# ufal/neuralmonkey

Hardware: AMD Instinct MI355X
Metric: target tokens/sec/node (train), 512-hid GRU+attn (higher is better)
Workload: dtype f32; 1 GPU; translation.ini-shape: biGRU-512 enc + Bahdanau attn + GRU-512 dec, B=128/GPU, src_len=tgt_len=50, V=32000, weights N(0,0.05)/orthogonal (BASELINE.md 3), CrossEntropyTrainer(l2=1e-8, clip_norm=1.0) + Adam(1e-4), one optimizer step per step, 8 distinct HBM-resident batches in rotation; global_batch=128, seq_len=50, parallelism=dp1

## Files before the change

neuralmonkey_amd/_lib.py:

```python
import ctypes
import os
from ctypes import c_char_p, c_float, c_int, c_int64, c_void_p

import torch

_HERE = os.path.dirname(os.path.abspath(__file__))
LIB_PATH = os.path.join(_HERE, "libnmhip.so")

_lib = None

P = c_void_p
I = c_int
L = c_int64
F = c_float

SIGNATURES = {
    "nm_last_error": (c_char_p, []),
    "nm_version": (I, []),
    "nm_crc32c": (ctypes.c_uint32, [ctypes.c_uint32, P, L]),
    "nm_gemm_f32": (I, [P, I, I, L, L, L, P, L, P, L, P, L, P, I, I, L, L, L, L, I, P, L]),
    "nm_gemm_f32_group": (I, [P, I, I, L, L, L, P, L, L, L, I, L]),
    "nm_gemm_f32_chain": (I, [P, L, L, L, L, P, L, L, P, L, I, P, L]),
    "nm_colsum_chain": (I, [P, P, ctypes.c_int32, ctypes.c_int32, L, L, L, L, P, I, P, L]),
    "nm_outer_chain": (I, [P, P, L, L, L, L, L, L, P, I]),
    "nm_embedding_gather": (I, [P, P, L, L, P, L, P, L, I, F]),
    "nm_gru_gates_fwd": (I, [P, P, L, L, L, P, P, P, P, P, I, I, I, L, L]),
    "nm_gru_blend_fwd": (I, [P, P, L, L, L, P, P, P, P, P, P, L, L, L, P, I, I, I, L, L]),
    "nm_layer_norm_fwd": (I, [P, P, L, P, P, P, L, P, P, L, L, F]),
    "nm_add_layer_norm_fwd": (I, [P, P, L, P, L, P, P, P, L, P, L, L, L, F]),
    "nm_add_layer_norm_stats_fwd": (I, [P, P, P, P, P, P, P, P, P, L, L, F]),
    "nm_copy_cols": (I, [P, P, L, P, L, L, L]),
    "nm_reduce_sum": (I, [P, P, L, P]),
    "nm_log_softmax": (I, [P, P, L, P, P, P, L, L, L]),
    "nm_attn_workspace_bytes": (L, [L, L, L]),
    "nm_attn_fwd": (I, [P, P, P, P, P, P, P, L, L, L, L, L, P, L, P, P, L, P]),
    "nm_attn_fwd_multi": (I, [P, P, P, P, P, P, P, L, L, L, L, L, L, L, P, L, P, P, L, P]),
    "nm_gru_rh_seq": (I, [P, P, P, P, P, I, L, L, I, L]),
    "nm_gru_gemm": (I, [P, P, I, L, P, L, L, P, L, L]),
    "nm_gru_seq_fwd": (I, [P, P, ctypes.c_int32, L, L, L, L, P, L, L, P, L, L, P, L, P]),
    "nm_gru_seq_bwd": (I, [P, P, ctypes.c_int32, L, L, P, L, L, P, L, L, P, L, P]),
    "nm_lstm_seq_workspace_bytes": (L, [L, L, ctypes.c_int32]),
    "nm_lstm_seq_fwd": (I, [P, P, ctypes.c_int32, L, L, L, P, L, L, F, P, L, P]),
    "nm_lstm_seq_bwd": (I, [P, P, ctypes.c_int32, L, L, P, L, L, P, L, P]),
    "nm_nematus_seq_workspace_bytes": (L, [L, L, ctypes.c_int32]),
    "nm_nematus_seq_fwd": (I, [P, P, ctypes.c_int32, L, L, L, L, P, L, L, P, L, L, P, P, P, L, P]),
    "nm_nematus_seq_bwd": (I, [P, P, ctypes.c_int32, L, L, L, P, L, L, P, L, L, P, L, P]),
    "nm_proj_split_bytes": (L, [L, L]),
    "nm_proj_split_prepare": (I, [P, P, L, I, L, L, P, L]),
    "nm_proj_split_forget": (I, [P]),
    "nm_gru_seq_supported": (I, [L, L, ctypes.c_int32]),
    "nm_gru_seq_workspace_bytes": (L, [L, L, ctypes.c_int32]),
    "nm_gru_seq_failed": (I, [P]),
    "nm_gru_seq_force_give_up": (I, [ctypes.c_int32]),
    "nm_gru_seq_test_hog": (I, [P, ctypes.c_int32, L, L]),
    "nm_test_xcc_ids": (I, [P, P, ctypes.c_int32, ctypes.c_int32]),
    "nm_create": (I, [I, P]),
    "nm_destroy": (I, [P]),
    "nm_ctx_bind": (I, [P]),
    "nm_ctx_current": (P, []),
    "nm_ctx_device": (I, [P]),
    "nm_ctx_switch": (I, [P, c_char_p, P]),
    "nm_ctx_set_background": (I, [P, I]),
    "nm_allreduce_unique_id": (I, [P, L]),
    "nm_allreduce_init": (I, [I, I, P, P]),
    "nm_allreduce_bucket": (I, [P, P, P, L]),
    "nm_allreduce_wait": (I, [P, P]),
    "nm_allreduce_destroy": (I, [P]),
    "nm_prof_enable": (I, [P, I]),
    "nm_prof_attn_step": (I, [P, P, P]),
    "nm_row_stats": (I, [P, P, L, L, L, P, P, P]),
    "nm_gumbel_argmax": (I, [P, P, L, L, L, ctypes.c_uint32, P]),
    "nm_greedy_update": (I, [P, P, P, P, P, L, I, P]),
    "nm_xent": (I, [P, P, L, L, L, P, P, P, P, I, F]),
    "nm_xent_colsum": (I, [P, P, L, L, L, P, P, P, P, F, P, L]),
    "nm_beam_workspace_bytes": (L, [L, L, L]),
    "nm_beam_topk_step": (I, [P, P, L, L, L, L, P, P, P, P, P, P, I, P, P, P, P, P, P, P, P, L, P]),
    "nm_beam_topk_step_fused": (I, [P, P, L, L, L, L, P, P, P, P, I, P, P, P, P, P, P, P, P, L, P, P, P]),
    "nm_tanh_bwd": (I, [P, P, P, L]),
    "nm_colsum_workspace_bytes": (L, [L]),
    "nm_colsum": (I, [P, P, L, L, L, P, I, P, L]),
    "nm_colsum_algo": (I, [P, P, L, L, L, P, I, P, L, I]),
    "nm_embedding_scatter_add": (I, [P, P, L, L, P, L, P, L, I]),
    "nm_layer_norm_bwd": (I, [P, P, P, P, P, P, P, P, L, L]),
    "nm_layer_norm_bwd_params_workspace_bytes": (L, [L]),
    "nm_layer_norm_bwd_params": (I, [P, P, P, P, P, P, P, L, L, P, P, I, P, L]),
    "nm_gru_step_bwd": (I, [P, I, P, P, L, L, L, P, P, P, P, L, L, L, P, L, L, L, P, P, P, P, I, I, I, L, L]),
    "nm_gru_seq_shift": (I, [P, P, P, P, I, L, L, I, L]),
    "nm_attn_softmax_bwd": (I, [P, P, P, P, P, L, L, L]),
    "nm_attn_energy_bwd": (I, [P, P, P, P, P, P, P, P, L, L, L, L, I]),
    "nm_attn_step_bwd": (I, [P, P, L, P, P, P, P, P, L, P, P, P, L, L, L, L, L]),
    "nm_attn_softmax_fwd": (I, [P, P, P, P, L, L, L, L]),
    "nm_ew": (I, [P, I, P, L, P, L, P, L, L, L, F, I]),
    "nm_blend_fwd": (I, [P, P, L, P, L, P, L, P, L, L, L]),
    "nm_blend_bwd": (I, [P, P, L, P, L, P, L, P, L, P, L, P, L, P, L, L, L]),
    "nm_gemm_bf16x3_nt": (I, [P, L, L, L, P, L, P, L, P, L, I, I]),
    "nm_lstm_cell_fwd": (I, [P, P, L, P, L, P, L, P, L, P, L, L, L, F]),
    "nm_lstm_cell_bwd": (I, [P, P, L, P, L, P, L, P, L, P, L, P, L, P, L, L, L, I, I]),
    "nm_nematus_cell_fwd": (I, [P, P, L, P, L, P, L, P, L, P, L, P, P, P, L, L, L]),
    "nm_nematus_state_step": (I, [P, P, L, P, L, P, P, L, P, L, P, P, P, L, L, L]),
    "nm_nematus_full_step": (I, [P, P, L, P, L, P, P, L, P, L, P, P, L, P, P, P, L, L, L, L]),
    "nm_nematus_cell_bwd": (I, [P, P, L, P, P, P, L, P, L, P, L, P, L, P, L, P, L, P, L, L, L, I, I, I, I]),
    "nm_dropout": (I, [P, P, L, P, L, L, L, F, ctypes.c_uint32, P, I]),
    "nm_rnn_select_fwd": (I, [P, P, L, P, L, P, I, P, L, P, L, L, L]),
    "nm_rnn_select_bwd": (I, [P, P, L, P, L, P, I, P, L, P, L, L, L]),
    "nm_reverse_sequence": (I, [P, P, P, P, L, L, L, I]),
    "nm_maxout_fwd": (I, [P, P, L, P, L, P, L, L, L]),
    "nm_maxout_bwd": (I, [P, P, L, P, P, L, L, L, L]),
    "nm_sdp_attn_fwd": (I, [P, P, L, P, L, P, L, P, L, L, L, L, L, L, L, I, F, ctypes.c_uint32, P, P, L, P]),
    "nm_sdp_attn_step": (I, [P, P, L, P, L, P, L, P, L, L, L, L, L, P, L, P, L, P]),
    "nm_sdp_attn_bwd": (I, [P, P, L, P, L, P, L, P, L, P, P, L, L, L, L, L, L, I, F, ctypes.c_uint32, P,
                            P, L, P, L, P, L, P, I]),
    "nm_add_position": (I, [P, P, P, P, L, L, L, L]),
    "nm_unfinished_mask": (I, [P, P, P, L, L]),
    "nm_time_sum": (I, [P, P, P, L, L, L]),
    "nm_time_bcast_add": (I, [P, P, P, L, L, L]),
    "nm_optim_workspace_bytes": (L, [L, L]),
    "nm_optim_regularize_norms": (I, [P, P, P, P, P, P, P, P, P, L, L, F, F, P, P, L]),
    "nm_optim_clip_adam": (I, [P, P, P, P, P, P, P, P, P, P, P, L, L, F, F, F, F, F, P, L]),
    "nm_optim_clip_adadelta": (I, [P, P, P, P, P, P, P, P, P, P, P, L, L, F, F, F, F, P, L]),
    "nm_optim_partials": (I, [P, P, P, P, P, P, P, P, P, L, L, F, F, L, L, P, L]),
    "nm_optim_partials_list": (I, [P, P, P, P, P, P, P, P, P, L, L, F, F, P, L, P, L]),
    "nm_optim_apply_list": (I, [P, I, P, P, P, P, P, P, P, P, P, P, L, L, F, F, F, F, F, P, L, P, P, L]),
    "nm_optim_segments": (I, [P, P, P, P, P, P, P, L, L, P, P, L]),
    "nm_optim_apply": (I, [P, I, P, P, P, P, P, P, P, P, P, P, L, L, F, F, F, F, F, L, L, P, P, L]),
    "nm_zero_if": (I, [P, P, P, L]),
    "nm_fill_u32": (I, [P, P, L, ctypes.c_uint32]),
    "nm_copy_d2d": (I, [P, P, P, L]),
    "nm_gather_rows_f32": (I, [P, P, L, P, P, L, L, L]),
    "nm_beam_reorder_tokens": (I, [P, P, P, P, P, L, L]),
    "nm_beam_backtrace": (I, [P, P, P, P, P, L, L]),
    "nm_logits_stats_tile": (L, [L]),
    "nm_logits_stats_bytes": (L, [L, L]),
    "nm_logits_stats_gemm": (I, [P, I, L, L, L, P, L, P, L, P, P, L, P, L]),
    "nm_greedy_finish": (I, [P, P, L, L, P, P, P, I, P, P, L, L, P, L, P, P, P]),
    "nm_attn_partials_layout": (I, [L, L, L, L, P, P, P]),
    "nm_attn_fwd_partials": (I, [P, P, P, P, P, P, P, L, L, L, L, L, P, L]),
    "nm_step_group": (I, [P, L, P, ctypes.c_int32]),
    "nm_decoder_step_fused": (I, [P, P]),
    "nm_dec_step_cluster_supported": (I, [L, L, L, L]),
    "nm_dec_step_cluster_workspace_bytes": (L, [L, L]),
    "nm_prof_stream_read": (I, [P, P, L, P]),
    "nm_beam_topk_step_tiles": (I, [P, P, L, P, L, L, L, L, P, P, P, P, I, P, P, P, P, P, P, P, P, L, P, P, P]),
    "nm_conv1d_pool_fwd": (I, [P, P, L, I, I, I, I, I, P, P, P, P, P, P, L, P, P, P, P, I]),
    "nm_conv1d_wgrad_workspace_bytes": (L, [I, I, I, I, P, P]),
    "nm_conv1d_pool_bwd": (I, [P, P, L, I, I, I, I, I, P, P, P, P, P, P, L, P, P, I, P, P, I, P, L, I]),
    "nm_highway_fwd": (I, [P, P, P, L, P, L, P, P, P, P, P, L, L]),
    "nm_highway_bwd": (I, [P, P, P, L, P, P, P, P, L, P, L, L, I]),
}

CTC_SIGNATURES = {
    "nm_ctc_workspace_bytes": (L, [L, L, L]),
    "nm_ctc_mask_lengths": (I, [P, P, L, L, L, P]),
    "nm_ctc_loss_fwd": (I, [P, P, L, L, L, L, L, P, L, P, P, I, P, P, P, L]),
    "nm_ctc_loss_bwd": (I, [P, P, L, L, L, L, L, P, L, P, P, P, P, L, L, P, L]),
    "nm_ctc_greedy": (I, [P, P, L, L, L, L, L, P, I, ctypes.c_int32, P, P, P, L]),
}

LABEL_SIGNATURES = {
    "nm_label_rows_max_classes": (L, []),
    "nm_label_rows": (I, [P, P, L, L, L, P, ctypes.c_int32, P, I, P, P, L, P, P, ctypes.c_int32, P]),
    "nm_label_rows_from_stats": (I, [P, P, L, L, L, P, ctypes.c_int32, P, P, P, P, P, P, ctypes.c_int32, P]),
}

POOL_SIGNATURES = {
    "nm_pool_fwd": (I, [P, I, P, L, P, L, L, L, P, L, P]),
    "nm_pool_bwd": (I, [P, I, P, L, P, P, L, P, P, L, L, L, L, P, L, I]),
    "nm_time_softmax_fwd": (I, [P, P, L, P, L, L, L, P, L, P, L, P]),
    "nm_time_softmax_bwd": (I, [P, P, L, P, L, P, P, L, L, L, P, L, I]),
    "nm_sqerr_rows": (I, [P, P, L, L, L, P, P, I, P]),
}

CONVS2S_SIGNATURES = {
    "nm_conv1d_glu_fwd": (I, [P, P, L, L, L, L, L, P, P, P, L, P, P, I]),
    "nm_conv1d_glu_workspace_bytes": (L, [L, L, L, L]),
    "nm_conv1d_glu_bwd": (I, [P, P, L, L, L, L, L, P, P, P, P, L, P, P, L, I, P, P, I, P, L, I]),
}



class NMHipError(RuntimeError):
    pass


class GruEpilogue(ctypes.Structure):
    _fields_ = [("mode", ctypes.c_int32), ("t", ctypes.c_int32), ("rev_mask", ctypes.c_int32),
                ("ndir", ctypes.c_int32), ("R", L), ("H", L), ("lengths", P),
                ("xp", P), ("x_dir", L), ("x_row", L), ("x_time", L),
                ("h_in", P), ("h_out", P), ("ru", P), ("rh", P), ("c_save", P),
                ("out", P), ("o_dir", L), ("o_row", L), ("o_time", L),
                ("dh", P), ("dout", P), ("do_dir", L), ("do_row", L), ("do_time", L),
                ("c", P), ("h0", P), ("hseq", P), ("hs_dir", L), ("hs_row", L), ("hs_time", L),
                ("dxp", P), ("dx_dir", L), ("dx_row", L), ("dx_time", L),
                ("dgpre", P), ("dcpre", P)]


class StepProblem(ctypes.Structure):
    _fields_ = [("A", P), ("lda", L), ("Bt", P), ("ldb", L), ("N", L), ("K", L),
                ("a_kind", ctypes.c_int32), ("epilogue", ctypes.c_int32), ("act", ctypes.c_int32),
                ("nchunk", ctypes.c_int32),
                ("bias", P), ("add", P), ("ldadd", L), ("C", P), ("ldc", L),
                ("pctx", P), ("pstat", P), ("energies", P), ("mask", P), ("weights", P),
                ("S", L), ("mask_div", L), ("mask_mod", L),
                ("h", P), ("ldh", L), ("ru", P), ("rh", P), ("xc", P), ("ldxc", L),
                ("h_out", P), ("ldho", L), ("h_out2", P), ("ldho2", L), ("add_ids", P), ("xc_ids", P)]


class DecoderStep(ctypes.Structure):
    _fields_ = ([(n, L) for n in ("rows", "emb", "rnn", "attn_state", "ctx_width", "out", "vocab", "src_len",
                                  "rows_per_key")] +
                [("cat", P), ("h_copy", P), ("ld_h_copy", L), ("out_state", P), ("ld_out_state", L),
                 ("attn_weights", P), ("logits", P), ("ld_logits", L), ("stats", P), ("stats_bytes", L)] +
                [(n, P) for n in ("ru", "rh", "xc", "y", "pre_e", "pre", "ctx")] +
                [("attn_workspace", P), ("attn_workspace_bytes", L)] +
                [(n, P) for n in ("wg_t", "bg", "wcx_t", "wch_t", "bc", "wq_t", "bq", "keys", "values", "mask", "v",
                                  "attn_bias", "wo_h_t", "wo_e_t", "wo_c_t", "bo", "w_vocab")] +
                [("ld_w_vocab", L), ("b_vocab", P), ("out_act", ctypes.c_int32), ("vocab_trans_b", ctypes.c_int32)] +
                [(n, L) for n in ("ld_cat", "ld_ctx", "ld_wg", "ld_wcx", "ld_wch", "ld_wq", "ld_wo_h", "ld_wo_e",
                                  "ld_wo_c")] +
                [("in_table", P), ("ld_table", L), ("in_ids", P)] +
                [("cluster_ws", P), ("cluster_ws_bytes", L), ("sticky_error", P)])


def load():
    global _lib
    if _lib is not None:
        return _lib
    if not os.path.exists(LIB_PATH):
        raise NMHipError(
            f"{LIB_PATH} is missing: build it with `python -m neuralmonkey_amd.build` "
            "(hipcc --offload-arch=gfx950). There is no CPU fallback.")
    lib = ctypes.CDLL(LIB_PATH)
    for name, (res, args) in (list(SIGNATURES.items()) + list(CTC_SIGNATURES.items())
                              + list(LABEL_SIGNATURES.items()) + list(POOL_SIGNATURES.items())
                              + list(CONVS2S_SIGNATURES.items())):
        fn = getattr(lib, name)
        fn.restype = res
        fn.argtypes = args
    _lib = lib
    return lib


def check(code, what):
    if code != 0:
        msg = load().nm_last_error()
        raise NMHipError(f"{what} failed ({code}): {msg.decode() if msg else '?'}")
```

neuralmonkey_amd/csrc/nm_gemm.hip:

```cpp
#include <atomic>

#include "nm_common.h"

#include <stdlib.h>

typedef float f32x16 __attribute__((ext_vector_type(16)));

bool nm_medium_gemm(hipStream_t st, int transB, long M, long N, long K, const float* A, long lda, const float* B,
                    long ldb, float* C, long ldc, const float* bias, int act, int accumulate);

struct GemmArgs {
    const float* A;
    const float* B;
    float* C;
    const float* bias;
    int M, N, K;
    long lda, ldb, ldc;
    long sA, sB, sC;
    int act;
    int accumulate;
    float* ws;
    int splitk;
    int swizzle;
    float* stats;
    int store_c;
    int prio;
    const float* const* ptrs;
    int chain_k;
};

__device__ __forceinline__ float apply_act(float x, int act) {
    if (act == 1) return nm_tanh(x);
    if (act == 2) return fmaxf(x, 0.0f);
    return x;
}

__device__ __forceinline__ void store_tile32(const GemmArgs& g, float* __restrict__ C,
                                             const f32x16& acc, int m0, int n0, int lane) {
    const int col = n0 + (lane & 31);
    if (col >= g.N) return;
    const float bv = g.bias ? g.bias[col] : 0.0f;
#pragma unroll
    for (int r = 0; r < 16; ++r) {
        const int row = m0 + (r & 3) + 8 * (r >> 2) + 4 * (lane >> 5);
        if (row < g.M) {
            float* p = C + (long)row * g.ldc + col;
            float v = acc[r] + bv;
            if (g.accumulate) v += *p;
            *p = apply_act(v, g.act);
        }
    }
}

template <int WM, int WN, int TM, int TN, bool TA, bool TB, bool VEC, int BK, bool STATS = false, int PF = 1,
          int NCH = 1, bool CHAIN = false>
__global__ __launch_bounds__(WM * WN * 64) void gemm_tiled(GemmArgs g, int tiles_m) {
    static_assert(!CHAIN || (TA && !TB && VEC && !STATS), "chained K: the weight-gradient form only");
    constexpr int NT = WM * WN * 64;
    constexpr int BM = WM * 32 * TM, BN = WN * 32 * TN;
    constexpr int LA = BM * BK / 4 / NT, LB = BN * BK / 4 / NT, KQ = BK / 4;
    static_assert(LA >= 1 && LB >= 1 && LA * NT * 4 == BM * BK && LB * NT * 4 == BN * BK, "tile / thread mismatch");
    constexpr int LDAS = BM + 4, LDBS = BN + 4;
    constexpr int A_FLOATS = 2 * BK * LDAS, B_FLOATS = 2 * BK * LDBS;
    constexpr int ST_ROWS = BM > 256 ? 128 : BM / 2;
    constexpr int ST_FLOATS = STATS ? ST_ROWS * (BN + 1) + 3 * NT : 0;
    constexpr int SM_FLOATS = A_FLOATS + B_FLOATS > ST_FLOATS ? A_FLOATS + B_FLOATS : ST_FLOATS;
    static_assert((A_FLOATS * 4) % 16 == 0, "B tile must stay 16-byte aligned");
    __shared__ __attribute__((aligned(16))) float smem[SM_FLOATS];
    float (*As)[BK][LDAS] = reinterpret_cast<float (*)[BK][LDAS]>(smem);
    float (*Bs)[BK][LDBS] = reinterpret_cast<float (*)[BK][LDBS]>(smem + A_FLOATS);

    const int tid = threadIdx.x, lane = tid & 63, wave = tid >> 6;
    int bm, bn;
    {
        const int npid = (int)gridDim.x;
        int pid = (int)blockIdx.x;
        if (g.swizzle) {
            const int per = npid / 8, rem = npid % 8, x = pid % 8, i = pid / 8;
            pid = x * per + (x < rem ? x : rem) + i;
            constexpr int GROUP_M = 8;
            const int tiles_n = npid / tiles_m;
            const int width = GROUP_M * tiles_n;
            const int group = pid / width, first = group * GROUP_M;
            const int gsz = (tiles_m - first) < GROUP_M ? (tiles_m - first) : GROUP_M;
            bm = first + (pid % width) % gsz;
            bn = (pid % width) / gsz;
        } else {
            bm = pid % tiles_m;
            bn = pid / tiles_m;
        }
    }
    const int m0 = bm * BM, n0 = bn * BN;
    const float* __restrict__ A = (g.ptrs && !CHAIN) ? g.ptrs[3 * blockIdx.z] : g.A + (long)blockIdx.z * g.sA;
    const float* __restrict__ B = (g.ptrs && !CHAIN) ? g.ptrs[3 * blockIdx.z + 1] : g.B + (long)blockIdx.z * g.sB;
    float* __restrict__ C = (g.ptrs && !CHAIN) ? const_cast<float*>(g.ptrs[3 * blockIdx.z + 2]) : g.C + (long)blockIdx.z * g.sC;

    float4 ra0[LA], rb0[LB], ra1[PF == 2 ? LA : 1], rb1[PF == 2 ? LB : 1];

    auto load_a = [&](int k0, float4* ra) {
#pragma unroll
        for (int it = 0; it < LA; ++it) {
            const int idx = tid + it * NT;
            int m, k;
            if (TA) { k = idx / (BM / 4); m = (idx % (BM / 4)) * 4; }
            else    { m = idx / KQ;       k = (idx % KQ) * 4; }
            const int gm = m0 + m, gk = k0 + k;
            float4 v = make_float4(0.f, 0.f, 0.f, 0.f);
            if (TA) {
                const float* p = A + (long)gk * g.lda + gm;
                if constexpr (CHAIN) {
                    const int mem = k0 / g.chain_k;
                    p = g.ptrs[3 * mem] + (long)(gk - mem * g.chain_k) * g.lda + gm;
                }
                if (gk < g.K) {
                    if (VEC) { if (gm < g.M) v = *reinterpret_cast<const float4*>(p); }
                    else {
                        if (gm + 0 < g.M) v.x = p[0];
                        if (gm + 1 < g.M) v.y = p[1];
                        if (gm + 2 < g.M) v.z = p[2];
                        if (gm + 3 < g.M) v.w = p[3];
                    }
                }
            } else {
                const float* p = A + (long)gm * g.lda + gk;
                if (gm < g.M) {
                    if (VEC) { if (gk < g.K) v = *reinterpret_cast<const float4*>(p); }
                    else {
                        if (gk + 0 < g.K) v.x = p[0];
                        if (gk + 1 < g.K) v.y = p[1];
                        if (gk + 2 < g.K) v.z = p[2];
                        if (gk + 3 < g.K) v.w = p[3];
                    }
                }
            }
            ra[it] = v;
        }
    };
    auto load_b = [&](int k0, float4* rb) {
#pragma unroll
        for (int it = 0; it < LB; ++it) {
            const int idx = tid + it * NT;
            int n, k;
            if (!TB) { k = idx / (BN / 4); n = (idx % (BN / 4)) * 4; }
            else     { n = idx / KQ;       k = (idx % KQ) * 4; }
            const int gn = n0 + n, gk = k0 + k;
            float4 v = make_float4(0.f, 0.f, 0.f, 0.f);
            if (!TB) {
                const float* p = B + (long)gk * g.ldb + gn;
                if constexpr (CHAIN) {
                    const int mem = k0 / g.chain_k;
                    p = g.ptrs[3 * mem + 1] + (long)(gk - mem * g.chain_k) * g.ldb + gn;
                }
                if (gk < g.K) {
                    if (VEC) { if (gn < g.N) v = *reinterpret_cast<const float4*>(p); }
                    else {
                        if (gn + 0 < g.N) v.x = p[0];
                        if (gn + 1 < g.N) v.y = p[1];
                        if (gn + 2 < g.N) v.z = p[2];
                        if (gn + 3 < g.N) v.w = p[3];
                    }
                }
            } else {
                const float* p = B + (long)gn * g.ldb + gk;
                if (gn < g.N) {
                    if (VEC) { if (gk < g.K) v = *reinterpret_cast<const float4*>(p); }
                    else {
                        if (gk + 0 < g.K) v.x = p[0];
                        if (gk + 1 < g.K) v.y = p[1];
                        if (gk + 2 < g.K) v.z = p[2];
                        if (gk + 3 < g.K) v.w = p[3];
                    }
                }
            }
            rb[it] = v;
        }
    };
    auto store_lds = [&](int buf, const float4* ra, const float4* rb) {
#pragma unroll
        for (int it = 0; it < LA; ++it) {
            const int idx = tid + it * NT;
            if (TA) {
                const int k = idx / (BM / 4), m = (idx % (BM / 4)) * 4;
                *reinterpret_cast<float4*>(&As[buf][k][m]) = ra[it];
            } else {
                const int m = idx / KQ, k = (idx % KQ) * 4;
                As[buf][k + 0][m] = ra[it].x;
                As[buf][k + 1][m] = ra[it].y;
                As[buf][k + 2][m] = ra[it].z;
                As[buf][k + 3][m] = ra[it].w;
            }
        }
#pragma unroll
        for (int it = 0; it < LB; ++it) {
            const int idx = tid + it * NT;
            if (!TB) {
                const int k = idx / (BN / 4), n = (idx % (BN / 4)) * 4;
                *reinterpret_cast<float4*>(&Bs[buf][k][n]) = rb[it];
            } else {
                const int n = idx / KQ, k = (idx % KQ) * 4;
                Bs[buf][k + 0][n] = rb[it].x;
                Bs[buf][k + 1][n] = rb[it].y;
                Bs[buf][k + 2][n] = rb[it].z;
                Bs[buf][k + 3][n] = rb[it].w;
            }
        }
    };

    static_assert(NCH == 1 || NCH == 2 || NCH == 4, "accumulation chains: 1, 2 or 4");
    static_assert(NCH == 1 || PF == 1, "chains are implemented for the one-tile-ahead loop");
    f32x16 accs[NCH][TM][TN];
#pragma unroll
    for (int c = 0; c < NCH; ++c)
#pragma unroll
        for (int i = 0; i < TM; ++i)
#pragma unroll
            for (int j = 0; j < TN; ++j)
#pragma unroll
                for (int r = 0; r < 16; ++r) accs[c][i][j][r] = 0.0f;
    f32x16 (&acc)[TM][TN] = accs[0];

    const int wm = (wave / WN) * 32 * TM, wn = (wave % WN) * 32 * TN;
    const int nkt_all = (g.K + BK - 1) / BK;
    const int per_slice = (nkt_all + g.splitk - 1) / g.splitk;
    const int kt0 = blockIdx.y * per_slice;
    const int nkt = min(nkt_all, kt0 + per_slice);

    auto mma_tile = [&](int cur, f32x16 (&acc)[TM][TN]) {
        float a[2][TM], b[2][TN];
#pragma unroll
        for (int i = 0; i < TM; ++i) a[0][i] = As[cur][lane >> 5][wm + i * 32 + (lane & 31)];
#pragma unroll
        for (int j = 0; j < TN; ++j) b[0][j] = Bs[cur][lane >> 5][wn + j * 32 + (lane & 31)];
#pragma unroll
        for (int kk = 0; kk < BK; kk += 2) {
            const int p = (kk >> 1) & 1;
            if (kk + 2 < BK) {
                const int kr = kk + 2 + (lane >> 5);
#pragma unroll
                for (int i = 0; i < TM; ++i) a[p ^ 1][i] = As[cur][kr][wm + i * 32 + (lane & 31)];
#pragma unroll
                for (int j = 0; j < TN; ++j) b[p ^ 1][j] = Bs[cur][kr][wn + j * 32 + (lane & 31)];
            }
#pragma unroll
            for (int i = 0; i < TM; ++i)
#pragma unroll
                for (int j = 0; j < TN; ++j)
                    acc[i][j] = __builtin_amdgcn_mfma_f32_32x32x2f32(a[p][i], b[p][j], acc[i][j], 0, 0, 0);
            __builtin_amdgcn_sched_group_barrier(0x100, TM + TN, 0);
            __builtin_amdgcn_sched_group_barrier(0x008, TM * TN, 0);
        }
    };

    load_a(kt0 * BK, ra0);
    load_b(kt0 * BK, rb0);
    store_lds(0, ra0, rb0);
    __syncthreads();
    if constexpr (PF == 2) {
        if (kt0 + 1 < nkt) { load_a((kt0 + 1) * BK, ra1); load_b((kt0 + 1) * BK, rb1); }
        int kt = kt0;
        while (kt < nkt) {
            if (kt + 2 < nkt) { load_a((kt + 2) * BK, ra0); load_b((kt + 2) * BK, rb0); }
            mma_tile(0, accs[0]);
            if (kt + 1 < nkt) store_lds(1, ra1, rb1);
            __syncthreads();
            if (++kt >= nkt) break;
            if (kt + 2 < nkt) { load_a((kt + 2) * BK, ra1); load_b((kt + 2) * BK, rb1); }
            mma_tile(1, accs[0]);
            if (kt + 1 < nkt) store_lds(0, ra0, rb0);
            __syncthreads();
            ++kt;
        }
    } else if constexpr (NCH == 1) {
        int cur = 0;
        for (int kt = kt0; kt < nkt; ++kt) {
            if (kt + 1 < nkt) { load_a((kt + 1) * BK, ra0); load_b((kt + 1) * BK, rb0); }
            mma_tile(cur, accs[0]);
            if (kt + 1 < nkt) store_lds(cur ^ 1, ra0, rb0);
            __syncthreads();
            cur ^= 1;
        }
    } else {
        int kt = kt0;
        while (kt < nkt) {
#pragma unroll
            for (int c = 0; c < NCH; ++c) {
                if (kt + 1 < nkt) { load_a((kt + 1) * BK, ra0); load_b((kt + 1) * BK, rb0); }
                mma_tile(c & 1, accs[c]);
                if (kt + 1 < nkt) store_lds((c & 1) ^ 1, ra0, rb0);
                __syncthreads();
                if (++kt >= nkt) break;
            }
        }
#pragma unroll
        for (int i = 0; i < TM; ++i)
#pragma unroll
            for (int j = 0; j < TN; ++j) {
                if constexpr (NCH == 4) {
#pragma unroll
                    for (int r = 0; r < 16; ++r)
                        accs[0][i][j][r] = (accs[0][i][j][r] + accs[1][i][j][r]) + (accs[2][i][j][r] + accs[3][i][j][r]);
                } else {
#pragma unroll
                    for (int r = 0; r < 16; ++r) accs[0][i][j][r] += accs[1][i][j][r];
                }
            }
    }

    if (g.splitk > 1) {
        GemmArgs gs = g;
        gs.ldc = g.N; gs.bias = nullptr; gs.act = 0; gs.accumulate = 0;
        float* slab = g.ws + (long)blockIdx.y * g.M * g.N;
#pragma unroll
        for (int i = 0; i < TM; ++i)
#pragma unroll
            for (int j = 0; j < TN; ++j)
                store_tile32(gs, slab, acc[i][j], m0 + wm + i * 32, n0 + wn + j * 32, lane);
        return;
    }
    if constexpr (STATS) {
        if (g.act == 9) return;
        constexpr int HR = ST_ROWS, TS = BN + 1;
        constexpr int NP = BM / HR;
        static_assert(NP * HR == BM, "statistics epilogue: whole passes");
        constexpr int TPR = NT / HR, CW = BN / TPR;
        static_assert(NT % HR == 0 && BN % TPR == 0 && TPR <= 16, "statistics epilogue thread layout");
        float* T = smem;
        float* pmax = smem + HR * TS;
        int* parg = reinterpret_cast<int*>(pmax + NT);
        float* psum = pmax + 2 * NT;
        bool okj[TN];
#pragma unroll
        for (int j = 0; j < TN; ++j) {
            const int col = n0 + wn + j * 32 + (lane & 31);
            okj[j] = col < g.N;
            const float bv = (okj[j] && g.bias) ? g.bias[col] : 0.0f;
#pragma unroll
            for (int i = 0; i < TM; ++i)
#pragma unroll
                for (int r = 0; r < 16; ++r) acc[i][j][r] += bv;
        }
        const int tiles_n = (int)gridDim.x / tiles_m;
        const int rr = tid % HR, q = tid / HR;
        for (int h = 0; h < NP; ++h) {
            __syncthreads();
#pragma unroll
            for (int i = 0; i < TM; ++i) {
                const int rbase = wm + i * 32 - h * HR;
                if (rbase >= 0 && rbase < HR) {
#pragma unroll
                    for (int j = 0; j < TN; ++j)
#pragma unroll
                        for (int r = 0; r < 16; ++r)
                            T[(rbase + (r & 3) + 8 * (r >> 2) + 4 * (lane >> 5)) * TS + wn + j * 32 + (lane & 31)] =
                                okj[j] ? acc[i][j][r] : -INFINITY;
                }
            }
            __syncthreads();
            const float* trow = T + rr * TS + q * CW;
            float best = -INFINITY;
            int bi = 0x7fffffff;
#pragma unroll
            for (int c = 0; c < CW; ++c) {
                const float v = trow[c];
                if (v > best) { best = v; bi = n0 + q * CW + c; }
            }
            pmax[q * HR + rr] = best;
            parg[q * HR + rr] = bi;
            __syncthreads();
            float m = pmax[rr];
#pragma unroll
            for (int w = 1; w < TPR; ++w) m = fmaxf(m, pmax[w * HR + rr]);
            float sum = 0.0f;
#pragma unroll
            for (int c = 0; c < CW; ++c) sum += expf(trow[c] - m);
            psum[q * HR + rr] = sum;
            __syncthreads();
            const int row = m0 + h * HR + tid;
            if (tid < HR && row < g.M) {
                float tot = psum[tid];
                int a = parg[tid];
#pragma unroll
                for (int w = 1; w < TPR; ++w) {
                    tot += psum[w * HR + tid];
                }
                float bm = pmax[tid];
#pragma unroll
                for (int w = 1; w < TPR; ++w)
                    if (pmax[w * HR + tid] > bm) { bm = pmax[w * HR + tid]; a = parg[w * HR + tid]; }
                float4 rec;
                rec.x = bm; rec.y = tot; rec.z = __int_as_float(a); rec.w = 0.0f;
                *reinterpret_cast<float4*>(g.stats + ((long)row * tiles_n + bn) * 4) = rec;
            }
        }
        if (!g.store_c) return;
        GemmArgs gs = g;
        gs.bias = nullptr;
#pragma unroll
        for (int i = 0; i < TM; ++i)
#pragma unroll
            for (int j = 0; j < TN; ++j)
                store_tile32(gs, C, acc[i][j], m0 + wm + i * 32, n0 + wn + j * 32, lane);
        return;
    }
    if (!g.store_c) return;
#pragma unroll
    for (int i = 0; i < TM; ++i)
#pragma unroll
        for (int j = 0; j < TN; ++j)
            store_tile32(g, C, acc[i][j], m0 + wm + i * 32, n0 + wn + j * 32, lane);
}

__global__ void splitk_reduce(GemmArgs g) {
    const long idx = (long)blockIdx.x * blockDim.x + threadIdx.x;
    const long total = (long)g.M * g.N;
    if (idx >= total) return;
    const int row = (int)(idx / g.N), col = (int)(idx - (long)row * g.N);
    float s = 0.0f;
    for (int k = 0; k < g.splitk; ++k) s += g.ws[(long)k * total + idx];
    float* p = g.C + (long)row * g.ldc + col;
    float v = s + (g.bias ? g.bias[col] : 0.0f);
    if (g.accumulate) v += *p;
    *p = apply_act(v, g.act);
}

#include "nm_gru.h"

__device__ __forceinline__ void gru_epilogue(const GruEpi& e, int d, int row, int col, float s) {
    const int H = e.H;
    const long ro = (long)d * e.R + row;
    int pos, ppos;
    const bool live = gru_epi_pos(e, row, d, e.t, pos, ppos);
    if (e.mode == 1) {
        float gate = 0.0f;
        if (live) gate = nm_sigmoid(e.xp[d * e.x_dir + (long)row * e.x_row + (long)pos * e.x_time + col] + s);
        e.ru[ro * 2 * H + col] = gate;
        if (col < H) e.rh[ro * H + col] = live ? gate * e.h_in[ro * H + col] : 0.0f;
    } else if (e.mode == 2) {
        const float hp = e.h_in[ro * H + col];
        if (!live) {
            if (e.h_out != e.h_in) e.h_out[ro * H + col] = hp;
            if (e.c_save) e.c_save[ro * H + col] = 0.0f;
            return;
        }
        const float c = nm_tanh(e.xp[d * e.x_dir + (long)row * e.x_row + (long)pos * e.x_time + 2 * H + col] + s);
        const float u = e.ru[ro * 2 * H + H + col];
        const float hn = u * hp + (1.0f - u) * c;
        e.h_out[ro * H + col] = hn;
        if (e.c_save) e.c_save[ro * H + col] = c;
        if (e.out) e.out[d * e.o_dir + (long)row * e.o_row + (long)pos * e.o_time + col] = hn;
    } else if (e.mode == 3) {
        if (!live) { e.dgpre[ro * 2 * H + col] = 0.0f; return; }
        const float rr = e.ru[ro * 2 * H + col];
        const float hp = gru_epi_hprev(e, ro, d, row, e.t, ppos, col);
        const float drp = s * hp * rr * (1.0f - rr);
        e.dh[ro * H + col] += s * rr;
        e.dgpre[ro * 2 * H + col] = drp;
        e.dxp[d * e.dx_dir + (long)row * e.dx_row + (long)pos * e.dx_time + col] = drp;
    } else {
        if (!live) {
            e.dh[ro * H + col] = s;
            e.dcpre[ro * H + col] = 0.0f;
            e.dgpre[ro * 2 * H + H + col] = 0.0f;
            return;
        }
        float dhv = s;
        if (e.dout) dhv += e.dout[d * e.do_dir + (long)row * e.do_row + (long)pos * e.do_time + col];
        const float u = e.ru[ro * 2 * H + H + col];
        const float c = e.c[ro * H + col];
        const float hp = gru_epi_hprev(e, ro, d, row, e.t, ppos, col);
        const float dcp = dhv * (1.0f - u) * (1.0f - c * c);
        const float dup = dhv * (hp - c) * u * (1.0f - u);
        e.dh[ro * H + col] = dhv * u;
        e.dcpre[ro * H + col] = dcp;
        e.dgpre[ro * 2 * H + H + col] = dup;
        float* dx = e.dxp + d * e.dx_dir + (long)row * e.dx_row + (long)pos * e.dx_time;
        dx[H + col] = dup;
        dx[2 * H + col] = dcp;
    }
}

struct GruPre {
    float a, b, c, d;
    int pos, ppos;
    bool live;
};

__device__ __forceinline__ GruPre gru_epi_load(const GruEpi& e, int d, int row, int col, const float* __restrict__ C,
                                               long ldc, bool accumulate) {
    GruPre q;
    q.a = q.b = q.c = q.d = 0.0f;
    const int H = e.H;
    const long ro = (long)d * e.R + row;
    q.live = gru_epi_pos(e, row, d, e.t, q.pos, q.ppos);
    if (e.mode == 1) {
        if (q.live) q.a = e.xp[d * e.x_dir + (long)row * e.x_row + (long)q.pos * e.x_time + col];
        if (col < H && q.live) q.b = e.h_in[ro * H + col];
    } else if (e.mode == 2) {
        q.b = e.h_in[ro * H + col];
        if (q.live) {
            q.a = e.xp[d * e.x_dir + (long)row * e.x_row + (long)q.pos * e.x_time + 2 * H + col];
            q.c = e.ru[ro * 2 * H + H + col];
        }
    } else if (e.mode == 3) {
        if (q.live) {
            q.a = e.ru[ro * 2 * H + col];
            q.b = gru_epi_hprev(e, ro, d, row, e.t, q.ppos, col);
            q.c = e.dh[ro * H + col];
        }
    } else {
        if (accumulate) q.d = C[(long)row * ldc + col];
        if (q.live) {
            if (e.dout) q.a = e.dout[d * e.do_dir + (long)row * e.do_row + (long)q.pos * e.do_time + col];
            q.b = e.ru[ro * 2 * H + H + col];
            q.c = e.c[ro * H + col];
        }
    }
    return q;
}

__device__ __forceinline__ void gru_epi_apply(const GruEpi& e, const GruPre& q, int d, int row, int col, float s) {
    const int H = e.H;
    const long ro = (long)d * e.R + row;
    if (e.mode == 1) {
        const float gate = q.live ? nm_sigmoid(q.a + s) : 0.0f;
        e.ru[ro * 2 * H + col] = gate;
        if (col < H) e.rh[ro * H + col] = q.live ? gate * q.b : 0.0f;
    } else if (e.mode == 2) {
        const float hp = q.b;
        if (!q.live) {
            if (e.h_out != e.h_in) e.h_out[ro * H + col] = hp;
            if (e.c_save) e.c_save[ro * H + col] = 0.0f;
            return;
        }
        const float c = nm_tanh(q.a + s);
        const float u = q.c;
        const float hn = u * hp + (1.0f - u) * c;
        e.h_out[ro * H + col] = hn;
        if (e.c_save) e.c_save[ro * H + col] = c;
        if (e.out) e.out[d * e.o_dir + (long)row * e.o_row + (long)q.pos * e.o_time + col] = hn;
    } else if (e.mode == 3) {
        if (!q.live) { e.dgpre[ro * 2 * H + col] = 0.0f; return; }
        const float rr = q.a, hp = q.b;
        const float drp = s * hp * rr * (1.0f - rr);
        e.dh[ro * H + col] = q.c + s * rr;
        e.dgpre[ro * 2 * H + col] = drp;
        e.dxp[d * e.dx_dir + (long)row * e.dx_row + (long)q.pos * e.dx_time + col] = drp;
    } else {
        s += q.d;
        if (!q.live) {
            e.dh[ro * H + col] = s;
            e.dcpre[ro * H + col] = 0.0f;
            e.dgpre[ro * 2 * H + H + col] = 0.0f;
            return;
        }
        const float dhv = s + q.a;
        const float u = q.b, c = q.c;
        const float hp = gru_epi_hprev(e, ro, d, row, e.t, q.ppos, col);
        const float dcp = dhv * (1.0f - u) * (1.0f - c * c);
        const float dup = dhv * (hp - c) * u * (1.0f - u);
        e.dh[ro * H + col] = dhv * u;
        e.dcpre[ro * H + col] = dcp;
        e.dgpre[ro * 2 * H + H + col] = dup;
        float* dx = e.dxp + d * e.dx_dir + (long)row * e.dx_row + (long)q.pos * e.dx_time;
        dx[H + col] = dup;
        dx[2 * H + col] = dcp;
    }
}

template <int KS, bool TB>
__global__ __launch_bounds__(KS * 64) void gemm_skinny(GemmArgs g, int tiles_m, GruEpi epi) {
    if (g.prio) __builtin_amdgcn_s_setprio(3);
    __shared__ float red[KS][16][64];
    const int tid = threadIdx.x, lane = tid & 63, wave = tid >> 6;
    const int bm = blockIdx.x % tiles_m, bn = blockIdx.x / tiles_m;
    const int m0 = bm * 32, n0 = bn * 32;
    const float* __restrict__ A = g.A + (long)blockIdx.z * g.sA;
    const float* __restrict__ B = g.B + (long)blockIdx.z * g.sB;
    float* __restrict__ C = g.C + (long)blockIdx.z * g.sC;

    const int r = lane & 31, half = lane >> 5;
    const int mm = min(m0 + r, g.M - 1), nn = min(n0 + r, g.N - 1);
    const int kper = ((g.K / 8 + KS - 1) / KS) * 8;
    const int kbeg = wave * kper, kend = min(g.K, kbeg + kper);

    f32x16 acc;
#pragma unroll
    for (int i = 0; i < 16; ++i) acc[i] = 0.0f;

    const float* ap = A + (long)mm * g.lda + 4 * half;
    const float* bp = TB ? (B + (long)nn * g.ldb + 4 * half) : (B + (long)(4 * half) * g.ldb + nn);
    for (int k0 = kbeg; k0 < kend; k0 += 64) {
        float4 av[8], bv[8];
#pragma unroll
        for (int c = 0; c < 8; ++c) {
            const int k = k0 + 8 * c;
            av[c] = make_float4(0.f, 0.f, 0.f, 0.f);
            bv[c] = av[c];
            if (k < kend) {
                av[c] = *reinterpret_cast<const float4*>(ap + k);
                if (TB) {
                    bv[c] = *reinterpret_cast<const float4*>(bp + k);
                } else {
                    const float* q = bp + (long)k * g.ldb;
                    bv[c].x = q[0];
                    bv[c].y = q[g.ldb];
                    bv[c].z = q[2 * g.ldb];
                    bv[c].w = q[3 * g.ldb];
                }
            }
        }
#pragma unroll
        for (int c = 0; c < 8; ++c) {
            if (k0 + 8 * c >= kend) break;
            acc = __builtin_amdgcn_mfma_f32_32x32x2f32(av[c].x, bv[c].x, acc, 0, 0, 0);
            acc = __builtin_amdgcn_mfma_f32_32x32x2f32(av[c].y, bv[c].y, acc, 0, 0, 0);
            acc = __builtin_amdgcn_mfma_f32_32x32x2f32(av[c].z, bv[c].z, acc, 0, 0, 0);
            acc = __builtin_amdgcn_mfma_f32_32x32x2f32(av[c].w, bv[c].w, acc, 0, 0, 0);
        }
    }
#pragma unroll
    for (int i = 0; i < 16; ++i) red[wave][i][lane] = acc[i];
    __syncthreads();
    for (int o = tid; o < 16 * 64; o += KS * 64) {
        const int reg = o >> 6, ln = o & 63;
        float s = 0.0f;
#pragma unroll
        for (int w = 0; w < KS; ++w) s += red[w][reg][ln];
        const int col = n0 + (ln & 31);
        const int row = m0 + (reg & 3) + 8 * (reg >> 2) + 4 * (ln >> 5);
        if (row < g.M && col < g.N) {
            if (epi.mode) {
                if (g.accumulate) s += C[(long)row * g.ldc + col];
                gru_epilogue(epi, blockIdx.z, row, col, s);
                continue;
            }
            float* p = C + (long)row * g.ldc + col;
            float v = s + (g.bias ? g.bias[col] : 0.0f);
            if (g.accumulate) v += *p;
            *p = apply_act(v, g.act);
        }
    }
}

typedef float f32x4 __attribute__((ext_vector_type(4)));

template <int KS, bool TB>
__device__ __forceinline__ void skinny16_tile(const GemmArgs& g, int tiles_m, const GruEpi& epi, int tile, int z,
                                              float (*red)[4][64]) {
    const int tid = threadIdx.x, lane = tid & 63, wave = tid >> 6;
    const int bm = tile % tiles_m, bn = tile / tiles_m;
    const int m0 = bm * 16, n0 = bn * 16;
    const float* __restrict__ A = g.A + (long)z * g.sA;
    const float* __restrict__ B = g.B + (long)z * g.sB;
    float* __restrict__ C = g.C + (long)z * g.sC;

    const int i16 = lane & 15, kq = lane >> 4;
    const int mm = min(m0 + i16, g.M - 1), nn = min(n0 + i16, g.N - 1);
    const int kper = (((g.K + 15) / 16 + KS - 1) / KS) * 16;
    const int kbeg = wave * kper, kend = min(g.K, kbeg + kper);

    f32x4 acc;
#pragma unroll
    for (int i = 0; i < 4; ++i) acc[i] = 0.0f;

    const int e_col = n0 + (tid & 15), e_row = m0 + 4 * ((tid & 63) >> 4) + (tid >> 6);
    const bool e_ok = tid < 256 && e_row < g.M && e_col < g.N;
    GruPre pre;
    float e_bias = 0.0f, e_old = 0.0f;
    if (e_ok) {
        if (epi.mode) pre = gru_epi_load(epi, z, e_row, e_col, C, g.ldc, g.accumulate != 0);
        else {
            if (g.bias) e_bias = g.bias[e_col];
            if (g.accumulate) e_old = C[(long)e_row * g.ldc + e_col];
        }
    }

    const float* ap = A + (long)mm * g.lda + 4 * kq;
    const float* bp = TB ? (B + (long)nn * g.ldb + 4 * kq) : (B + (long)(4 * kq) * g.ldb + nn);
    for (int k0 = kbeg; k0 < kend; k0 += 64) {
        float4 av[4], bv[4];
#pragma unroll
        for (int c = 0; c < 4; ++c) {
            const int k = k0 + 16 * c;
            av[c] = make_float4(0.f, 0.f, 0.f, 0.f);
            bv[c] = av[c];
            if (k + 4 * kq < kend) {
                av[c] = *reinterpret_cast<const float4*>(ap + k);
                if (TB) {
                    bv[c] = *reinterpret_cast<const float4*>(bp + k);
                } else {
                    const float* q = bp + (long)k * g.ldb;
                    bv[c].x = q[0];
                    bv[c].y = q[g.ldb];
                    bv[c].z = q[2 * g.ldb];
                    bv[c].w = q[3 * g.ldb];
                }
            }
        }
#pragma unroll
        for (int c = 0; c < 4; ++c) {
            if (k0 + 16 * c >= kend) break;
            acc = __builtin_amdgcn_mfma_f32_16x16x4f32(av[c].x, bv[c].x, acc, 0, 0, 0);
            acc = __builtin_amdgcn_mfma_f32_16x16x4f32(av[c].y, bv[c].y, acc, 0, 0, 0);
            acc = __builtin_amdgcn_mfma_f32_16x16x4f32(av[c].z, bv[c].z, acc, 0, 0, 0);
            acc = __builtin_amdgcn_mfma_f32_16x16x4f32(av[c].w, bv[c].w, acc, 0, 0, 0);
        }
    }
#pragma unroll
    for (int i = 0; i < 4; ++i) red[wave][i][lane] = acc[i];
    __syncthreads();
    static_assert(KS >= 4, "the epilogue maps one output element to each of the first 256 threads");
    if (e_ok) {
// ... 45 lines not shown
        for (int i = 0; i < 4; ++i) acc[g][i] = 0.0f;
    const float* ap = p.h + (long)mm * p.ldh + 4 * kq;
    const float* bp = p.w + (long)(4 * kq) * p.ldw + un;
    for (int k0 = kbeg; k0 < kend; k0 += 64) {
        float4 av[4], bv[3][4];
#pragma unroll
        for (int c = 0; c < 4; ++c) {
            const int k = k0 + 16 * c;
            av[c] = make_float4(0.f, 0.f, 0.f, 0.f);
#pragma unroll
            for (int g = 0; g < 3; ++g) bv[g][c] = av[c];
            if (k + 4 * kq < kend) {
                av[c] = *reinterpret_cast<const float4*>(ap + k);
#pragma unroll
                for (int g = 0; g < 3; ++g) {
                    const float* q = bp + (long)k * p.ldw + (long)g * p.H;
                    bv[g][c].x = q[0];
                    bv[g][c].y = q[p.ldw];
                    bv[g][c].z = q[2 * p.ldw];
                    bv[g][c].w = q[3 * p.ldw];
                }
            }
        }
#pragma unroll
        for (int c = 0; c < 4; ++c) {
            if (k0 + 16 * c >= kend) break;
#pragma unroll
            for (int g = 0; g < 3; ++g) {
                acc[g] = __builtin_amdgcn_mfma_f32_16x16x4f32(av[c].x, bv[g][c].x, acc[g], 0, 0, 0);
                acc[g] = __builtin_amdgcn_mfma_f32_16x16x4f32(av[c].y, bv[g][c].y, acc[g], 0, 0, 0);
                acc[g] = __builtin_amdgcn_mfma_f32_16x16x4f32(av[c].z, bv[g][c].z, acc[g], 0, 0, 0);
                acc[g] = __builtin_amdgcn_mfma_f32_16x16x4f32(av[c].w, bv[g][c].w, acc[g], 0, 0, 0);
            }
        }
    }
#pragma unroll
    for (int g = 0; g < 3; ++g)
#pragma unroll
        for (int i = 0; i < 4; ++i) red[wave][g][i][lane] = acc[g][i];
    __syncthreads();
    static_assert(KS >= 4, "one output element per thread of the first four waves");
    const int e_col = u0 + (tid & 15), e_row = m0 + 4 * ((tid & 63) >> 4) + (tid >> 6);
    if (tid >= 256 || e_row >= p.M || e_col >= p.H) return;
    const int reg = tid >> 6, ln = tid & 63;
    float s[3];
#pragma unroll
    for (int g = 0; g < 3; ++g) {
        float t = 0.0f;
#pragma unroll
        for (int w = 0; w < KS; ++w) t += red[w][g][reg][ln];
        s[g] = t + (p.b ? p.b[g * p.H + e_col] : 0.0f);
    }
    const float* xr = p.x + (long)e_row * p.ldx + e_col;
    const float r = nm_sigmoid(s[0] + xr[0]);
    const float u = nm_sigmoid(s[1] + xr[p.H]);
    const float c = nm_tanh(s[2] * r + xr[2 * p.H]);
    p.hn[(long)e_row * p.ldhn + e_col] = u * p.h[(long)e_row * p.ldh + e_col] + (1.0f - u) * c;
    if (p.ru) {
        p.ru[(long)e_row * 2 * p.H + e_col] = r;
        p.ru[(long)e_row * 2 * p.H + p.H + e_col] = u;
    }
    if (p.c) p.c[(long)e_row * p.H + e_col] = c;
    if (p.sc) p.sc[(long)e_row * p.ldsc + e_col] = s[2];
}

struct NemFull {
    NemStep st;
    const float* xin; long ldxi;
    const float* wi; long ldwi;
    const float* bi;
    int D;
};

template <int KS>
__device__ __forceinline__ void nem_accumulate(const float* __restrict__ A, long lda, const float* __restrict__ W, long ldw,
                                               int H, int K, int mm, int un, int kq, int wave, f32x4& a0, f32x4& a1,
                                               f32x4& a2) {
    const int kper = (((K + 15) / 16 + KS - 1) / KS) * 16;
    const int kbeg = wave * kper, kend = min(K, kbeg + kper);
    const float* ap = A + (long)mm * lda + 4 * kq;
    const float* bp = W + (long)(4 * kq) * ldw + un;
    for (int k0 = kbeg; k0 < kend; k0 += 64) {
        float4 av[4], bv[3][4];
#pragma unroll
        for (int c = 0; c < 4; ++c) {
            const int k = k0 + 16 * c;
            av[c] = make_float4(0.f, 0.f, 0.f, 0.f);
#pragma unroll
            for (int g = 0; g < 3; ++g) bv[g][c] = av[c];
            if (k + 4 * kq < kend) {
                av[c] = *reinterpret_cast<const float4*>(ap + k);
#pragma unroll
                for (int g = 0; g < 3; ++g) {
                    const float* q = bp + (long)k * ldw + (long)g * H;
                    bv[g][c].x = q[0];
                    bv[g][c].y = q[ldw];
                    bv[g][c].z = q[2 * ldw];
                    bv[g][c].w = q[3 * ldw];
                }
            }
        }
#pragma unroll
        for (int c = 0; c < 4; ++c) {
            if (k0 + 16 * c >= kend) break;
            a0 = __builtin_amdgcn_mfma_f32_16x16x4f32(av[c].x, bv[0][c].x, a0, 0, 0, 0);
            a0 = __builtin_amdgcn_mfma_f32_16x16x4f32(av[c].y, bv[0][c].y, a0, 0, 0, 0);
            a0 = __builtin_amdgcn_mfma_f32_16x16x4f32(av[c].z, bv[0][c].z, a0, 0, 0, 0);
            a0 = __builtin_amdgcn_mfma_f32_16x16x4f32(av[c].w, bv[0][c].w, a0, 0, 0, 0);
            a1 = __builtin_amdgcn_mfma_f32_16x16x4f32(av[c].x, bv[1][c].x, a1, 0, 0, 0);
            a1 = __builtin_amdgcn_mfma_f32_16x16x4f32(av[c].y, bv[1][c].y, a1, 0, 0, 0);
            a1 = __builtin_amdgcn_mfma_f32_16x16x4f32(av[c].z, bv[1][c].z, a1, 0, 0, 0);
            a1 = __builtin_amdgcn_mfma_f32_16x16x4f32(av[c].w, bv[1][c].w, a1, 0, 0, 0);
            a2 = __builtin_amdgcn_mfma_f32_16x16x4f32(av[c].x, bv[2][c].x, a2, 0, 0, 0);
            a2 = __builtin_amdgcn_mfma_f32_16x16x4f32(av[c].y, bv[2][c].y, a2, 0, 0, 0);
            a2 = __builtin_amdgcn_mfma_f32_16x16x4f32(av[c].z, bv[2][c].z, a2, 0, 0, 0);
            a2 = __builtin_amdgcn_mfma_f32_16x16x4f32(av[c].w, bv[2][c].w, a2, 0, 0, 0);
        }
    }
}

template <int KS>
__global__ __launch_bounds__(KS * 64) void nematus_full_step_kernel(NemFull f) {
    const NemStep& p = f.st;
    if (p.prio) __builtin_amdgcn_s_setprio(3);
    __shared__ float red[KS][4][4][64];
    const int tid = threadIdx.x, lane = tid & 63, wave = tid >> 6;
    const int tiles_m = (p.M + 15) / 16;
    const int bm = blockIdx.x % tiles_m, bu = blockIdx.x / tiles_m;
    const int m0 = bm * 16, u0 = bu * 16;
    const int i16 = lane & 15, kq = lane >> 4;
    const int mm = min(m0 + i16, p.M - 1), un = min(u0 + i16, p.H - 1);
    f32x4 acc[4];
#pragma unroll
    for (int g = 0; g < 4; ++g)
#pragma unroll
        for (int i = 0; i < 4; ++i) acc[g][i] = 0.0f;
    nem_accumulate<KS>(p.h, p.ldh, p.w, p.ldw, p.H, p.H, mm, un, kq, wave, acc[0], acc[1], acc[2]);
    nem_accumulate<KS>(f.xin, f.ldxi, f.wi, f.ldwi, p.H, f.D, mm, un, kq, wave, acc[0], acc[1], acc[3]);
#pragma unroll
    for (int g = 0; g < 4; ++g)
#pragma unroll
        for (int i = 0; i < 4; ++i) red[wave][g][i][lane] = acc[g][i];
    __syncthreads();
    static_assert(KS >= 4, "one output element per thread of the first four waves");
    const int e_col = u0 + (tid & 15), e_row = m0 + 4 * ((tid & 63) >> 4) + (tid >> 6);
    if (tid >= 256 || e_row >= p.M || e_col >= p.H) return;
    const int reg = tid >> 6, ln = tid & 63;
    float s[4];
#pragma unroll
    for (int g = 0; g < 4; ++g) {
        float t = 0.0f;
#pragma unroll
        for (int w = 0; w < KS; ++w) t += red[w][g][reg][ln];
        s[g] = t;
    }
    const int H = p.H;
    if (p.b) { s[0] += p.b[e_col]; s[1] += p.b[H + e_col]; s[2] += p.b[2 * H + e_col]; }
    if (f.bi) { s[0] += f.bi[e_col]; s[1] += f.bi[H + e_col]; s[3] += f.bi[2 * H + e_col]; }
    const float r = nm_sigmoid(s[0]);
    const float u = nm_sigmoid(s[1]);
    const float c = nm_tanh(s[2] * r + s[3]);
    p.hn[(long)e_row * p.ldhn + e_col] = u * p.h[(long)e_row * p.ldh + e_col] + (1.0f - u) * c;
    if (p.ru) {
        p.ru[(long)e_row * 2 * H + e_col] = r;
        p.ru[(long)e_row * 2 * H + H + e_col] = u;
    }
    if (p.c) p.c[(long)e_row * H + e_col] = c;
    if (p.sc) p.sc[(long)e_row * p.ldsc + e_col] = s[2];
}

extern "C" int nm_nematus_full_step(void* stream, const float* h_prev, int64_t ldh, const float* w_st, int64_t ldw,
                                    const float* b_st, const float* x, int64_t ldx, const float* w_in, int64_t ldwi,
                                    const float* b_in, float* h_new, int64_t ldhn, float* ru, float* c_out, float* sc_out,
                                    int64_t ldsc, int64_t rows, int64_t H, int64_t D) {
    NM_REQUIRE(h_prev && w_st && x && w_in && h_new, "nm_nematus_full_step: null pointer");
    NM_REQUIRE(rows >= 0 && H > 0 && H % 8 == 0 && D > 0 && D % 8 == 0 && ldh >= H && ldh % 4 == 0 && ldx >= D &&
                   ldx % 4 == 0 && ldw >= 3 * H && ldwi >= 3 * H && ldhn >= H && (!sc_out || ldsc >= H) && rows < (1 << 24),
               "nm_nematus_full_step: bad shape rows=%ld H=%ld D=%ld (H, D in steps of 8, rows of h and x 16-byte aligned)",
               (long)rows, (long)H, (long)D);
    NM_REQUIRE(nm_aligned16(h_prev) && nm_aligned16(x), "nm_nematus_full_step: h_prev / x not 16-byte aligned");
    NM_REQUIRE(h_new != h_prev, "nm_nematus_full_step: the new state may not overwrite the old one (other tiles read it)");
    if (rows == 0) return NM_OK;
    NemFull f{{h_prev, (long)ldh, w_st, (long)ldw, b_st, nullptr, 0, h_new, (long)ldhn, ru, c_out, sc_out, (long)ldsc,
               (int)rows, (int)H, nm_cur()->sw.background ? 0 : nm_cur()->sw.step_prio},
              x, (long)ldx, w_in, (long)ldwi, b_in, (int)D};
    const dim3 grid((unsigned)(nm_cdiv(rows, 16) * nm_cdiv(H, 16)));
    hipLaunchKernelGGL(nematus_full_step_kernel<8>, grid, dim3(512), 0, nm_stream(stream), f);
    NM_LAUNCH_CHECK("nm_nematus_full_step");
}

extern "C" int nm_nematus_state_step(void* stream, const float* h_prev, int64_t ldh, const float* w_st, int64_t ldw,
                                     const float* b_st, const float* x_all, int64_t ldx, float* h_new, int64_t ldhn,
                                     float* ru, float* c_out, float* sc_out, int64_t ldsc, int64_t rows, int64_t H) {
    NM_REQUIRE(h_prev && w_st && x_all && h_new, "nm_nematus_state_step: null pointer");
    NM_REQUIRE(rows >= 0 && H > 0 && H % 8 == 0 && ldh >= H && ldh % 4 == 0 && ldw >= 3 * H && ldx >= 3 * H && ldhn >= H &&
                   (!sc_out || ldsc >= H) && rows < (1 << 24),
               "nm_nematus_state_step: bad shape rows=%ld H=%ld (H in steps of 8, rows of h 16-byte aligned)", (long)rows,
               (long)H);
    NM_REQUIRE(nm_aligned16(h_prev), "nm_nematus_state_step: h_prev not 16-byte aligned");
    NM_REQUIRE(h_new != h_prev, "nm_nematus_state_step: the new state may not overwrite the old one (other tiles read it)");
    if (rows == 0) return NM_OK;
    NemStep p{h_prev, (long)ldh, w_st, (long)ldw, b_st, x_all, (long)ldx, h_new, (long)ldhn, ru, c_out, sc_out, (long)ldsc,
              (int)rows, (int)H, nm_cur()->sw.background ? 0 : nm_cur()->sw.step_prio};
    const dim3 grid((unsigned)(nm_cdiv(rows, 16) * nm_cdiv(H, 16)));
    if (H >= 512) hipLaunchKernelGGL(nematus_state_step_kernel<16>, grid, dim3(1024), 0, nm_stream(stream), p);
    else hipLaunchKernelGGL(nematus_state_step_kernel<8>, grid, dim3(512), 0, nm_stream(stream), p);
    NM_LAUNCH_CHECK("nm_nematus_state_step");
}

static constexpr int NM_GEMM_BG_MAX_PAD = 96 * 1024;
static inline int bg_pad(int want_lds, int static_lds) {
    if (want_lds <= static_lds) return 0;
    const int pad = ((want_lds - static_lds + 255) / 256) * 256;
    return pad > NM_GEMM_BG_MAX_PAD ? NM_GEMM_BG_MAX_PAD : pad;
}

typedef std::atomic<unsigned> DevMask;

template <typename Kern, typename... Args>
static void launch_padded(Kern kern, DevMask& devs, int pad, dim3 grid, dim3 block, hipStream_t st, Args... args) {
    if (pad > 0) {
        const unsigned ok_bit = 1u << (nm_cur()->device & 15), bad_bit = ok_bit << 16;
        unsigned seen = devs.load(std::memory_order_relaxed);
        if (!(seen & (ok_bit | bad_bit))) {
            const bool ok = hipFuncSetAttribute((const void*)kern, hipFuncAttributeMaxDynamicSharedMemorySize,
                                                NM_GEMM_BG_MAX_PAD) == hipSuccess;
            if (!ok) (void)hipGetLastError();
            seen = devs.fetch_or(ok ? ok_bit : bad_bit, std::memory_order_relaxed) | (ok ? ok_bit : bad_bit);
        }
        if ((seen & bad_bit) && pad > 30 * 1024) pad = 30 * 1024;
    }
    hipLaunchKernelGGL(kern, grid, block, (size_t)pad, st, args...);
}

static inline int bg_lds_target() {
    const int cap = nm_cur()->sw.gemm_bg_wgs;
    return (cap >= 1 && cap <= 3) ? 160 * 1024 / (cap + 1) + 512 : 0;
}

static void launch_skinny(const GemmArgs& g_in, int batch, bool tb, const GruEpi& epi, hipStream_t st) {
    GemmArgs g = g_in;
    const bool background = nm_cur()->sw.background != 0;
    g.prio = background ? 0 : nm_cur()->sw.step_prio;
    const int want = background ? bg_lds_target() : 0;
    const int K = g.K;
    const bool no16 = nm_cur()->sw.gemm_no16;
    if (!no16 && K >= 256 && (long)nm_cdiv(g.M, 32) * nm_cdiv(g.N, 32) * batch < 256) {
        const int tiles_m = nm_cdiv(g.M, 16), tiles_n = nm_cdiv(g.N, 16);
        dim3 grid(tiles_m * tiles_n, 1, (unsigned)batch);
        static const bool wide = !(getenv("NM_SKINNY16_WIDE") && atoi(getenv("NM_SKINNY16_WIDE")) == 0);
        const long ntiles = (long)tiles_m * tiles_n * batch;
        const int ks = (K >= 512 && !(wide && ntiles > 512)) ? 16 : 8;
        static DevMask devs16[4];
#define NM_GS16(KS_, I_)                                                                                               \
    do {                                                                                                               \
        const int pad = bg_pad(want, KS_ * 1024);                                                                      \
        if (tb) launch_padded(gemm_skinny16<KS_, true>, devs16[I_], pad, grid, dim3(KS_ * 64), st, g, tiles_m, epi);   \
        else launch_padded(gemm_skinny16<KS_, false>, devs16[I_ + 1], pad, grid, dim3(KS_ * 64), st, g, tiles_m, epi); \
    } while (0)
        if (ks == 16) NM_GS16(16, 0);
        else NM_GS16(8, 2);
#undef NM_GS16
        return;
    }
    const int tiles_m = nm_cdiv(g.M, 32), tiles_n = nm_cdiv(g.N, 32);
    dim3 grid(tiles_m * tiles_n, 1, (unsigned)batch);
    const int ks = (K >= 512) ? 16 : (K >= 256 ? 8 : (K >= 128 ? 4 : 1));
    static DevMask devs32[8];
#define NM_GS(KS_, I_)                                                                                               \
    do {                                                                                                             \
        const int pad = bg_pad(want, KS_ * 4096);                                                                    \
        if (tb) launch_padded(gemm_skinny<KS_, true>, devs32[I_], pad, grid, dim3(KS_ * 64), st, g, tiles_m, epi);   \
        else launch_padded(gemm_skinny<KS_, false>, devs32[I_ + 1], pad, grid, dim3(KS_ * 64), st, g, tiles_m, epi); \
    } while (0)
    if (ks == 16) NM_GS(16, 0);
    else if (ks == 8) NM_GS(8, 2);
    else if (ks == 4) NM_GS(4, 4);
    else NM_GS(1, 6);
#undef NM_GS
}

template <int WM, int WN, int TM, int TN, int BK, int PF = 1, int NCH = 1>
static void launch_tiled(const GemmArgs& g, int batch, bool ta, bool tb, bool vec, hipStream_t st, int pad_lds = 0) {
    const int tiles_m = nm_cdiv(g.M, WM * 32 * TM), tiles_n = nm_cdiv(g.N, WN * 32 * TN);
    dim3 grid(tiles_m * tiles_n, g.splitk, batch), block(WM * WN * 64);
    static DevMask attr_devs[8];
#define NM_GT(TA_, TB_, V_)                                                                              \
    launch_padded(gemm_tiled<WM, WN, TM, TN, TA_, TB_, V_, BK, false, PF, NCH>,                         \
                  attr_devs[(TA_ ? 4 : 0) + (TB_ ? 2 : 0) + (V_ ? 1 : 0)], pad_lds, grid, block, st, g, tiles_m)
    if (vec) {
        if (!ta && !tb) NM_GT(false, false, true);
        else if (!ta && tb) NM_GT(false, true, true);
        else if (ta && !tb) NM_GT(true, false, true);
        else NM_GT(true, true, true);
    } else {
        if (!ta && !tb) NM_GT(false, false, false);
        else if (!ta && tb) NM_GT(false, true, false);
        else if (ta && !tb) NM_GT(true, false, false);
        else NM_GT(true, true, false);
    }
#undef NM_GT
}

extern "C" int nm_gemm_f32(void* stream, int transA, int transB, int64_t M, int64_t N, int64_t K,
                           const float* A, int64_t lda, const float* B, int64_t ldb, float* C,
                           int64_t ldc, const float* bias, int act, int accumulate, int64_t batch,
                           int64_t strideA, int64_t strideB, int64_t strideC, int algo,
                           void* workspace, int64_t workspace_bytes) {
    NM_REQUIRE(A && B && C, "nm_gemm_f32: null operand");
    NM_REQUIRE(M >= 0 && N >= 0 && K >= 0 && batch >= 1, "nm_gemm_f32: bad shape %ld %ld %ld x%ld",
               (long)M, (long)N, (long)K, (long)batch);
    NM_REQUIRE(act >= 0 && act <= 2, "nm_gemm_f32: bad act %d", act);
    NM_REQUIRE(M < (1 << 30) && N < (1 << 30) && K < (1 << 30), "nm_gemm_f32: dim too large");
    if (M == 0 || N == 0) return NM_OK;
    NM_REQUIRE(K > 0, "nm_gemm_f32: K == 0");
    GemmArgs g{A, B, C, bias, (int)M, (int)N, (int)K, (long)lda, (long)ldb, (long)ldc,
               (long)strideA, (long)strideB, (long)strideC, act, accumulate, nullptr, 1, 0, nullptr, 1};
    const NmSwitches& sw = nm_cur()->sw;
    const int swz_env = sw.gemm_swz;
    g.swizzle = swz_env;
    const bool nostore = sw.gemm_nostore;
    if (nostore) g.store_c = 0;
    hipStream_t st = nm_stream(stream);
    const bool ta = transA != 0, tb = transB != 0;
    if (algo == 0 && !sw.background && !ta && batch == 1 && !nostore &&
        nm_medium_gemm(st, transB, M, N, K, A, lda, B, ldb, C, ldc, bias, act, accumulate)) {
        NM_LAUNCH_CHECK("nm_gemm_f32 (medium)");
    }

    const bool a_vec = nm_aligned16(A) && lda % 4 == 0 && strideA % 4 == 0 && ((ta ? M : K) % 4 == 0);
    const bool b_vec = nm_aligned16(B) && ldb % 4 == 0 && strideB % 4 == 0 && ((tb ? K : N) % 4 == 0);
    const bool vec = a_vec && b_vec;

    int bg_lds = 0;
    if (algo == 4 || (algo == 0 && sw.background)) {
        algo = 0;
        bg_lds = bg_lds_target();
    }
    bool skinny_ok = !ta && a_vec && K % 8 == 0 && (!tb || b_vec);
    int pick = algo;
    if (pick == 0) {
        const long blocks128 = (long)nm_cdiv(M, 128) * nm_cdiv(N, 128) * batch;
        if (skinny_ok && M <= 256 && (long)N * K <= (4L << 20)) pick = 3;
        else if (blocks128 >= 512) pick = 1;
        else pick = 2;
    }
    if (pick == 3) {
        NM_REQUIRE(skinny_ok, "nm_gemm_f32: skinny path needs transA=0, aligned A, K%%8==0");
        launch_skinny(g, (int)batch, tb, GruEpi{}, st);
    } else {
        if (workspace && batch == 1 && K >= 1024) {
            const bool big = (algo == 1) || (algo == 0 && M >= 128 && N >= 128);
            const int tile = big ? 128 : 64;
            const long tiles = (long)nm_cdiv(M, tile) * nm_cdiv(N, tile);
            const int sk_env = sw.gemm_sk;
            const long nkt = (K + 15) / 16;
            const double kt_us = big ? 0.95 : 0.30;
            long best_sk = 1;
            double best = 1e30;
            for (long sk = 1; sk <= 16; ++sk) {
                if (sk > 1 && (K / sk < 128 || sk * M * N * (long)sizeof(float) > workspace_bytes)) break;
                const long blocks = tiles * sk;
                const long rounds = (blocks + 255) / 256;
                const double per_cu = (double)blocks / 256.0;
                const double thin = per_cu <= 1.0 ? 1.35 : (per_cu <= 2.0 ? 1.15 : 1.0);
                double cost = (double)rounds * (double)((nkt + sk - 1) / sk) * kt_us * thin;
                if (sk > 1) cost += (double)(sk + 1) * M * N * 4.0 / 3.0e6 + 3.0;
                if (cost < best) { best = cost; best_sk = sk; }
            }
            if (sk_env > 0 && sk_env <= 16 && K / sk_env >= 128 &&
                (long)sk_env * M * N * (long)sizeof(float) <= workspace_bytes) best_sk = sk_env;
            if (best_sk >= 2) {
                g.splitk = (int)best_sk;
                g.ws = reinterpret_cast<float*>(workspace);
                if (algo == 0) pick = big ? 1 : 2;
            }
        }
        const int cfg_env = sw.gemm_cfg;
        if (pick == 1) {
            if (bg_lds > 0 && sw.gemm_bg_cfg == 2) launch_tiled<4, 2, 2, 2, 16>(g, (int)batch, ta, tb, vec, st, bg_pad(bg_lds, 50176));
            else if (cfg_env == 1) launch_tiled<4, 2, 1, 2, 16>(g, (int)batch, ta, tb, vec, st, bg_pad(bg_lds, 33792));
            else if (cfg_env == 3) launch_tiled<4, 4, 1, 1, 32>(g, (int)batch, ta, tb, vec, st);
            else if (cfg_env == 4) launch_tiled<4, 2, 1, 2, 32>(g, (int)batch, ta, tb, vec, st);
            else if (cfg_env == 5) launch_tiled<2, 4, 2, 1, 16>(g, (int)batch, ta, tb, vec, st);
            else if (cfg_env == 2) launch_tiled<4, 2, 2, 2, 16>(g, (int)batch, ta, tb, vec, st);
            else if (cfg_env == 6) launch_tiled<4, 2, 1, 2, 16, 2>(g, (int)batch, ta, tb, vec, st);
            else if (cfg_env == 7) launch_tiled<4, 2, 2, 2, 16, 2>(g, (int)batch, ta, tb, vec, st);
            else if (cfg_env == 8) launch_tiled<2, 2, 2, 2, 16, 2>(g, (int)batch, ta, tb, vec, st);
            else if (cfg_env == 9) launch_tiled<4, 2, 1, 2, 32, 2>(g, (int)batch, ta, tb, vec, st);
            else launch_tiled<2, 2, 2, 2, 16>(g, (int)batch, ta, tb, vec, st);
        } else if (sw.gemm_cfg64 == 1 && bg_lds == 0 && g.splitk == 1) {
            launch_tiled<2, 1, 2, 2, 16>(g, (int)batch, ta, tb, vec, st);
        } else if (sw.gemm_cfg64 == 2 && bg_lds == 0 && g.splitk == 1) {
            launch_tiled<1, 2, 2, 2, 16>(g, (int)batch, ta, tb, vec, st);
        } else if (sw.gemm_cfg64 == 3 && bg_lds == 0 && g.splitk == 1) {
            launch_tiled<2, 2, 2, 2, 16>(g, (int)batch, ta, tb, vec, st);
        } else if (sw.gemm_chains == 4) {
            launch_tiled<2, 2, 1, 1, 16, 1, 4>(g, (int)batch, ta, tb, vec, st);
        } else if (sw.gemm_chains == 2) {
            launch_tiled<2, 2, 1, 1, 16, 1, 2>(g, (int)batch, ta, tb, vec, st);
        } else {
            launch_tiled<2, 2, 1, 1, 16>(g, (int)batch, ta, tb, vec, st, bg_pad(bg_lds, 17408));
        }
        if (g.splitk > 1) {
            const long total = (long)M * N;
            hipLaunchKernelGGL(splitk_reduce, dim3(nm_cdiv(total, 256)), dim3(256), 0, st, g);
        }
    }
    NM_LAUNCH_CHECK("nm_gemm_f32");
}

extern "C" int nm_gemm_f32_group(void* stream, int transA, int transB, int64_t M, int64_t N, int64_t K,
                                 const void* pointer_table, int64_t lda, int64_t ldb, int64_t ldc, int accumulate,
                                 int64_t count) {
    NM_REQUIRE(pointer_table && count >= 1 && count < 65536, "nm_gemm_f32_group: null table / bad count %ld", (long)count);
    NM_REQUIRE(M > 0 && N > 0 && K > 0 && M < (1 << 30) && N < (1 << 30) && K < (1 << 30),
               "nm_gemm_f32_group: bad shape %ld %ld %ld", (long)M, (long)N, (long)K);
    const bool ta = transA != 0, tb = transB != 0;
    NM_REQUIRE(lda % 4 == 0 && ldb % 4 == 0 && ldc % 4 == 0 && (ta ? M : K) % 4 == 0 && (tb ? K : N) % 4 == 0,
               "nm_gemm_f32_group: leading dimensions and contiguous extents must be multiples of 4 (the operands "
               "themselves 16-byte aligned)");
    GemmArgs g{nullptr, nullptr, nullptr, nullptr, (int)M, (int)N, (int)K, (long)lda, (long)ldb, (long)ldc,
               0, 0, 0, 0, accumulate, nullptr, 1, 0, nullptr, 1};
    g.swizzle = nm_cur()->sw.gemm_swz;
    g.ptrs = reinterpret_cast<const float* const*>(pointer_table);
    hipStream_t st = nm_stream(stream);
    const long blocks128 = (long)nm_cdiv(M, 128) * nm_cdiv(N, 128) * count;
    if (blocks128 >= 192) launch_tiled<4, 2, 1, 2, 16>(g, (int)count, ta, tb, true, st);
    else launch_tiled<2, 2, 1, 1, 16>(g, (int)count, ta, tb, true, st);
    NM_LAUNCH_CHECK("nm_gemm_f32_group");
}

extern "C" int nm_gemm_f32_chain(void* stream, int64_t M, int64_t N, int64_t rows, int64_t count,
                                 const void* pointer_table, int64_t lda, int64_t ldb, float* C, int64_t ldc,
                                 int accumulate, void* workspace, int64_t workspace_bytes) {
    NM_REQUIRE(pointer_table && C && count >= 1 && count < 65536, "nm_gemm_f32_chain: null pointer / bad count %ld", (long)count);
    NM_REQUIRE(M > 0 && N > 0 && rows > 0 && rows % 16 == 0 && rows * count < (1 << 30) && M < (1 << 30) && N < (1 << 30),
               "nm_gemm_f32_chain: bad shape M=%ld N=%ld rows=%ld (a multiple of 16) x %ld", (long)M, (long)N, (long)rows,
               (long)count);
    NM_REQUIRE(lda % 4 == 0 && ldb % 4 == 0 && M % 4 == 0 && N % 4 == 0,
               "nm_gemm_f32_chain: leading dimensions and M, N must be multiples of 4 (the operands 16-byte aligned)");
    const long K = rows * count;
    GemmArgs g{nullptr, nullptr, C, nullptr, (int)M, (int)N, (int)K, (long)lda, (long)ldb, (long)ldc,
               0, 0, 0, 0, accumulate, nullptr, 1, 0, nullptr, 1};
    g.swizzle = nm_cur()->sw.gemm_swz;
    g.ptrs = reinterpret_cast<const float* const*>(pointer_table);
    g.chain_k = (int)rows;
    const bool big = M >= 128 && N >= 128;
    const int tile = big ? 128 : 64;
    const long tiles = (long)nm_cdiv(M, tile) * nm_cdiv(N, tile);
    if (workspace && K >= 1024) {
        const long nkt = (K + 15) / 16;
        const double kt_us = big ? 0.95 : 0.30;
        long best_sk = 1;
        double best = 1e30;
        for (long sk = 1; sk <= 16; ++sk) {
            if (sk > 1 && (K / sk < 128 || sk * M * N * (long)sizeof(float) > workspace_bytes)) break;
            const long blocks = tiles * sk;
            const long rounds = (blocks + 255) / 256;
            const double per_cu = (double)blocks / 256.0;
            const double thin = per_cu <= 1.0 ? 1.35 : (per_cu <= 2.0 ? 1.15 : 1.0);
            double cost = (double)rounds * (double)((nkt + sk - 1) / sk) * kt_us * thin;
            if (sk > 1) cost += (double)(sk + 1) * M * N * 4.0 / 3.0e6 + 3.0;
            if (cost < best) { best = cost; best_sk = sk; }
        }
        if (best_sk >= 2) { g.splitk = (int)best_sk; g.ws = reinterpret_cast<float*>(workspace); }
    }
    hipStream_t st = nm_stream(stream);
    static DevMask devs[2];
    if (big) {
        const int tiles_m = nm_cdiv(g.M, 128), tiles_n = nm_cdiv(g.N, 128);
        launch_padded(gemm_tiled<4, 2, 1, 2, true, false, true, 16, false, 1, 1, true>, devs[0], 0,
                      dim3(tiles_m * tiles_n, g.splitk, 1), dim3(512), st, g, tiles_m);
    } else {
        const int tiles_m = nm_cdiv(g.M, 64), tiles_n = nm_cdiv(g.N, 64);
        launch_padded(gemm_tiled<2, 2, 1, 1, true, false, true, 16, false, 1, 1, true>, devs[1], 0,
                      dim3(tiles_m * tiles_n, g.splitk, 1), dim3(256), st, g, tiles_m);
    }
    if (g.splitk > 1)
        hipLaunchKernelGGL(splitk_reduce, dim3(nm_cdiv((long)M * N, 256)), dim3(256), 0, st, g);
    NM_LAUNCH_CHECK("nm_gemm_f32_chain");
}


extern "C" int nm_gru_gemm(void* stream, const nm_gru_epilogue* e, int transB, int64_t K, const float* A,
                           int64_t lda, int64_t strideA, const float* B, int64_t ldb, int64_t strideB) {
    NM_REQUIRE(e && A && B, "nm_gru_gemm: null pointer");
    NM_REQUIRE(e->mode >= 1 && e->mode <= 4, "nm_gru_gemm: mode must be 1..4");
    NM_REQUIRE(e->R > 0 && e->H > 0 && e->H % 4 == 0 && e->ndir >= 1 && e->ndir <= 2 && K > 0 && K % 8 == 0,
               "nm_gru_gemm: bad shape R=%ld H=%ld K=%ld", (long)e->R, (long)e->H, (long)K);
    NM_REQUIRE(nm_aligned16(A) && lda % 4 == 0 && strideA % 4 == 0 &&
                   (!transB || (nm_aligned16(B) && ldb % 4 == 0 && strideB % 4 == 0)),
               "nm_gru_gemm: operands must be 16-byte aligned with strides %% 4 == 0");
    const bool fwd = e->mode <= 2;
    if (fwd) NM_REQUIRE(e->xp && e->h_in && e->ru && (e->mode == 1 ? (e->rh != nullptr) : (e->h_out != nullptr)),
                        "nm_gru_gemm: missing forward operand");
    else NM_REQUIRE(e->dh && e->ru && e->hseq && e->dxp && e->dgpre && (e->mode == 3 || (e->c && e->dcpre)),
                    "nm_gru_gemm: missing backward operand");
    const int64_t N = (e->mode == 1) ? 2 * e->H : e->H;
    GemmArgs g{A, B, e->dh, nullptr, (int)e->R, (int)N, (int)K, (long)lda, (long)ldb, (long)e->H,
               (long)strideA, (long)strideB, (long)(e->R * e->H), 0, e->mode == 4 ? 1 : 0, nullptr, 1, 0, nullptr, 1};
    GruEpi d;
    d.mode = e->mode; d.lengths = e->lengths; d.t = e->t; d.rev_mask = e->rev_mask; d.H = (int)e->H; d.R = e->R;
    d.xp = e->xp; d.x_dir = e->x_dir; d.x_row = e->x_row; d.x_time = e->x_time;
    d.h_in = e->h_in; d.h_out = e->h_out; d.ru = e->ru; d.rh = e->rh; d.c_save = e->c_save;
    d.out = e->out; d.o_dir = e->o_dir; d.o_row = e->o_row; d.o_time = e->o_time;
    d.dh = e->dh; d.dout = e->dout; d.do_dir = e->do_dir; d.do_row = e->do_row; d.do_time = e->do_time;
    d.c = e->c; d.h0 = e->h0; d.hseq = e->hseq; d.hs_dir = e->hs_dir; d.hs_row = e->hs_row; d.hs_time = e->hs_time;
    d.dxp = e->dxp; d.dx_dir = e->dx_dir; d.dx_row = e->dx_row; d.dx_time = e->dx_time;
    d.dgpre = e->dgpre; d.dcpre = e->dcpre;
    launch_skinny(g, e->ndir, transB != 0, d, nm_stream(stream));
    NM_LAUNCH_CHECK("nm_gru_gemm");
}

static int stats_cfg() {
    return nm_cur()->sw.stats_cfg;
}
extern "C" int64_t nm_logits_stats_tile(int64_t M) { return (M <= 256 && !(stats_cfg() & 1)) ? 64 : 128; }

extern "C" int64_t nm_logits_stats_bytes(int64_t M, int64_t N) {
    if (M <= 0 || N <= 0) return 0;
    const int64_t tile = nm_logits_stats_tile(M);
    return M * ((N + tile - 1) / tile) * 4 * (int64_t)sizeof(float);
}

extern "C" int nm_logits_stats_gemm(void* stream, int transB, int64_t M, int64_t N, int64_t K, const float* A,
                                    int64_t lda, const float* B, int64_t ldb, const float* bias, float* C,
                                    int64_t ldc, float* stats, int64_t stats_bytes) {
    NM_REQUIRE(A && B && stats, "nm_logits_stats_gemm: null operand");
    NM_REQUIRE(M > 0 && N > 0 && K > 0 && M < (1 << 30) && N < (1 << 30) && K < (1 << 30),
               "nm_logits_stats_gemm: bad shape %ld %ld %ld", (long)M, (long)N, (long)K);
    NM_REQUIRE(stats_bytes >= nm_logits_stats_bytes(M, N) && nm_aligned16(stats),
               "nm_logits_stats_gemm: statistics buffer too small / unaligned");
    NM_REQUIRE(!C || ldc >= N, "nm_logits_stats_gemm: ldc < N");
    const bool tb = transB != 0;
    const bool vec = nm_aligned16(A) && lda % 4 == 0 && K % 4 == 0 && nm_aligned16(B) && ldb % 4 == 0 &&
                     ((tb ? K : N) % 4 == 0);
    NM_REQUIRE(vec, "nm_logits_stats_gemm: operands must be 16-byte aligned with K, N and the leading dimensions "
                    "multiples of 4");
    GemmArgs g{A, B, C, bias, (int)M, (int)N, (int)K, (long)lda, (long)ldb, (long)(C ? ldc : 0), 0, 0, 0, 0, 0,
               nullptr, 1, 1, stats, C ? 1 : 0};
    const bool ablate = nm_cur()->sw.stats_ablate;
    if (ablate) g.act = 9;
    const int tile = (int)nm_logits_stats_tile(M);
    hipStream_t st = nm_stream(stream);
    if (!ablate && nm_proj_split_try(st, transB, M, N, K, A, lda, B, bias, C, C ? ldc : 0, stats, tile)) {
        NM_LAUNCH_CHECK("nm_logits_stats_gemm (split)");
    }
    if (!ablate && nm_proj_astat_try(st, transB, M, N, K, A, lda, B, ldb, bias, C, C ? ldc : 0, stats, tile)) {
        NM_LAUNCH_CHECK("nm_logits_stats_gemm (activation-stationary)");
    }
    const bool pf2 = (stats_cfg() & 2) != 0;
    const int tiles_m = nm_cdiv(M, 128), tiles_n = nm_cdiv(N, tile);
    dim3 grid(tiles_m * tiles_n, 1, 1), block(512);
#define NM_ST(TN_, BK_, TB_, PF_) \
    hipLaunchKernelGGL((gemm_tiled<4, 2, 1, TN_, false, TB_, true, BK_, true, PF_>), grid, block, 0, st, g, tiles_m)
    if (tile == 64) {
        if (tb) { if (pf2) NM_ST(1, 32, true, 2); else NM_ST(1, 32, true, 1); }
        else { if (pf2) NM_ST(1, 32, false, 2); else NM_ST(1, 32, false, 1); }
    } else {
        if (tb) { if (pf2) NM_ST(2, 16, true, 2); else NM_ST(2, 16, true, 1); }
        else { if (pf2) NM_ST(2, 16, false, 2); else NM_ST(2, 16, false, 1); }
    }
#undef NM_ST
    NM_LAUNCH_CHECK("nm_logits_stats_gemm");
}
```

neuralmonkey_amd/csrc/nm_logits.hip:

```cpp
#include "nm_common.h"
#include <stdlib.h>

#define NM_NEG_INF_F (-1e9f)

template <int NT>
__device__ __forceinline__ void block_argmax(float& v, int& i, float* shv, int* shi) {
#pragma unroll
    for (int off = 32; off > 0; off >>= 1) {
        const float ov = __shfl_xor(v, off, 64);
        const int oi = __shfl_xor(i, off, 64);
        if (ov > v || (ov == v && oi < i)) { v = ov; i = oi; }
    }
    const int w = threadIdx.x >> 6;
    if ((threadIdx.x & 63) == 0) { shv[w] = v; shi[w] = i; }
    __syncthreads();
    if (threadIdx.x == 0) {
        float bv = shv[0];
        int bi = shi[0];
        for (int k = 1; k < NT / 64; ++k)
            if (shv[k] > bv || (shv[k] == bv && shi[k] < bi)) { bv = shv[k]; bi = shi[k]; }
        shv[0] = bv;
        shi[0] = bi;
    }
    __syncthreads();
// ... 888 lines not shown

template <int NT>
__device__ __forceinline__ void merge_row_tiles(const float4* __restrict__ st, int ntiles, float& M, int& A, float& lse,
                                                float* shf, int* shi) {
    float bv = -INFINITY;
    int bi = 0x7fffffff;
    for (int t = threadIdx.x; t < ntiles; t += NT) {
        const float4 r = st[t];
        const int a = __float_as_int(r.z);
        if (r.x > bv || (r.x == bv && a < bi)) { bv = r.x; bi = a; }
    }
    block_argmax<NT>(bv, bi, shf, shi);
    float s = 0.0f;
    for (int t = threadIdx.x; t < ntiles; t += NT) {
        const float4 r = st[t];
        s += r.y * expf(r.x - bv);
    }
    s = block_sum<NT>(s, shf);
    M = bv; A = bi; lse = logf(s);
}

__global__ __launch_bounds__(256) void greedy_finish_kernel(const float4* __restrict__ stats, int ntiles,
                                                            int* __restrict__ finished, int* __restrict__ sym_out,
                                                            int* __restrict__ mask_out, int end_id,
                                                            int* __restrict__ all_finished,
                                                            const float* __restrict__ table, int V, int E,
                                                            float* __restrict__ emb_out, long ld_emb,
                                                            int* __restrict__ argmax_out, float* __restrict__ max_out,
                                                            float* __restrict__ lse_out) {
    __shared__ float shf[4];
    __shared__ int shi[4];
    __shared__ int sym_s;
    const int r = blockIdx.x;
    float M, lse;
    int A;
    merge_row_tiles<256>(stats + (long)r * ntiles, ntiles, M, A, lse, shf, shi);
    if (threadIdx.x == 0) {
        int f = finished[r];
        const int s = f ? 0 : A;
        f = f | (s == end_id);
        finished[r] = f;
        sym_out[r] = s;
        if (mask_out) mask_out[r] = !f;
        if (all_finished && !f) *all_finished = 0;
        if (argmax_out) argmax_out[r] = A;
        if (max_out) max_out[r] = M;
        if (lse_out) lse_out[r] = lse;
        sym_s = s;
    }
    __syncthreads();
    if (!emb_out) return;
    int s = sym_s;
    s = s < 0 ? 0 : (s >= V ? V - 1 : s);
    const float* src = table + (long)s * E;
    float* dst = emb_out + (long)r * ld_emb;
    if ((E & 3) == 0 && (ld_emb & 3) == 0 && nm_aligned16_dev(src) && nm_aligned16_dev(dst)) {
        for (int c = threadIdx.x * 4; c < E; c += 1024)
            *reinterpret_cast<float4*>(dst + c) = *reinterpret_cast<const float4*>(src + c);
    } else {
        for (int c = threadIdx.x; c < E; c += 256) dst[c] = src[c];
    }
}

extern "C" int nm_greedy_finish(void* stream, const float* stats, int64_t ntiles, int64_t R, int32_t* finished,
                                int32_t* sym_out, int32_t* mask_out, int end_id, int32_t* all_finished,
                                const float* table, int64_t V, int64_t E, float* emb_out, int64_t ld_emb,
                                int32_t* argmax_out, float* max_out, float* lse_out) {
    NM_REQUIRE(stats && finished && sym_out && R >= 0 && ntiles > 0, "nm_greedy_finish: bad args");
    NM_REQUIRE(nm_aligned16(stats), "nm_greedy_finish: statistics must be 16-byte aligned");
    NM_REQUIRE(!emb_out || (table && V > 0 && E > 0 && ld_emb >= E), "nm_greedy_finish: bad embedding arguments");
    if (R == 0) return NM_OK;
    hipLaunchKernelGGL(greedy_finish_kernel, dim3((unsigned)R), dim3(256), 0, nm_stream(stream),
                       reinterpret_cast<const float4*>(stats), (int)ntiles, finished, sym_out, mask_out, end_id,
                       all_finished, table, (int)V, (int)E, emb_out, (long)ld_emb, argmax_out, max_out, lse_out);
    NM_LAUNCH_CHECK("nm_greedy_finish");
}

#define TILE_SCAN_TILES 64
template <int K>
__global__ __launch_bounds__(256) void beam_tile_scan_kernel(const float* __restrict__ x, long ldx, int V,
                                                             const float4* __restrict__ stats, int ntiles, int tile_w,
                                                             float* __restrict__ max_out, float* __restrict__ lse_out,
                                                             int k, const float* __restrict__ logprob_sum,
                                                             const int* __restrict__ lengths,
                                                             const int* __restrict__ finished,
                                                             const float* __restrict__ penalty,
                                                             float* __restrict__ part_score, int* __restrict__ part_idx) {
    __shared__ float shf[4];
    __shared__ int shi[4];
    __shared__ float shs[4 * K];
    __shared__ int shx[4 * K];
    __shared__ float cand_s[ROW_SCAN_CAND];
    __shared__ int cand_i[ROW_SCAN_CAND];
    __shared__ int cand_n, tile_n;
    __shared__ int tile_list[TILE_SCAN_TILES];
    const int r = blockIdx.x, tid = threadIdx.x, lane = tid & 63, wave = tid >> 6;
    const int base = (r % k) * V;
    if (finished[r]) {
        if (tid < K) {
            const float pen = penalty[lengths[r]];
            const float lp = (tid == 0) ? 0.0f : NM_NEG_INF_F;
            part_score[(long)r * K + tid] = tid < V ? (logprob_sum[r] + lp) / pen : -INFINITY;
            part_idx[(long)r * K + tid] = tid < V ? base + tid : 0x7fffffff;
        }
        return;
    }
    const float4* st = stats + (long)r * ntiles;
    float bv, lse;
    int bi;
    merge_row_tiles<256>(st, ntiles, bv, bi, lse, shf, shi);
    if (tid == 0) {
        if (max_out) max_out[r] = bv;
        if (lse_out) lse_out[r] = lse;
        cand_n = 0;
        tile_n = 0;
    }
    const float lps = logprob_sum[r];
    const float pen = penalty[lengths[r] + 1];
    float tau = -INFINITY;
    {
        float mine[4];
#pragma unroll
        for (int q = 0; q < 4; ++q) mine[q] = (tid + q * 256 < ntiles) ? st[tid + q * 256].x : -INFINITY;
        for (int p = 0; p < K; ++p) {
            float v = fmaxf(fmaxf(mine[0], mine[1]), fmaxf(mine[2], mine[3]));
            int who = tid;
            block_argmax<256>(v, who, shf, shi);
            tau = v;
            if (who == tid) {
                bool done = false;
#pragma unroll
                for (int q = 0; q < 4; ++q)
                    if (!done && mine[q] == v) { mine[q] = -INFINITY; done = true; }
            }
        }
    }
    const float margin = (fabsf(lse) + fabsf(lps) + (bv - tau) + 1.0f) * (1.0f / 262144.0f);
    const float cut = tau - margin;
    __syncthreads();
    bool overflow = !(cut > -INFINITY) || ntiles > 1024;
    if (!overflow) {
        for (int t = tid; t < ntiles; t += 256) {
            if (st[t].x >= cut) {
                const int slot = atomicAdd(&tile_n, 1);
                if (slot < TILE_SCAN_TILES) tile_list[slot] = t;
            }
        }
        __syncthreads();
        const int nt = tile_n;
        if (nt > TILE_SCAN_TILES) overflow = true;
        else {
            const float* row = x + (long)r * ldx;
            for (int i = tid; i < nt * tile_w; i += 256) {
                const int col = tile_list[i / tile_w] * tile_w + (i % tile_w);
                if (col < V) {
                    const float xe = row[col];
                    if (xe >= cut) {
                        const int slot = atomicAdd(&cand_n, 1);
                        if (slot < ROW_SCAN_CAND) {
                            cand_s[slot] = (lps + ((xe - bv) - lse)) / pen;
                            cand_i[slot] = base + col;
                        }
                    }
                }
            }
            __syncthreads();
            if (cand_n > ROW_SCAN_CAND) overflow = true;
        }
    }
    float s[K];
    int ix[K];
#pragma unroll
    for (int p = 0; p < K; ++p) { s[p] = -INFINITY; ix[p] = 0x7fffffff; }
    if (!overflow) {
        const int ncand = cand_n;
        if (tid < ncand) {
            const float sc = cand_s[tid];
            const int ic = cand_i[tid];
            int rank = 0;
            for (int j = 0; j < ncand; ++j) rank += cand_better(cand_s[j], cand_i[j], sc, ic) ? 1 : 0;
            if (rank < K) { part_score[(long)r * K + rank] = sc; part_idx[(long)r * K + rank] = ic; }
        } else if (tid < K) {
            part_score[(long)r * K + tid] = -INFINITY;
            part_idx[(long)r * K + tid] = 0x7fffffff;
        }
        return;
    }
    {
        const float* row = x + (long)r * ldx;
        for (int v = tid; v < V; v += 256) topk_insert<K>(s, ix, (lps + ((row[v] - bv) - lse)) / pen, base + v);
    }
    topk_wave_merge<K>(s, ix);
    if (lane == 0) {
#pragma unroll
        for (int p = 0; p < K; ++p) { shs[wave * K + p] = s[p]; shx[wave * K + p] = ix[p]; }
    }
    __syncthreads();
    if (wave == 0) {
#pragma unroll
        for (int p = 0; p < K; ++p) {
            s[p] = lane < 4 ? shs[lane * K + p] : -INFINITY;
            ix[p] = lane < 4 ? shx[lane * K + p] : 0x7fffffff;
        }
        topk_wave_merge<K>(s, ix);
        if (lane == 0) {
#pragma unroll
            for (int p = 0; p < K; ++p) { part_score[(long)r * K + p] = s[p]; part_idx[(long)r * K + p] = ix[p]; }
        }
    }
}

extern "C" int nm_beam_topk_step_tiles(void* stream, const float* logits, int64_t ldx, const float* stats,
                                       int64_t tile_w, int64_t B, int64_t k, int64_t V, const float* logprob_sum,
                                       const int32_t* lengths, const int32_t* finished, const float* penalty,
                                       int end_id, float* out_score, int32_t* out_word, int32_t* out_beam,
                                       float* out_logprob_sum, int32_t* out_lengths, int32_t* out_finished,
                                       int32_t* out_src_row, void* workspace, int64_t workspace_bytes,
                                       int32_t* all_finished, float* rmax_out, float* rlse_out) {
    NM_REQUIRE(logits && stats && logprob_sum && lengths && finished && penalty && out_score && out_word && out_beam &&
                   out_logprob_sum && out_lengths && out_finished && out_src_row && workspace && rmax_out && rlse_out,
               "nm_beam_topk_step_tiles: null pointer");
    NM_REQUIRE(B > 0 && k >= 1 && k <= BEAM_MAX_K && V > 0 && k * V < (1L << 31) && ldx >= V,
               "nm_beam_topk_step_tiles: bad shape B=%ld k=%ld V=%ld", (long)B, (long)k, (long)V);
    NM_REQUIRE((tile_w == 64 || tile_w == 128) && nm_aligned16(stats),
               "nm_beam_topk_step_tiles: tile width %ld (nm_logits_stats_tile gives 64 or 128)", (long)tile_w);
    const int64_t ntiles = (V + tile_w - 1) / tile_w;
    NM_REQUIRE(workspace_bytes >= nm_beam_workspace_bytes(B, k, V), "nm_beam_topk_step_tiles: workspace too small");
    float* ps = reinterpret_cast<float*>(workspace);
    int* pi = reinterpret_cast<int*>(ps + B * 64 * BEAM_MAX_K);
    const unsigned rows = (unsigned)(B * k);
    hipStream_t st = nm_stream(stream);
    const float4* st4 = reinterpret_cast<const float4*>(stats);
#define NM_TILES(K_)                                                                                              \
    do {                                                                                                          \
        hipLaunchKernelGGL((beam_tile_scan_kernel<K_>), dim3(rows), dim3(256), 0, st, logits, (long)ldx, (int)V, st4, \
                           (int)ntiles, (int)tile_w, rmax_out, rlse_out, (int)k, logprob_sum, lengths, finished, penalty, \
                           ps, pi);                                                                               \
        hipLaunchKernelGGL((beam_topk_final<K_>), dim3((unsigned)B), dim3(64), 0, st, logits, (long)ldx, (int)V,   \
                           (int)k, rmax_out, rlse_out, logprob_sum, lengths, finished, penalty, ps, pi, (int)k,    \
                           (int)B, end_id, out_score, out_word, out_beam, out_logprob_sum, out_lengths,           \
                           out_finished, out_src_row, all_finished);                                             \
    } while (0)
    if (k <= 4) NM_TILES(4);
    else if (k <= 8) NM_TILES(8);
    else NM_TILES(16);
#undef NM_TILES
    NM_LAUNCH_CHECK("nm_beam_topk_step_tiles");
}

__global__ void gather_rows_f32_kernel(const float* __restrict__ src, long lds_, const int* __restrict__ idx,
                                       float* __restrict__ dst, long ldd, long rows, int w) {
    const long r = blockIdx.y;
    const int c = blockIdx.x * blockDim.x + threadIdx.x;
    if (c < w) dst[r * ldd + c] = src[(long)idx[r] * lds_ + c];
}

extern "C" int nm_gather_rows_f32(void* stream, const float* src, int64_t ld_src, const int32_t* idx,
                                  float* dst, int64_t ld_dst, int64_t rows, int64_t width) {
    NM_REQUIRE(src && idx && dst && rows >= 0 && width >= 0 && src != dst, "nm_gather_rows_f32: bad args");
    if (rows == 0 || width == 0) return NM_OK;
    hipLaunchKernelGGL(gather_rows_f32_kernel, dim3(nm_cdiv(width, 256), (unsigned)rows), dim3(256), 0,
                       nm_stream(stream), src, (long)ld_src, idx, dst, (long)ld_dst, (long)rows, (int)width);
    NM_LAUNCH_CHECK("nm_gather_rows_f32");
}

__global__ void beam_tokens_kernel(const int* __restrict__ src, const int* __restrict__ idx,
                                   const int* __restrict__ word, int* __restrict__ dst, int steps, int R) {
    const int r = blockIdx.x * blockDim.x + threadIdx.x;
    if (r >= R) return;
    const int sr = idx[r];
    for (int t = 0; t < steps; ++t) dst[(long)t * R + r] = src[(long)t * R + sr];
    dst[(long)steps * R + r] = word[r];
}

extern "C" int nm_beam_reorder_tokens(void* stream, const int32_t* src, const int32_t* src_row,
                                      const int32_t* word, int32_t* dst, int64_t steps, int64_t R) {
    NM_REQUIRE(src && src_row && word && dst && steps >= 0 && R > 0 && src != dst,
               "nm_beam_reorder_tokens: bad args");
    hipLaunchKernelGGL(beam_tokens_kernel, dim3(nm_cdiv(R, 256)), dim3(256), 0, nm_stream(stream), src,
                       src_row, word, dst, (int)steps, (int)R);
    NM_LAUNCH_CHECK("nm_beam_reorder_tokens");
}


__global__ void beam_backtrace_kernel(const int* __restrict__ parent, const int* __restrict__ word,
                                      const int* __restrict__ first, int* __restrict__ out, int steps, int R) {
    const int r = blockIdx.x * blockDim.x + threadIdx.x;
    if (r >= R) return;
    int cur = r;
    for (int t = steps - 1; t >= 0; --t) {
        out[(long)(t + 1) * R + r] = word[(long)t * R + cur];
        cur = parent[(long)t * R + cur];
    }
    out[r] = first[cur];
}

extern "C" int nm_beam_backtrace(void* stream, const int32_t* src_row, const int32_t* word, const int32_t* first,
                                 int32_t* out, int64_t steps, int64_t R) {
    NM_REQUIRE(src_row && word && first && out && steps >= 0 && R > 0 && R < (1LL << 31), "nm_beam_backtrace: bad args");
    hipLaunchKernelGGL(beam_backtrace_kernel, dim3(nm_cdiv(R, 64)), dim3(64), 0, nm_stream(stream), src_row, word,
                       first, out, (int)steps, (int)R);
    NM_LAUNCH_CHECK("nm_beam_backtrace");
}
```

neuralmonkey_amd/decoders/decoder.py:

```python
from typing import Any, List, NamedTuple, Optional, Tuple

import contextlib
import os

import numpy as np
import torch

from .. import ops
from ..attention.base_attention import AttentionLoopState, BaseAttention
from ..model.model_part import InitializerSpecs, ModelPart
from ..model.sequence import EmbeddedSequence
from ..model.stateful import Stateful
from ..nn import gru
from ..nn.dropout import dropout
from ..runtime import tensor
from ..vocabulary import END_TOKEN_INDEX, START_TOKEN_INDEX, Vocabulary, sentence_mask
from .autoregressive import (AutoregressiveDecoder, DecoderConstants, DecoderFeedables,
                             DecoderHistories, LoopState)
from .decoder_general import GeneralDecoderMixin, make_stepper
from .encoder_projection import (EncoderProjection, concat_encoder_projection, empty_initial_state,
                                 linear_encoder_projection)
from .output_projection import OutputProjection, OutputProjectionSpec, nonlinear_output

RNN_CELL_TYPES = ("NematusGRU", "GRU", "LSTM")
FORWARD_OVERLAP = int(os.environ.get("NM_FWD_OVERLAP", "1"))
DW_EARLY = os.environ.get("NM_DW_EARLY", "0") != "0"
CHECK_EVERY = int(os.environ.get("NM_CHECK_EVERY", "8"))
CHECK_EVERY_BEAM = int(os.environ.get("NM_CHECK_EVERY_BEAM", "4"))
CHECK_EVERY_TRANSFORMER = int(os.environ.get("NM_CHECK_EVERY_TRANSFORMER", "4"))


class RNNFeedables(NamedTuple):
    prev_rnn_state: torch.Tensor
    prev_rnn_output: torch.Tensor
    prev_contexts: List[torch.Tensor]


class RNNHistories(NamedTuple):
    rnn_outputs: torch.Tensor
    attention_histories: List[Any]


class TrainResult(NamedTuple):
    loss_sum: torch.Tensor
    token_count: float
    steps: int
    saved: dict


class RuntimeResult(NamedTuple):
    symbols: torch.Tensor
    mask: torch.Tensor
    steps: int
    xent_sum: Optional[torch.Tensor]
    logits: Optional[torch.Tensor]
    output_states: torch.Tensor
    rnn_outputs: torch.Tensor
    attention_weights: List[torch.Tensor]


class Decoder(GeneralDecoderMixin, AutoregressiveDecoder):
    def __init__(self, encoders: List[Stateful], vocabulary: Vocabulary, data_id: str, name: str,
                 max_output_len: int, dropout_keep_prob: float = 1.0, embedding_size: int = None,
                 embeddings_source: EmbeddedSequence = None, tie_embeddings: bool = False,
                 label_smoothing: float = None, rnn_size: int = None,
                 output_projection: OutputProjectionSpec = None,
                 encoder_projection: EncoderProjection = None,
                 attentions: List[BaseAttention] = None, attention_on_input: bool = False,
                 rnn_cell: str = "GRU", conditional_gru: bool = False, supress_unk: bool = False,
                 reuse: ModelPart = None, save_checkpoint: str = None, load_checkpoint: str = None,
                 initializers: InitializerSpecs = None) -> None:
        AutoregressiveDecoder.__init__(
            self, name=name, vocabulary=vocabulary, data_id=data_id, max_output_len=max_output_len,
            dropout_keep_prob=dropout_keep_prob, embedding_size=embedding_size,
            embeddings_source=embeddings_source, tie_embeddings=tie_embeddings,
            label_smoothing=label_smoothing, supress_unk=supress_unk, reuse=reuse,
            save_checkpoint=save_checkpoint, load_checkpoint=load_checkpoint, initializers=initializers)
        self.encoders = encoders
        self._output_projection_spec = output_projection
        self._conditional_gru = conditional_gru
        self._attention_on_input = attention_on_input
        self._rnn_cell_str = rnn_cell
        self._rnn_size = rnn_size
        self._encoder_projection = encoder_projection
        self.attentions: List[BaseAttention] = attentions if attentions is not None else []
        if not rnn_size and not encoder_projection and not encoders:
            raise ValueError("No RNN size, no encoders and no encoder_projection specified")
        if self._rnn_cell_str not in RNN_CELL_TYPES:
            raise ValueError("RNN cell must be a either 'GRU', 'LSTM', or 'NematusGRU'. Not {}"
                             .format(self._rnn_cell_str))
        for att in self.attentions:
            att.bind_query_size(self.rnn_size)
            if hasattr(att, "bind_decoder"):
                att.bind_decoder(self)
        self._build_cells()
        if self.embedding_size != self.output_dimension:
            raise ValueError("The dimension ({}) of the output projection must be same as the "
                             "dimension of the input embedding ({})"
                             .format(self.output_dimension, self.embedding_size))

    @property
    def encoder_projection(self) -> EncoderProjection:
        if not hasattr(self, "_enc_proj_cached"):
            if self._encoder_projection is not None:
                proj = self._encoder_projection
            elif not self.encoders:
                proj = empty_initial_state
            elif self._rnn_size is None:
                proj = concat_encoder_projection
            else:
                proj = linear_encoder_projection(self.dropout_keep_prob)
            self._enc_proj_cached = proj
        return self._enc_proj_cached

    @property
    def rnn_size(self) -> int:
        if self._rnn_size is not None:
            return self._rnn_size
        if self._encoder_projection is None:
            assert self.encoders
            return sum(e.output_size for e in self.encoders)
        raise ValueError("Cannot infer RNN size.")

    @property
    def output_projection_spec(self) -> Tuple[OutputProjection, int]:
        if not hasattr(self, "_out_proj_cached"):
            spec = self._output_projection_spec
            if spec is None:
                spec = (nonlinear_output(self.rnn_size)[0], self.rnn_size)
            elif not isinstance(spec, tuple):
                spec = (spec, self.rnn_size)
            self._out_proj_cached = spec
        return self._out_proj_cached

    @property
    def output_projection(self) -> OutputProjection:
        return self.output_projection_spec[0]

    @property
    def output_dimension(self) -> int:
        return self.output_projection_spec[1]

    def declare_variables(self, store) -> None:
        AutoregressiveDecoder.declare_variables(self, store)
        e, h = self.embedding_size, self.rnn_size
        self.encoder_projection.declare_variables(self, store, self.rnn_size, self.encoders)
        self._declare_general_variables(store)
        self.output_projection.declare_variables(
            self, store, h, e, [a.context_vector_size for a in self.attentions])

    def _cell(self, ctx):
        pre = "attention_decoder/OrthoGRUCell"
        e = self.embedding_size
        wg, wc = self.var(ctx, pre + "/gates/kernel"), self.var(ctx, pre + "/candidate/kernel")
        return {"wg_x": wg[:e], "wg_h": wg[e:], "bg": self.var(ctx, pre + "/gates/bias"),
                "wc_x": wc[:e], "wc_h": wc[e:], "bc": self.var(ctx, pre + "/candidate/bias")}

    @tensor
    def initial_state(self, ctx) -> torch.Tensor:
        bsz = int(ctx.fed(self.batch_size))
        out = ctx.buffer((id(self), "s0"), (bsz, self.rnn_size))
        train = bool(ctx.fed(self.train_mode))
        state = self.encoder_projection.apply(ctx, self, self.rnn_size, self.encoders, out, train)
        return dropout(ctx, state, self.dropout_keep_prob, train)

    def _time_loops_beside(self) -> bool:
        encs = list(self.encoders) + [att.encoder for att in self.attentions]
        return any(getattr(enc, "has_time_loop", False) for enc in encs)

    def _input_projection(self, ctx, cell, emb, xp, algo=0):
        h = self.rnn_size
        ops.gemm(emb, cell["wg_x"], out=xp[:, :2 * h], bias=cell["bg"], algo=algo)
        ops.gemm(emb, cell["wc_x"], out=xp[:, 2 * h:], bias=cell["bc"], algo=algo)

    def _recurrent(self, ctx, cell, xp, t_index, x_time_stride, h_prev, h_out, ru, c_save, bufs, rh=None, wt=None):
        h = self.rnn_size
        rows = h_prev.shape[0]
        rh = bufs["rh"] if rh is None else rh
        wg, wc = wt if wt is not None else (cell["wg_h"], cell["wc_h"])
        gru.step_fwd(xp, (0, 3 * h, x_time_stride), h_prev, h_out, wg, wc, ru, rh, c_save,
                     None, (0, 0, 0), None, t_index, 1, rows, h, False, bufs["hg"], bufs["hc"],
                     transposed=wt is not None)

    def _step_bufs(self, ctx, rows):
        h = self.rnn_size
        key = (id(self), "step", rows)
        return {"hg": ctx.buffer(key + ("hg",), (rows, 2 * h)), "hc": ctx.buffer(key + ("hc",), (rows, h)),
                "rh": ctx.buffer(key + ("rh",), (rows, h)), "ru": ctx.buffer(key + ("ru",), (rows, 2 * h)),
                "xp": ctx.buffer(key + ("xp",), (rows, 3 * h))}

    def full_step(self, ctx, cell, emb_in, h_prev, h_out, att_states, out_state, logits, bufs):
        self._input_projection(ctx, cell, emb_in, bufs["xp"])
        self._recurrent(ctx, cell, bufs["xp"], 0, 0, h_prev, h_out, bufs["ru"], None, bufs)
        contexts, new_states = [], []
        for att, st in zip(self.attentions, att_states):
            c, ns = att.attention(ctx, h_out, h_prev, emb_in, st)
            contexts.append(c)
            new_states.append(ns)
        self.output_projection.apply(ctx, self, h_out, emb_in, contexts, out_state)
        self.state_to_logits(ctx, out_state, logits)
        return new_states

    def _dec_input_ids(self, ctx) -> torch.Tensor:
        def shift(ids):
            tb = np.ascontiguousarray(ids.T)
            out = np.empty_like(tb)
            out[0] = START_TOKEN_INDEX
            out[1:] = tb[:-1]
            return out
        key = (id(self), "dec_in_tb")
        if key not in ctx.memo:
            ctx.memo[key] = ctx.session.staged(key, ctx.session.to_device(ctx.fed(self.train_tokens), torch.int32,
                                                                         "dec_in_tb", shift))
        return ctx.memo[key]

    def stage_inputs(self, ctx) -> None:
        AutoregressiveDecoder.stage_inputs(self, ctx)
        if self.has_targets(ctx):
            self._dec_input_ids(ctx)

    def decoding_loop(self, ctx, train_mode: bool, sample: bool = False, temperature: float = 1.0):
        self.check_sampling_args(train_mode, sample, temperature)
        if train_mode:
            return self._train_loop(ctx)
        if sample or temperature != 1.0:
            return self._runtime_loop(ctx, keep_logits=True, sample=sample, temperature=float(temperature))
        return self._runtime_loop(ctx, keep_logits=False)

    def _train_loop(self, ctx, want_grad: bool = False, grad_scale: Optional[torch.Tensor] = None) -> TrainResult:
        if self.uses_general_path(bool(ctx.fed(self.train_mode))):
            return self._general_train_loop(ctx, want_grad, grad_scale)
        key = (id(self), "train")
        tgt = self.train_inputs(ctx)
        tmask = self.train_mask(ctx)
        steps, bsz = tgt.shape
        e, h, v = self.embedding_size, self.rnn_size, len(self.vocabulary)
        cell = self._cell(ctx)
        rows = steps * bsz

        overlap = FORWARD_OVERLAP and ctx.session.side_active() and self._time_loops_beside()
        emb_all = ctx.buffer(key + ("emb",), (steps, bsz, e))
        xp = ctx.buffer(key + ("xp",), (rows, 3 * h))
        dec_ids = self._dec_input_ids(ctx)
        def input_half():
            self.embed_input_symbols(ctx, dec_ids.reshape(-1), out=emb_all.view(rows, e))
            self._input_projection(ctx, cell, emb_all.view(rows, e), xp,
                                   algo=ops.GEMM_BACKGROUND if overlap and FORWARD_OVERLAP == 2 else 0)
        if overlap:
            ctx.session.defer_side(input_half)
        else:
            input_half()

        s0 = self.initial_state(ctx)
        if overlap:
            ctx.session.start_deferred_side()
            ctx.session.join_side(0)
            for att in self.attentions:
                att.attention_states(ctx)
                att.attention_mask(ctx)
            with ctx.session.side(0):
                for att in self.attentions:
                    att.hidden_features(ctx)
        s_ext = ctx.buffer(key + ("s_ext",), (steps + 1, bsz, h))
        ops.copy(s_ext[0], s0)
        s_all = s_ext[1:]
        ru_all = ctx.buffer(key + ("ru_all",), (steps, bsz, 2 * h))
        c_all = ctx.buffer(key + ("c_all",), (steps, bsz, h))
        rh_all = ctx.buffer(key + ("rh_all",), (steps, bsz, h))
        bufs = self._step_bufs(ctx, bsz)
        att_states = [a.initial_loop_state(ctx, bsz, steps) for a in self.attentions]
        y_all = [ctx.buffer(key + ("y", i), (steps, bsz, a.state_size)) for i, a in enumerate(self.attentions)]
        e_all = [ctx.buffer(key + ("e", i), (steps, bsz, st.weights.shape[2])) for i, st in enumerate(att_states)]
        for att in self.attentions:
            att.hidden_features(ctx)
            att.attention_mask(ctx)

        wt = None

        def time_loop():
            for t in range(steps):
                self._recurrent(ctx, cell, xp, t, bsz * 3 * h, s_ext[t], s_all[t], ru_all[t], c_all[t], bufs,
                                rh=rh_all[t], wt=wt)
        loop_h = gru.seq_mode(ctx.session, bsz, h, 1, cell["wg_h"], cell["wc_h"])
        if loop_h:
            gru.seq_fwd(ctx, id(self), loop_h, steps, 1, bsz, h, xp, (0, 3 * h, bsz * 3 * h), s_ext[0], s_ext[1], bsz * h,
                        ru_all[0], bsz * 2 * h, rh_all[0], bsz * h, c_all[0], bsz * h, cell["wg_h"], cell["wc_h"])
        else:
            ctx.session.graphed((id(self), "train_loop", bsz, steps), time_loop)
        if overlap:
            ctx.session.join_side(0)
        for i, att in enumerate(self.attentions):
            att.attention_all_steps(ctx, s_all, y_all[i], att_states[i].contexts, att_states[i].weights, e_all[i])
        att_states = [AttentionLoopState(st.contexts, st.weights, steps) for st in att_states]

        out_all = ctx.buffer(key + ("out",), (rows, self.output_dimension))
        self.output_projection.apply(ctx, self, s_all.view(rows, h), emb_all.view(rows, e),
                                     [st.contexts.view(rows, -1) for st in att_states], out_all)
        logits = ctx.buffer(key + ("logits",), (rows, v))
        self.state_to_logits(ctx, out_all, logits)
        loss_rows = ctx.buffer(key + ("loss_rows",), (rows,))
        db_partial = None
        if want_grad and not self.tie_embeddings and ops.xent_colsum_ok(logits):
            db_partial = ctx.buffer(key + ("db_partial",), (min(rows, ops.XENT_COLSUM_ROWS), v))
            ops.xent_colsum(logits, tgt.reshape(-1), self.xent_weights(tmask.reshape(-1)), loss_rows, grad_scale,
                            self.label_smoothing or 0.0, db_partial)
        else:
            ops.xent(logits, tgt.reshape(-1), self.xent_weights(tmask.reshape(-1)), loss_rows, grad_scale, want_grad,
                     self.label_smoothing or 0.0)
        loss_sum = ctx.buffer(key + ("loss_sum",), (1,))
        ops.reduce_sum(loss_rows, loss_sum)
        for att, st in zip(self.attentions, att_states):
            att.finalize_loop("{}_train".format(self.name), st)
        saved = {"emb_all": emb_all, "xp": xp, "s0": s0, "s_all": s_all, "s_ext": s_ext, "ru_all": ru_all,
                 "c_all": c_all, "rh_all": rh_all, "y_all": y_all, "e_all": e_all,
                 "att_states": att_states, "out_all": out_all,
                 "dlogits": logits if want_grad else None, "db_partial": db_partial, "cell": cell, "steps": steps,
                 "bsz": bsz,
                 "loss_rows": loss_rows, "loss_layout": "tb"}
        return TrainResult(loss_sum, self.train_token_count(ctx), steps, saved)

    def backward(self, ctx, res: TrainResult) -> None:
        store = ctx.store
        sv = res.saved
        if "tape" in sv:
            return self._general_backward(ctx, res)
        steps, bsz = sv["steps"], sv["bsz"]
        rows = steps * bsz
        e, h, v = self.embedding_size, self.rnn_size, len(self.vocabulary)
        key = (id(self), "bwd")
        cell = sv["cell"]
        dlogits, out_all = sv["dlogits"], sv["out_all"]
        emb2 = sv["emb_all"].view(rows, e)
        s2 = sv["s_all"].reshape(rows, h)
        odim = self.output_dimension

        loops = self._time_loops_beside()
        side = ctx.session.side if loops else (lambda lane=0: contextlib.nullcontext())
        bg = ctx.session.leaf_algo() if loops else 0
        acc = self.shares_variables
        from .. import distributed
        dp = distributed.current()
        dp_overlap = dp is not None and bool(ctx.memo.get("dp_overlap", False))

        d_out = ctx.buffer(key + ("d_out",), (rows, odim))
        if self.tie_embeddings:
            emat = self.embedding_matrix(ctx)
            ops.gemm(dlogits, emat, out=d_out)
        else:
            ops.gemm(dlogits, self.var(ctx, "state_to_word_W"), out=d_out, trans_b=True)

        proj = self.output_projection
        if proj.activation == "tanh":
            ops.tanh_bwd(d_out, out_all)
        elif proj.activation != "identity":
            raise NotImplementedError("backward of activation {}".format(proj.activation))
        wo = proj.kernel(ctx, self)
        g_wo = store.g(self.var_name("attention_decoder/{}/kernel".format(proj.scope)))
        ctx_all = [st.contexts.view(rows, -1) for st in sv["att_states"]]
        d_s = ctx.buffer(key + ("d_s",), (rows, h))
        d_emb = ctx.buffer(key + ("d_emb",), (rows, e))
        d_ctx = [ctx.buffer(key + ("d_ctx", i), (rows, c.shape[1])) for i, c in enumerate(ctx_all)]
        row = 0
        for x, dx, sz in zip([s2, emb2] + ctx_all, [d_s, d_emb] + d_ctx, proj.sizes):
            ops.gemm(d_out, wo[row:row + sz], out=dx, trans_b=True)
            row += sz
        with side():
            row = 0
            for x, sz in zip([s2, emb2] + ctx_all, proj.sizes):
                ops.gemm(x, d_out, out=g_wo[row:row + sz], trans_a=True, accumulate=acc, algo=bg)
                row += sz
            ops.colsum(d_out, store.g(self.var_name("attention_decoder/{}/bias".format(proj.scope))), accumulate=acc)

        def vocabulary_projection_gradient():
            if self.tie_embeddings:
                ops.gemm(dlogits, out_all, out=store.g(self.embedding_matrix_name), trans_a=True,
                         accumulate=True, algo=bg)
            else:
                ops.gemm(out_all, dlogits, out=store.g(self.var_name("state_to_word_W")), trans_a=True, accumulate=acc,
                         algo=bg)
                ops.colsum(sv["db_partial"] if sv.get("db_partial") is not None else dlogits,
                           store.g(self.var_name("state_to_word_b")), accumulate=acc)
                if dp_overlap:
                    dp.all_reduce_early(store, [self.var_name("state_to_word_W"), self.var_name("state_to_word_b")])
        early_dw = DW_EARLY
        if early_dw:
            with side(1):
                vocabulary_projection_gradient()

        d_att_states = []
        for i, att in enumerate(self.attentions):
            st = sv["att_states"][i]
            d_att_states.append(att.backward(ctx, d_ctx[i].view(steps, bsz, -1), sv["s_all"], sv["y_all"][i],
                                             st.weights, sv["e_all"][i], d_s))
        if not early_dw:
            with side(1):
                vocabulary_projection_gradient()

        dh = ctx.buffer(key + ("dh",), (1, bsz, h), zero=True)
        dxp = ctx.buffer(key + ("dxp",), (rows, 3 * h))
        dgpre = ctx.buffer(key + ("dgpre",), (2, 1, bsz, 2 * h))
        dcpre = ctx.buffer(key + ("dcpre",), (1, bsz, h))
        drh = ctx.buffer(key + ("drh",), (1, bsz, h))
        s_all = sv["s_all"]
        seq_strides = (0, h, bsz * h)
        dxp_strides = (0, 3 * h, bsz * 3 * h)
        def bptt_loop():
            ops.zero(dh)
            gru.bptt(steps, dh, d_s, seq_strides, sv["ru_all"], sv["c_all"], sv["s0"], s_all, seq_strides, dxp,
                     dxp_strides, cell["wg_h"].unsqueeze(0), cell["wc_h"].unsqueeze(0), None, 1, bsz, h, False,
                     dgpre, dcpre, drh)
        loop_h = gru.seq_mode(ctx.session, bsz, h, 1, cell["wg_h"], cell["wc_h"])
        if loop_h:
            ops.zero(dh)
            gru.seq_bwd(ctx, id(self), loop_h, steps, 1, bsz, h, dh, d_s, seq_strides, sv["ru_all"][0], bsz * 2 * h,
                        sv["c_all"][0], bsz * h, sv["s0"], s_all, seq_strides, dxp, dxp_strides, cell["wg_h"],
                        cell["wc_h"])
            if dp is not None:
                dp.after_time_loops()
        else:
            ctx.session.graphed((id(self), "bptt_loop", bsz, steps), bptt_loop)
        ds0 = dh[0]

        pre = "attention_decoder/OrthoGRUCell"
        g_wg, g_wc = store.g(self.var_name(pre + "/gates/kernel")), store.g(self.var_name(pre + "/candidate/kernel"))
        dg_all, dc_all = dxp[:, :2 * h], dxp[:, 2 * h:]
        s_prev = sv["s_ext"][:steps].reshape(rows, h)
        with side():
            ops.gemm(emb2, dg_all, out=g_wg[:e], trans_a=True, accumulate=acc, algo=bg)
            ops.gemm(s_prev, dg_all, out=g_wg[e:], trans_a=True, accumulate=acc, algo=bg)
            ops.gemm(emb2, dc_all, out=g_wc[:e], trans_a=True, accumulate=acc, algo=bg)
            ops.gemm(sv["rh_all"].view(rows, h), dc_all, out=g_wc[e:], trans_a=True, accumulate=acc, algo=bg)
            ops.colsum(dg_all, store.g(self.var_name(pre + "/gates/bias")), accumulate=acc)
            ops.colsum(dc_all, store.g(self.var_name(pre + "/candidate/bias")), accumulate=acc)
            ops.gemm(dg_all, cell["wg_x"], out=d_emb, trans_b=True, accumulate=True, algo=bg)
            ops.gemm(dc_all, cell["wc_x"], out=d_emb, trans_b=True, accumulate=True, algo=bg)
            ops.embedding_scatter_add(store.g(self.embedding_matrix_name), self._dec_input_ids(ctx).reshape(-1),
                                      d_emb)
            if dp_overlap and not self.tie_embeddings and self.embeddings_source is None:
                sparse = False
                if dp.sparse_embeddings:
                    ids_host = np.concatenate([np.asarray(ctx.fed(self.train_tokens)).reshape(-1),
                                               np.asarray([START_TOKEN_INDEX])])
                    negate = lambda src, dst: ops.ew("scale", src, None, dst, alpha=-1.0)
                    scatter = lambda table, ids, rows: ops.embedding_scatter_add(table, ids, rows)
                    sparse = dp.exchange_sparse_rows(store, self.embedding_matrix_name, ids_host, ops.gather_rows,
                                                     scatter, negate, skip_pad=False)
                if not sparse:
                    dp.all_reduce_early(store, [self.embedding_matrix_name])

        d_enc_out = self.encoder_projection.backward(ctx, self, self.rnn_size, self.encoders, ds0)
        enc_grads = {}
        for att, dst in zip(self.attentions, d_att_states):
            enc_grads.setdefault(att.encoder, [None, None])[0] = dst
        for enc, dfin in zip(self.encoders, d_enc_out):
            enc_grads.setdefault(enc, [None, None])[1] = dfin
        for enc, (dst, dfin) in enc_grads.items():
            ctx.defer_backward(enc, dst, dfin)

    @tensor
    def train_loss(self, ctx) -> torch.Tensor:
        res = self.train_loop_result(ctx)
        out = ctx.buffer((id(self), "train_loss"), (1,))
        alpha = 1.0 / res.token_count if res.token_count else float("nan")
        return ops.ew("scale", res.loss_sum[0:1], None, out, alpha=alpha)[0]

    def _runtime_loop(self, ctx, keep_logits: bool, sample: bool = False, temperature: float = 1.0) -> RuntimeResult:
        key = (id(self), "run", keep_logits)
        plain = not sample and temperature == 1.0
        if not plain:
            key = key + ("sample" if sample else "argmax", temperature)
        bsz = int(ctx.fed(self.batch_size))
        e, h, v = self.embedding_size, self.rnn_size, len(self.vocabulary)
        tmax = self.max_output_len
        has_tgt = self.has_targets(ctx)
        if has_tgt:
            tgt, tmask = self.train_inputs(ctx), self.train_mask(ctx)
            t_target = tgt.shape[0]

        s0 = self.initial_state(ctx)
        s_all = ctx.buffer(key + ("s_all",), (tmax, bsz, h))
        out_all = ctx.buffer(key + ("out_all",), (tmax, bsz, self.output_dimension))
        symbols = ctx.buffer(key + ("sym",), (tmax, bsz), torch.int32, zero=True)
        omask = ctx.buffer(key + ("mask",), (tmax, bsz), torch.int32, zero=True)
        finished = ctx.buffer(key + ("fin",), (bsz,), torch.int32, zero=True)
        allfin = ctx.buffer(key + ("allfin",), (tmax,), torch.int32)
        ops.fill(allfin, 1)
        argmax = ctx.buffer(key + ("argmax",), (bsz,), torch.int32)
        logits_all = ctx.buffer(key + ("logits_all",), (tmax, bsz, v)) if keep_logits else None
        logits_one = ctx.buffer(key + ("logits",), (bsz, v))
        xent_rows = ctx.buffer(key + ("xent_rows",), (tmax, bsz), zero=True) if has_tgt else None
        stepper = make_stepper(self, ctx, bsz, "greedy")
        stepper.start(s0)
        emb = stepper.emb_view
        att_states = [a.initial_loop_state(ctx, bsz, tmax) for a in self.attentions]

        go = ctx.buffer(key + ("go",), (bsz,), torch.int32)
        ops.fill(go, START_TOKEN_INDEX)
        self.embed_input_symbols(ctx, go, out=emb)
        att0 = att_states
        graph_ok = getattr(stepper, "graph_safe", False)
        indexed = getattr(stepper, "indexed", False)
        for att in self.attentions if graph_ok else []:
            att.hidden_features(ctx)
            att.attention_mask(ctx)
        self.decoding_bias(ctx)
        t_xent = min(t_target, tmax) if has_tgt else 0

        drops = bool(ctx.fed(self.train_mode)) and self.dropout_keep_prob < 1.0
        use_stats = plain and graph_ok and not drops and self.logits_stats_ok(ctx, out_all[0])
        salts = self.sampling_salts(ctx, tmax) if sample else None
        stats = ctx.buffer(key + ("stats",), (ops.logits_stats_numel(bsz, v),)) if use_stats else None
        table = self.embedding_matrix(ctx)

        resident = getattr(stepper, "state_resident", False)
        h_prev_of = lambda t: s0 if t == 0 else (stepper.sel if resident else s_all[t - 1])

        tabled = getattr(stepper, "table", None) is not None
        ids_kw = (lambda t: {"ids": go if t == 0 else symbols[t - 1]}) if tabled else (lambda t: {})

        def body(t):
            logits = logits_all[t] if keep_logits else logits_one
            st_t = [AttentionLoopState(st.contexts, st.weights, t) for st in att0]
            if use_stats:
                want_logits = keep_logits or t < t_xent
                stepper.step(emb, st_t, out_all[t], logits if want_logits else None, h_out=s_all[t],
                             h_prev=h_prev_of(t), stats=stats, **ids_kw(t))
                if t < t_xent:
                    ops.xent(logits, tgt[t], tmask[t], xent_rows[t])
                ops.greedy_finish(stats, v, finished, symbols[t], omask[t], END_TOKEN_INDEX, allfin[t:t + 1],
                                  table=None if tabled else table, emb_out=None if tabled else emb)
                return
            if graph_ok:
                stepper.step(emb, st_t, out_all[t], logits, h_out=s_all[t], h_prev=h_prev_of(t), **ids_kw(t))
            else:
                if indexed:
                    stepper.set_position(t, 0)
                stepper.step(emb, st_t, out_all[t], logits, h_out=s_all[t])
            if temperature != 1.0:
                ops.ew("scale", logits, None, logits, alpha=1.0 / temperature)
            if sample:
                ops.gumbel_argmax(logits, salts[t], argmax)
            else:
                ops.row_stats(logits, None, None, argmax)
            if t < t_xent:
                ops.xent(logits, tgt[t], tmask[t], xent_rows[t])
            ops.greedy_update(argmax, finished, symbols[t], omask[t], END_TOKEN_INDEX, allfin[t:t + 1])
            if not (tabled and graph_ok):
                self.embed_input_symbols(ctx, symbols[t], out=emb)

        shape_key = tuple(tuple(st.weights.shape) for st in att0)
        graphed = (graph_ok or indexed) and not sample
        chunk_key = key + ("chunk", bsz, t_xent, shape_key, getattr(stepper, "shape_key", ()))

        def launch(t0, n):
            def chunk():
                for t in range(t0, t0 + n):
                    body(t)
            if graphed:
                ctx.session.graphed(chunk_key + (t0, n), chunk)
            else:
                chunk()
        steps, _ = ctx.session.decode_chunks(tmax, CHECK_EVERY, launch, allfin, run_ahead=graphed)
        xent_sum = None
        if has_tgt:
            xent_sum = ctx.buffer(key + ("xent_sum",), (1,))
            ops.reduce_sum(xent_rows[:min(steps, t_target)].reshape(-1), xent_sum)
        att_states = [AttentionLoopState(st.contexts, st.weights, steps) for st in att_states]
        for att, st in zip(self.attentions, att_states):
            att.finalize_loop("{}_run".format(self.name), st)
        return RuntimeResult(symbols[:steps], omask[:steps], steps, xent_sum,
                             logits_all[:steps] if keep_logits else None, out_all[:steps], s_all[:steps],
                             [st.weights[:steps] for st in att_states])

    @tensor
    def runtime_loss(self, ctx):
        res = self.runtime_loop_result(ctx)
        if res.xent_sum is None:
            return 0.0
        return res.xent_sum[0] / res.mask.sum().to(torch.float32)

    @tensor
    def decoded_symbols(self, ctx) -> torch.Tensor:
        return self.runtime_loop_result(ctx).symbols

    @tensor
    def runtime_mask(self, ctx) -> torch.Tensor:
        return self.runtime_loop_result(ctx).mask

    @tensor
    def runtime_logits(self, ctx) -> torch.Tensor:
        key = (id(self), "runtime_full")
        if key not in ctx.memo:
            ctx.memo[key] = self._runtime_loop(ctx, keep_logits=True)
        return ctx.memo[key].logits

    @tensor
    def runtime_logprobs(self, ctx) -> torch.Tensor:
        logits = self.runtime_logits(ctx)
        t, b, v = logits.shape
        mx = ctx.buffer((id(self), "lp_max"), (t * b,))
        lse = ctx.buffer((id(self), "lp_lse"), (t * b,))
        ops.row_stats(logits.view(t * b, v), mx, lse, None)
        out = ctx.buffer((id(self), "logprobs"), (t, b, v))
        ops.log_softmax_from_stats(logits.view(t * b, v), mx, lse, out.view(t * b, v))
        return out

    @tensor
    def train_logprobs(self, ctx) -> torch.Tensor:
        logits = self.train_logits(ctx)
        t, b, v = logits.shape
        logits = logits.contiguous()
        mx = ctx.buffer((id(self), "train_lp_max"), (t * b,))
        lse = ctx.buffer((id(self), "train_lp_lse"), (t * b,))
        ops.row_stats(logits.view(t * b, v), mx, lse, None)
        out = ctx.buffer((id(self), "train_logprobs"), (t, b, v))
        ops.log_softmax_from_stats(logits.view(t * b, v), mx, lse, out.view(t * b, v))
        return out

    @tensor
    def runtime_output_states(self, ctx) -> torch.Tensor:
        return self.runtime_loop_result(ctx).output_states

    @tensor
    def train_logits(self, ctx) -> torch.Tensor:
        res = self.train_loop_result(ctx)
        if res.saved["dlogits"] is not None:
            raise RuntimeError("train_logits were overwritten by their gradient in this run")
        steps, bsz = res.saved["steps"], res.saved["bsz"]
        if "tape" in res.saved:
            return res.saved["logits"].view(steps, bsz, -1)
        return ctx.buffer((id(self), "train", "logits"), (steps * bsz, len(self.vocabulary))) \
            .view(steps, bsz, -1)
```

neuralmonkey_amd/ops.py:

```python
import ctypes
import struct
import os
import threading
from typing import Optional

import numpy as np
import torch

from . import _lib

ACT = {None: 0, "none": 0, "tanh": 1, "relu": 2}


def _stream():
    return torch.cuda.current_stream().cuda_stream


def _p(t: Optional[torch.Tensor]):
    return None if t is None else t.data_ptr()


def _f32(t):
    assert t.dtype == torch.float32 and t.is_cuda, (t.dtype, t.device)
    return t
# ... 26 lines not shown
    d = x.shape[-1]
    rows = x.numel() // d
    assert sum_out.is_contiguous() and out.is_contiguous()
    _lib.check(_lib.load().nm_add_layer_norm_stats_fwd(_stream(), a.data_ptr(), x.data_ptr(), gamma.data_ptr(),
                                                       beta.data_ptr(), sum_out.data_ptr(), out.data_ptr(),
                                                       mean.data_ptr(), rstd.data_ptr(), rows, d, float(eps)),
               "nm_add_layer_norm_stats_fwd")
    return sum_out, out


GEMM_BACKGROUND = 4


def gemm(a: torch.Tensor, b: torch.Tensor, out: Optional[torch.Tensor] = None, bias=None, act=None,
         trans_a=False, trans_b=False, accumulate=False, algo=0):
    lib = _lib.load()
    _f32(a), _f32(b)
    batched = a.dim() == 3
    if batched:
        assert b.dim() == 3 and a.shape[0] == b.shape[0]
        nb = a.shape[0]
        a2, b2 = a[0], b[0]
        s_a, s_b = a.stride(0), b.stride(0)
    else:
        nb, a2, b2, s_a, s_b = 1, a, b, 0, 0
    assert a2.stride(1) == 1 and b2.stride(1) == 1, "inner stride must be 1"
    m, k = (a2.shape[1], a2.shape[0]) if trans_a else (a2.shape[0], a2.shape[1])
    kb, n = (b2.shape[1], b2.shape[0]) if trans_b else (b2.shape[0], b2.shape[1])
    assert k == kb, f"inner dims differ: {k} vs {kb}"
    if out is None:
        assert not accumulate
        out = torch.empty((nb, m, n) if batched else (m, n), dtype=torch.float32, device=a.device)
    o2 = out[0] if batched else out
    assert tuple(o2.shape) == (m, n) and o2.stride(1) == 1
    s_c = out.stride(0) if batched else 0
    ws = _gemm_workspace(a.device) if (nb == 1 and k >= 1024) else None
    _lib.check(lib.nm_gemm_f32(_stream(), int(trans_a), int(trans_b), m, n, k,
                               a.data_ptr(), a2.stride(0), b.data_ptr(), b2.stride(0),
                               out.data_ptr(), o2.stride(0), _p(bias), ACT[act], int(accumulate),
                               nb, s_a, s_b, s_c, algo, _p(ws), ws.numel() * 4 if ws is not None else 0),
               "nm_gemm_f32")
    return out


_GROUP_TABLES = {}


def gemm_group(items, trans_a=False, trans_b=False, accumulate=True):
    lib = _lib.load()
    a0, b0, o0 = items[0]
    m, k = (a0.shape[1], a0.shape[0]) if trans_a else (a0.shape[0], a0.shape[1])
    n = b0.shape[0] if trans_b else b0.shape[1]
    lda, ldb, ldc = a0.stride(0), b0.stride(0), o0.stride(0)
    ptrs = []
    for a, b, o in items:
        assert a.shape == a0.shape and b.shape == b0.shape and o.shape == o0.shape
        assert (a.stride(0), b.stride(0), o.stride(0)) == (lda, ldb, ldc) and a.stride(1) == b.stride(1) == o.stride(1) == 1
        assert a.data_ptr() % 16 == 0 and b.data_ptr() % 16 == 0 and o.data_ptr() % 16 == 0
        ptrs += [a.data_ptr(), b.data_ptr(), o.data_ptr()]
    assert len({p for p in ptrs[2::3]}) == len(items), "two products of a group share their output"
    table = _pointer_table(a0.device, ptrs)
    _lib.check(lib.nm_gemm_f32_group(_stream(), int(trans_a), int(trans_b), m, n, k, table.data_ptr(), lda, ldb, ldc,
                                     int(accumulate), len(items)), "nm_gemm_f32_group")


def _pointer_table(device, ptrs):
    key = (device, tuple(ptrs))
    table = _GROUP_TABLES.get(key)
    if table is None:
        if len(_GROUP_TABLES) > 1024:
            _GROUP_TABLES.clear()
        table = _GROUP_TABLES[key] = torch.tensor(ptrs, dtype=torch.int64, device=device)
    return table


def gemm_chain(members, out, accumulate=True):
    lib = _lib.load()
    a0, b0 = members[0]
    rows, m, n = a0.shape[0], a0.shape[1], b0.shape[1]
    lda, ldb = a0.stride(0), b0.stride(0)
    ptrs = []
    for a, b in members:
        assert a.shape == a0.shape and b.shape == b0.shape and (a.stride(0), b.stride(0)) == (lda, ldb)
        assert a.stride(1) == 1 and b.stride(1) == 1 and a.data_ptr() % 16 == 0 and b.data_ptr() % 16 == 0
        ptrs += [a.data_ptr(), b.data_ptr(), 0]
    assert out.shape == (m, n) and out.stride(1) == 1
    table = _pointer_table(a0.device, ptrs)
    ws = _gemm_workspace(a0.device)
    _lib.check(lib.nm_gemm_f32_chain(_stream(), m, n, rows, len(members), table.data_ptr(), lda, ldb, out.data_ptr(),
                                     out.stride(0), int(accumulate), ws.data_ptr(), ws.numel() * 4), "nm_gemm_f32_chain")
    return out


OUTER_CHAIN_MAX = 64


def outer_chain(members, out, accumulate=True):
    w0, d0 = members[0]
    bsz, s, c = out.shape
    assert out.is_contiguous() and len(members) <= OUTER_CHAIN_MAX
    ptrs = []
    for w, d in members:
        assert w.shape[0] == bsz and d.shape == (bsz, c) and w.stride(1) == 1 and d.stride(1) == 1
        assert w.stride(0) == w0.stride(0) and d.stride(0) == d0.stride(0) and w.shape[1] >= s
        ptrs += [w.data_ptr(), d.data_ptr()]
    table = _pointer_table(out.device, ptrs)
    _lib.check(_lib.load().nm_outer_chain(_stream(), table.data_ptr(), len(members), bsz, s, c, w0.stride(0), d0.stride(0),
                                          out.data_ptr(), int(accumulate)), "nm_outer_chain")
    return out


def colsum_chain(members, out, accumulate=True):
    lib = _lib.load()
    x0 = members[0]
    rows, cols, ld = x0.shape[0], x0.shape[1], x0.stride(0)
    for x in members:
        assert x.shape == x0.shape and x.stride(0) == ld and x.stride(1) == 1 and x.data_ptr() % 16 == 0
    table = _pointer_table(x0.device, [x.data_ptr() for x in members])
    ws = _colsum_workspace(x0.device, cols)
    _lib.check(lib.nm_colsum_chain(_stream(), table.data_ptr(), 1, 0, len(members), rows, ld, cols, out.data_ptr(),
                                   int(accumulate), ws.data_ptr(), ws.numel() * 4), "nm_colsum_chain")
    return out


_GEMM_WS = {}
GEMM_WORKSPACE_BYTES = 128 << 20
_TLS = threading.local()


def workspace_tag():
    return getattr(_TLS, "workspace_tag", None)


def set_workspace_tag(tag):
    old = workspace_tag()
    _TLS.workspace_tag = tag
    return old


def _gemm_workspace(device):
    key = (device, _stream(), workspace_tag())
    ws = _GEMM_WS.get(key)
    if ws is None:
        ws = torch.empty(GEMM_WORKSPACE_BYTES // 4, dtype=torch.float32, device=device)
        _GEMM_WS[key] = ws
    return ws


def embedding_gather(table, ids, out=None, mask_pad=False, scale=1.0):
    lib = _lib.load()
    _f32(table), _i32(ids)
    n = ids.numel()
    e = table.shape[1]
    if out is None:
        out = torch.empty(tuple(ids.shape) + (e,), dtype=torch.float32, device=table.device)
    ldo = out.stride(-2) if out.dim() >= 2 else e
    _lib.check(lib.nm_embedding_gather(_stream(), table.data_ptr(), table.shape[0], e,
                                       ids.data_ptr(), n, out.data_ptr(), ldo, int(mask_pad),
                                       float(scale)), "nm_embedding_gather")
    return out


def _rev_mask(ndir, reverse_dir0):
    return 1 if reverse_dir0 else (2 if ndir == 2 else 0)


def gru_gates_fwd(xp, x_dir_off, x_row_stride, x_time_stride, hg, h, ru, rh, lengths, t, ndir, rows, hsz,
                  reverse_dir0=False):
    lib = _lib.load()
    _lib.check(lib.nm_gru_gates_fwd(_stream(), xp.data_ptr(), x_dir_off, x_row_stride, x_time_stride,
                                    hg.data_ptr(), h.data_ptr(), ru.data_ptr(), rh.data_ptr(),
                                    _p(lengths), t, _rev_mask(ndir, reverse_dir0), ndir, rows, hsz),
               "nm_gru_gates_fwd")


def gru_blend_fwd(xp, x_dir_off, x_row_stride, x_time_stride, hc, ru, h_in, h_out, c_save, out,
                  out_dir_off, out_row_stride, out_time_stride, lengths, t, ndir, rows, hsz,
                  reverse_dir0=False):
    lib = _lib.load()
    _lib.check(lib.nm_gru_blend_fwd(_stream(), xp.data_ptr(), x_dir_off, x_row_stride, x_time_stride,
                                    hc.data_ptr(), ru.data_ptr(), h_in.data_ptr(), h_out.data_ptr(),
                                    _p(c_save), _p(out), out_dir_off, out_row_stride, out_time_stride,
                                    _p(lengths), t, _rev_mask(ndir, reverse_dir0), ndir, rows, hsz),
               "nm_gru_blend_fwd")


def layer_norm_fwd(x, gamma, beta, out=None, mean=None, rstd=None, eps=1e-6):
    lib = _lib.load()
    d = x.shape[-1]
    rows = x.numel() // d
    assert x.is_contiguous()
    if out is None:
        out = torch.empty_like(x)
    _lib.check(lib.nm_layer_norm_fwd(_stream(), x.data_ptr(), d, gamma.data_ptr(), beta.data_ptr(),
                                     out.data_ptr(), d, _p(mean), _p(rstd), rows, d, float(eps)),
               "nm_layer_norm_fwd")
    return out


def copy_cols(src, dst):
    lib = _lib.load()
    assert src.dim() == 2 and dst.dim() == 2 and src.stride(1) == 1 and dst.stride(1) == 1
    _lib.check(lib.nm_copy_cols(_stream(), src.data_ptr(), src.stride(0), dst.data_ptr(), dst.stride(0),
                                src.shape[0], src.shape[1]), "nm_copy_cols")


def reduce_sum(x, out):
    lib = _lib.load()
    assert x.is_contiguous()
    _lib.check(lib.nm_reduce_sum(_stream(), x.data_ptr(), x.numel(), out.data_ptr()), "nm_reduce_sum")
    return out


def log_softmax_from_stats(x, rmax, rlse, out):
    lib = _lib.load()
    assert x.dim() == 2 and out.dim() == 2 and x.stride(1) == 1 and out.stride(1) == 1
    _lib.check(lib.nm_log_softmax(_stream(), x.data_ptr(), x.stride(0), rmax.data_ptr(), rlse.data_ptr(),
                                  out.data_ptr(), out.stride(0), x.shape[0], x.shape[1]), "nm_log_softmax")
    return out


def attn_workspace(rows, s, c, device):
    lib = _lib.load()
    nbytes = lib.nm_attn_workspace_bytes(rows, s, c)
    return zero(torch.empty((nbytes + 3) // 4, dtype=torch.float32, device=device))


def gru_rh_seq(ru_all, hprev, out, lengths, ndir, hsz, reverse_dir0=False):
    lib = _lib.load()
    b, s = hprev.shape[0], hprev.shape[1]
    _lib.check(lib.nm_gru_rh_seq(_stream(), ru_all.data_ptr(), hprev.data_ptr(), out.data_ptr(),
                                 _p(lengths), _rev_mask(ndir, reverse_dir0), b, s, ndir, hsz),
               "nm_gru_rh_seq")


def attn_fwd(y, hf, states, mask, v, bias, rows_per_key, ctx, weights, workspace, energies_out=None):
    lib = _lib.load()
    r, a = y.shape
    _, s, c = states.shape
    assert hf.is_contiguous() and states.is_contiguous() and y.is_contiguous()
    assert ctx.stride(1) == 1
    _lib.check(lib.nm_attn_fwd(_stream(), y.data_ptr(), hf.data_ptr(), states.data_ptr(), _p(mask),
                               v.data_ptr(), _p(bias), r, rows_per_key, s, a, c, ctx.data_ptr(),
                               ctx.stride(0), _p(weights), workspace.data_ptr(),
                               workspace.numel() * 4, _p(energies_out)), "nm_attn_fwd")


def attn_fwd_time_major(y_all, hf, states, mask, v, bias, ctx_all, w_all, workspace, energies_out=None):
    lib = _lib.load()
    t, b, a = y_all.shape
    _, s, c = states.shape
    assert y_all.is_contiguous() and ctx_all.is_contiguous() and hf.is_contiguous() and states.is_contiguous()
    _lib.check(lib.nm_attn_fwd_multi(_stream(), y_all.data_ptr(), hf.data_ptr(), states.data_ptr(), _p(mask),
                                     v.data_ptr(), _p(bias), b, t, 1, b, s, a, c, ctx_all.data_ptr(), c,
                                     _p(w_all), workspace.data_ptr(), workspace.numel() * 4,
                                     _p(energies_out)), "nm_attn_fwd_multi")


def row_stats(x, rmax=None, lse=None, argmax=None):
    lib = _lib.load()
    assert x.dim() == 2 and x.stride(1) == 1
    _lib.check(lib.nm_row_stats(_stream(), x.data_ptr(), x.stride(0), x.shape[0], x.shape[1],
                                _p(rmax), _p(lse), _p(argmax)), "nm_row_stats")


def gumbel_argmax(x, salt: int, out):
    lib = _lib.load()
    assert x.dim() == 2 and x.stride(1) == 1 and out.dtype == torch.int32
    _lib.check(lib.nm_gumbel_argmax(_stream(), x.data_ptr(), x.stride(0), x.shape[0], x.shape[1],
                                    int(salt) & 0xFFFFFFFF, out.data_ptr()), "nm_gumbel_argmax")


def greedy_update(argmax, finished, sym_out, mask_out, end_id, all_finished=None):
    lib = _lib.load()
    _lib.check(lib.nm_greedy_update(_stream(), argmax.data_ptr(), finished.data_ptr(),
                                    sym_out.data_ptr(), _p(mask_out), argmax.numel(), end_id,
                                    _p(all_finished)), "nm_greedy_update")


def xent(logits, targets, weights, loss_rows, grad_scale=None, write_grad=False, label_smoothing=0.0):
    lib = _lib.load()
    assert logits.dim() == 2 and logits.stride(1) == 1
    _lib.check(lib.nm_xent(_stream(), logits.data_ptr(), logits.stride(0), logits.shape[0],
                           logits.shape[1], targets.data_ptr(), _p(weights), _p(loss_rows),
                           _p(grad_scale), int(write_grad), float(label_smoothing)), "nm_xent")


XENT_COLSUM_ROWS = 256


def xent_colsum_ok(logits) -> bool:
    v = logits.shape[1]
    return (logits.is_cuda and v % 4 == 0 and v <= 32768 and logits.stride(0) % 4 == 0 and
            logits.data_ptr() % 16 == 0 and os.environ.get("NM_XENT_COLSUM", "1") != "0")


def xent_colsum(logits, targets, weights, loss_rows, grad_scale, label_smoothing, partial):
    lib = _lib.load()
    assert logits.dim() == 2 and logits.stride(1) == 1 and partial.is_contiguous()
    assert partial.shape[1] == logits.shape[1] and 1 <= partial.shape[0] <= logits.shape[0]
    _lib.check(lib.nm_xent_colsum(_stream(), logits.data_ptr(), logits.stride(0), logits.shape[0], logits.shape[1],
                                  targets.data_ptr(), _p(weights), _p(loss_rows), _p(grad_scale),
                                  float(label_smoothing), partial.data_ptr(), partial.shape[0]), "nm_xent_colsum")


def beam_workspace(b, k, v, device):
    lib = _lib.load()
    return torch.empty((lib.nm_beam_workspace_bytes(b, k, v) + 3) // 4, dtype=torch.float32, device=device)


def beam_topk_step(logits, b, k, rmax, rlse, logprob_sum, lengths, finished, penalty, end_id,
                   out_score, out_word, out_beam, out_logprob_sum, out_lengths, out_finished,
                   out_src_row, workspace, all_finished=None):
    lib = _lib.load()
    assert logits.dim() == 2 and logits.stride(1) == 1 and logits.shape[0] == b * k
    _lib.check(lib.nm_beam_topk_step(_stream(), logits.data_ptr(), logits.stride(0), b, k,
                                     logits.shape[1], rmax.data_ptr(), rlse.data_ptr(),
                                     logprob_sum.data_ptr(), lengths.data_ptr(), finished.data_ptr(),
                                     penalty.data_ptr(), end_id, out_score.data_ptr(),
                                     out_word.data_ptr(), out_beam.data_ptr(),
                                     out_logprob_sum.data_ptr(), out_lengths.data_ptr(),
                                     out_finished.data_ptr(), out_src_row.data_ptr(),
                                     workspace.data_ptr(), workspace.numel() * 4, _p(all_finished)),
               "nm_beam_topk_step")


def beam_topk_step_fused(logits, b, k, logprob_sum, lengths, finished, penalty, end_id, out_score, out_word,
                         out_beam, out_logprob_sum, out_lengths, out_finished, out_src_row, workspace, rmax, rlse,
                         all_finished=None):
    lib = _lib.load()
    assert logits.dim() == 2 and logits.stride(1) == 1 and logits.shape[0] == b * k
    _lib.check(lib.nm_beam_topk_step_fused(
        _stream(), logits.data_ptr(), logits.stride(0), b, k, logits.shape[1], logprob_sum.data_ptr(),
        lengths.data_ptr(), finished.data_ptr(), penalty.data_ptr(), end_id, out_score.data_ptr(),
        out_word.data_ptr(), out_beam.data_ptr(), out_logprob_sum.data_ptr(), out_lengths.data_ptr(),
        out_finished.data_ptr(), out_src_row.data_ptr(), workspace.data_ptr(), workspace.numel() * 4,
        _p(all_finished), rmax.data_ptr(), rlse.data_ptr()), "nm_beam_topk_step_fused")


def logits_stats_numel(rows, vocab):
    return _lib.load().nm_logits_stats_bytes(rows, vocab) // 4


def logits_stats_buffer(rows, vocab, device):
    return torch.empty(logits_stats_numel(rows, vocab), dtype=torch.float32, device=device)


def logits_stats_gemm(state, w, bias, stats, out=None, trans_b=False):
    lib = _lib.load()
    _f32(state), _f32(w)
    m, k = state.shape
    n = w.shape[0] if trans_b else w.shape[1]
    assert state.stride(1) == 1 and w.stride(1) == 1 and (out is None or (out.stride(1) == 1 and out.shape == (m, n)))
    _lib.check(lib.nm_logits_stats_gemm(_stream(), int(trans_b), m, n, k, state.data_ptr(), state.stride(0),
                                        w.data_ptr(), w.stride(0), _p(bias), _p(out),
                                        out.stride(0) if out is not None else 0, stats.data_ptr(),
                                        stats.numel() * 4), "nm_logits_stats_gemm")


PROJ_SPLIT = os.environ.get("NM_PROJ_SPLIT", "0") == "1"


def proj_split_prepare(w, trans_b=False, planes=None):
    lib = _lib.load()
    _f32(w)
    assert w.dim() == 2 and w.stride(1) == 1
    n, k = (w.shape[0], w.shape[1]) if trans_b else (w.shape[1], w.shape[0])
    nbytes = lib.nm_proj_split_bytes(n, k)
    if nbytes <= 0:
        return None
    if planes is None or planes.numel() * 2 < nbytes:
        planes = torch.empty(nbytes // 2, dtype=torch.int16, device=w.device)
    _lib.check(lib.nm_proj_split_prepare(_stream(), w.data_ptr(), w.stride(0), int(trans_b), n, k, planes.data_ptr(),
                                         planes.numel() * 2), "nm_proj_split_prepare")
    return planes


def proj_split_forget(w=None):
    _lib.check(_lib.load().nm_proj_split_forget(_p(w)), "nm_proj_split_forget")


def greedy_finish(stats, vocab, finished, sym_out, mask_out, end_id, all_finished=None, table=None, emb_out=None,
                  argmax_out=None, max_out=None, lse_out=None):
    lib = _lib.load()
    rows = sym_out.numel()
    tile = lib.nm_logits_stats_tile(rows)
    ntiles = (vocab + tile - 1) // tile
    if emb_out is not None:
        assert emb_out.dim() == 2 and emb_out.stride(1) == 1 and emb_out.shape[0] == rows
    _lib.check(lib.nm_greedy_finish(_stream(), stats.data_ptr(), ntiles, rows, finished.data_ptr(),
                                    sym_out.data_ptr(), _p(mask_out), end_id, _p(all_finished), _p(table),
                                    table.shape[0] if table is not None else 0,
                                    table.shape[1] if table is not None else 0, _p(emb_out),
                                    emb_out.stride(0) if emb_out is not None else 0, _p(argmax_out), _p(max_out),
                                    _p(lse_out)), "nm_greedy_finish")


def beam_topk_step_tiles(logits, stats, b, k, logprob_sum, lengths, finished, penalty, end_id, out_score, out_word,
                         out_beam, out_logprob_sum, out_lengths, out_finished, out_src_row, workspace, rmax, rlse,
                         all_finished=None, tile=None):
    lib = _lib.load()
    assert logits.dim() == 2 and logits.stride(1) == 1 and logits.shape[0] == b * k
    if tile is None:
        tile = lib.nm_logits_stats_tile(b * k)
    v = logits.shape[1]
    _lib.check(lib.nm_beam_topk_step_tiles(
        _stream(), logits.data_ptr(), logits.stride(0), stats.data_ptr(), tile, b, k, v,
        logprob_sum.data_ptr(), lengths.data_ptr(), finished.data_ptr(), penalty.data_ptr(), end_id,
        out_score.data_ptr(), out_word.data_ptr(), out_beam.data_ptr(), out_logprob_sum.data_ptr(),
        out_lengths.data_ptr(), out_finished.data_ptr(), out_src_row.data_ptr(), workspace.data_ptr(),
        workspace.numel() * 4, _p(all_finished), rmax.data_ptr(), rlse.data_ptr()), "nm_beam_topk_step_tiles")


def attn_partials_layout(rows, s, a, c):
    lib = _lib.load()
    n, po, so = ctypes.c_int64(0), ctypes.c_int64(0), ctypes.c_int64(0)
    if lib.nm_attn_partials_layout(rows, s, a, c, ctypes.byref(n), ctypes.byref(po), ctypes.byref(so)) != 0:
        return None
    return int(n.value), int(po.value), int(so.value)


def attn_fwd_partials(y, hf, states, mask, v, bias, rows_per_key, workspace):
    lib = _lib.load()
    r, a = y.shape
    _, s, c = states.shape
    assert hf.is_contiguous() and states.is_contiguous() and y.is_contiguous()
    _lib.check(lib.nm_attn_fwd_partials(_stream(), y.data_ptr(), hf.data_ptr(), states.data_ptr(), _p(mask),
                                        v.data_ptr(), _p(bias), r, rows_per_key, s, a, c, workspace.data_ptr(),
                                        workspace.numel() * 4), "nm_attn_fwd_partials")


class StepGroup:

    def __init__(self, rows, problems):
        lib = _lib.load()
        self.rows = rows
        self.keep = []
        self.arr = (_lib.StepProblem * len(problems))()
        for slot, spec in zip(self.arr, problems):
            for name, val in spec.items():
                if isinstance(val, torch.Tensor):
                    self.keep.append(val)
                    val = val.data_ptr()
                setattr(slot, name, val)
        self._fn = lib.nm_step_group

    def patch(self, index, **fields):
        for name, val in fields.items():
            setattr(self.arr[index], name, val.data_ptr() if isinstance(val, torch.Tensor) else (val or 0))

    def launch(self):
        _lib.check(self._fn(_stream(), self.rows, self.arr, len(self.arr)), "nm_step_group")


class DecoderStepCall:

    def __init__(self, fields):
        lib = _lib.load()
        self.keep = {}
        self.desc = _lib.DecoderStep()
        self._set(fields)
        self._fn = lib.nm_decoder_step_fused

    def _set(self, fields):
        for name, val in fields.items():
            if isinstance(val, torch.Tensor):
                self.keep[name] = val
                val = val.data_ptr()
            setattr(self.desc, name, val or 0)

    def launch(self, **fields):
        self._set(fields)
        _lib.check(self._fn(_stream(), ctypes.byref(self.desc)), "nm_decoder_step_fused")


def gather_rows(src, idx, dst):
    lib = _lib.load()
    assert src.dim() == 2 and dst.dim() == 2 and src.stride(1) == 1 and dst.stride(1) == 1
    _lib.check(lib.nm_gather_rows_f32(_stream(), src.data_ptr(), src.stride(0), idx.data_ptr(),
                                      dst.data_ptr(), dst.stride(0), dst.shape[0], dst.shape[1]),
               "nm_gather_rows_f32")


def beam_reorder_tokens(src, src_row, word, dst, steps, rows):
    lib = _lib.load()
    _lib.check(lib.nm_beam_reorder_tokens(_stream(), src.data_ptr(), src_row.data_ptr(),
                                          word.data_ptr(), dst.data_ptr(), steps, rows),
               "nm_beam_reorder_tokens")


def beam_backtrace(src_hist, word_hist, first, out, steps):
    lib = _lib.load()
    rows = first.numel()
    assert src_hist.is_contiguous() and word_hist.is_contiguous() and out.is_contiguous()
    assert src_hist.shape[1] == rows and word_hist.shape[1] == rows and out.shape[1] == rows and out.shape[0] > steps
    _lib.check(lib.nm_beam_backtrace(_stream(), src_hist.data_ptr(), word_hist.data_ptr(), first.data_ptr(),
                                     out.data_ptr(), steps, rows), "nm_beam_backtrace")


def length_penalty_table(max_len: int, alpha: float, device) -> torch.Tensor:
    lens = np.arange(max_len + 1, dtype=np.float32)
    tab = ((np.float32(5.0) + lens) / np.float32(6.0)) ** np.float32(alpha)
    return torch.from_numpy(tab.astype(np.float32)).to(device)


def tanh_bwd(dy, y):
    lib = _lib.load()
    assert dy.is_contiguous() and y.is_contiguous() and dy.numel() == y.numel()
    _lib.check(lib.nm_tanh_bwd(_stream(), dy.data_ptr(), y.data_ptr(), dy.numel()), "nm_tanh_bwd")
    return dy


_COLSUM_WS = {}


def _colsum_workspace(device, cols):
    key = (device, cols, _stream(), workspace_tag())
    ws = _COLSUM_WS.get(key)
    if ws is None:
        ws = zero(torch.empty(_lib.load().nm_colsum_workspace_bytes(cols) // 4, dtype=torch.float32, device=device))
        _COLSUM_WS[key] = ws
    return ws


def colsum(x, out, accumulate=False):
    lib = _lib.load()
    assert x.dim() == 2 and x.stride(1) == 1
    cols = x.shape[1]
    ws = _colsum_workspace(x.device, cols)
    _lib.check(lib.nm_colsum_algo(_stream(), x.data_ptr(), x.stride(0), x.shape[0], cols, out.data_ptr(),
                                  int(accumulate), ws.data_ptr(), ws.numel() * 4,
                                  1 if getattr(_TLS, "on_side", False) else 0), "nm_colsum")
    return out


def embedding_scatter_add(dtable, ids, d, skip_pad=False):
    lib = _lib.load()
    assert d.dim() == 2 and d.stride(1) == 1 and dtable.is_contiguous()
    _lib.check(lib.nm_embedding_scatter_add(_stream(), dtable.data_ptr(), dtable.shape[0], dtable.shape[1],
                                            ids.data_ptr(), ids.numel(), d.data_ptr(), d.stride(0),
                                            int(skip_pad)), "nm_embedding_scatter_add")


_LNB_WS = {}


def layer_norm_bwd_params(dy, x, mean, rstd, gamma, dx, dgamma, dbeta, accumulate=True, accumulate_dx=False):
    lib = _lib.load()
    d = x.shape[-1]
    rows = x.numel() // d
    assert dy.is_contiguous() and x.is_contiguous() and dx.is_contiguous()
    key = (x.device, d)
    ws = _LNB_WS.get(key)
    if ws is None:
        ws = _LNB_WS[key] = torch.empty(lib.nm_layer_norm_bwd_params_workspace_bytes(d) // 4, dtype=torch.float32,
                                        device=x.device)
    _lib.check(lib.nm_layer_norm_bwd_params(_stream(), dy.data_ptr(), x.data_ptr(), mean.data_ptr(), rstd.data_ptr(),
                                            gamma.data_ptr(), dx.data_ptr(), rows, d, dgamma.data_ptr(),
                                            dbeta.data_ptr(), int(bool(accumulate)) | (2 if accumulate_dx else 0),
                                            ws.data_ptr(), ws.numel() * 4), "nm_layer_norm_bwd_params")


def layer_norm_bwd(dy, x, mean, rstd, gamma, dx, dyx):
    lib = _lib.load()
    d = x.shape[-1]
    rows = x.numel() // d
    assert dy.is_contiguous() and x.is_contiguous() and dx.is_contiguous() and dyx.is_contiguous()
    _lib.check(lib.nm_layer_norm_bwd(_stream(), dy.data_ptr(), x.data_ptr(), mean.data_ptr(),
                                     rstd.data_ptr(), gamma.data_ptr(), dx.data_ptr(), dyx.data_ptr(),
                                     rows, d), "nm_layer_norm_bwd")


def gru_step_bwd(phase, dh, dout, dout_strides, ru, c, h0, hseq, hseq_strides, dxp, dxp_strides, dgpre,
                 dcpre, drh, lengths, t, ndir, rows, hsz, reverse_dir0=False):
    lib = _lib.load()
    do = dout_strides or (0, 0, 0)
    _lib.check(lib.nm_gru_step_bwd(_stream(), phase, dh.data_ptr(), _p(dout), do[0], do[1], do[2],
                                   ru.data_ptr(), _p(c), _p(h0), hseq.data_ptr(), hseq_strides[0],
                                   hseq_strides[1], hseq_strides[2], dxp.data_ptr(), dxp_strides[0],
                                   dxp_strides[1], dxp_strides[2], dgpre.data_ptr(), _p(dcpre), _p(drh),
                                   _p(lengths), t, _rev_mask(ndir, reverse_dir0), ndir, rows, hsz),
               "nm_gru_step_bwd")


def gru_seq_shift(seq, out, lengths, ndir, hsz, reverse_dir0=False):
    lib = _lib.load()
    b, s = seq.shape[0], seq.shape[1]
    _lib.check(lib.nm_gru_seq_shift(_stream(), seq.data_ptr(), out.data_ptr(), _p(lengths),
                                    _rev_mask(ndir, reverse_dir0), b, s, ndir, hsz), "nm_gru_seq_shift")


def attn_softmax_bwd(dw, e, mask, de, bsz):
    lib = _lib.load()
    s = dw.shape[-1]
    rows = dw.numel() // s
    _lib.check(lib.nm_attn_softmax_bwd(_stream(), dw.data_ptr(), e.data_ptr(), _p(mask), de.data_ptr(),
                                       rows, bsz, s), "nm_attn_softmax_bwd")


def attn_step_bwd(dctx, states, e, mask, hf, y, v, de, dy):
    lib = _lib.load()
    b, s, c = states.shape
    a = hf.shape[2]
    assert states.is_contiguous() and hf.is_contiguous() and e.is_contiguous() and de.is_contiguous()
    assert dctx.stride(1) == 1 and y.stride(1) == 1 and dy.stride(1) == 1
    _lib.check(lib.nm_attn_step_bwd(_stream(), dctx.data_ptr(), dctx.stride(0), states.data_ptr(), e.data_ptr(), _p(mask),
# ... 1005 lines not shown
```

Baseline: 601,000 tokens/s.

## Fuse vocab cross-entropy into logits GEMM epilogue and backward GEMM loaders

Adds a fused cross-entropy path. The vocabulary GEMM epilogue computes per-tile softmax statistics, stores exp(logit - tile_max) and captures the target logit. A small merge kernel then produces per-tile rescale factors and the loss. The backward dstate and dweight GEMMs rebuild dlogits on the fly in their tile loaders (scale by a factor, subtract the one-hot target), and the dweight pass also accumulates the bias gradient. This removes the separate full-vocab softmax/xent pass and the dlogits writes over a 6400x32000 matrix. In exchange the loader does extra per-element work and fast __expf is used, which may change precision.

```diff
diff --git a/include/nmhip_xent.h b/include/nmhip_xent.h
--- /dev/null
+++ b/include/nmhip_xent.h
@@ -0,0 +1,29 @@
+#ifndef NMHIP_XENT_H
+#define NMHIP_XENT_H
+#include <stdint.h>
+#ifdef __cplusplus
+extern "C" {
+#endif
+
+int64_t nm_xent_tiles(int64_t V);
+
+int nm_xent_logits_fwd(void* stream, int64_t rows, int64_t V, int64_t K, const float* state, int64_t lds,
+                       const float* W, int64_t ldw, const float* bias, float* E, int64_t lde, float* stats,
+                       int64_t stats_bytes, const int32_t* targets, float* tlogit);
+
+int nm_xent_merge(void* stream, const float* stats, int64_t rows, int64_t V, const float* tlogit,
+                  const int32_t* targets, const float* weights, const float* grad_scale, float* loss_rows, float* f,
+                  float* hw);
+
+int nm_xent_dstate(void* stream, int64_t rows, int64_t V, int64_t state_size, const float* E, int64_t lde,
+                   const float* f, const int32_t* targets, const float* hw, const float* W, int64_t ldw,
+                   float* d_state, int64_t ldd, void* workspace, int64_t workspace_bytes);
+
+int nm_xent_dweight(void* stream, int64_t rows, int64_t V, int64_t state_size, const float* state, int64_t lds,
+                    const float* E, int64_t lde, const float* f, const int32_t* targets, const float* hw, float* dW,
+                    int64_t lddw, float* db, int accumulate, int algo);
+
+#ifdef __cplusplus
+}
+#endif
+#endif
diff --git a/neuralmonkey_amd/_lib.py b/neuralmonkey_amd/_lib.py
--- a/neuralmonkey_amd/_lib.py
+++ b/neuralmonkey_amd/_lib.py
@@ -176,6 +176,13 @@
     "nm_conv1d_glu_bwd": (I, [P, P, L, L, L, L, L, P, P, P, P, L, P, P, L, I, P, P, I, P, L, I]),
 }
 
+XENT_SIGNATURES = {
+    "nm_xent_tiles": (L, [L]),
+    "nm_xent_logits_fwd": (I, [P, L, L, L, P, L, P, L, P, P, L, P, L, P, P]),
+    "nm_xent_merge": (I, [P, P, L, L, P, P, P, P, P, P, P]),
+    "nm_xent_dstate": (I, [P, L, L, L, P, L, P, P, P, P, L, P, L, P, L]),
+    "nm_xent_dweight": (I, [P, L, L, L, P, L, P, L, P, P, P, P, L, P, I, I]),
+}
 
 
 class NMHipError(RuntimeError):
@@ -232,7 +239,7 @@
     lib = ctypes.CDLL(LIB_PATH)
     for name, (res, args) in (list(SIGNATURES.items()) + list(CTC_SIGNATURES.items())
                               + list(LABEL_SIGNATURES.items()) + list(POOL_SIGNATURES.items())
-                              + list(CONVS2S_SIGNATURES.items())):
+                              + list(CONVS2S_SIGNATURES.items()) + list(XENT_SIGNATURES.items())):
         fn = getattr(lib, name)
         fn.restype = res
         fn.argtypes = args
diff --git a/neuralmonkey_amd/csrc/nm_gemm.hip b/neuralmonkey_amd/csrc/nm_gemm.hip
--- a/neuralmonkey_amd/csrc/nm_gemm.hip
+++ b/neuralmonkey_amd/csrc/nm_gemm.hip
@@ -27,6 +27,13 @@
     int prio;
     const float* const* ptrs;
     int chain_k;
+    int xe_store_e;
+    const int* xe_t;
+    float* xe_tlogit;
+    const float* xe_f;
+    const float* xe_hw;
+    int xe_tiles;
+    float* xe_db;
 };
 
 __device__ __forceinline__ float apply_act(float x, int act) {
@@ -52,9 +59,112 @@
     }
 }
 
-template <int WM, int WN, int TM, int TN, bool TA, bool TB, bool VEC, int BK, bool STATS = false, int PF = 1,
-          int NCH = 1, bool CHAIN = false>
-__global__ __launch_bounds__(WM * WN * 64) void gemm_tiled(GemmArgs g, int tiles_m) {
+struct LoadIdentity {
+    static constexpr bool identity = true;
+    __device__ __forceinline__ void init(const GemmArgs&, int, int, int, int) {}
+    __device__ __forceinline__ void load(const GemmArgs&, int) {}
+    __device__ __forceinline__ float4 a(float4 v, int, int) { return v; }
+    __device__ __forceinline__ float4 b(float4 v, int, int) { return v; }
+    __device__ __forceinline__ void finish(const GemmArgs&, float*, int, int) {}
+};
+
+template <int NT, int KQ, int LA>
+struct XentLoadA {
+    static constexpr bool identity = false;
+    int t[LA], foff[LA], kq;
+    float hw[LA], fv[LA];
+    __device__ __forceinline__ void init(const GemmArgs& g, int tid, int m0, int, int) {
+        kq = (tid % KQ) * 4;
+#pragma unroll
+        for (int it = 0; it < LA; ++it) {
+            const int gm = m0 + (tid + it * NT) / KQ;
+            const bool ok = gm < g.M;
+            const int gc = ok ? gm : g.M - 1;
+            const int tt = g.xe_t[gc];
+            t[it] = (ok && tt >= 0 && tt < g.K) ? tt : -1;
+            hw[it] = g.xe_hw[gc];
+            foff[it] = gc;
+            fv[it] = 0.0f;
+        }
+    }
+    __device__ __forceinline__ void load(const GemmArgs& g, int k0) {
+#pragma unroll
+        for (int it = 0; it < LA; ++it) fv[it] = g.xe_f[(long)min(k0 >> 7, g.xe_tiles - 1) * g.M + foff[it]];
+    }
+    __device__ __forceinline__ float4 a(float4 v, int it, int k0) {
+        const int d = t[it] - (k0 + kq);
+        const float f = fv[it], h = hw[it];
+        v.x = v.x * f - (d == 0 ? h : 0.0f);
+        v.y = v.y * f - (d == 1 ? h : 0.0f);
+        v.z = v.z * f - (d == 2 ? h : 0.0f);
+        v.w = v.w * f - (d == 3 ? h : 0.0f);
+        return v;
+    }
+    __device__ __forceinline__ float4 b(float4 v, int, int) { return v; }
+    __device__ __forceinline__ void finish(const GemmArgs&, float*, int, int) {}
+};
+
+template <int NT, int BN, int BK, int LB>
+struct XentLoadB {
+    static constexpr bool identity = false;
+    static constexpr int KR = NT / (BN / 4);
+    static_assert(KR * LB == BK, "one float4 of every k-row per thread set");
+    int t[LB], kr, gn, kmax, nmax;
+    float hw[LB], fv[LB];
+    float4 cs[LB];
+    bool sums;
+    __device__ __forceinline__ void init(const GemmArgs& g, int tid, int, int n0, int bm) {
+        kmax = g.K;
+        nmax = g.N;
+        kr = tid / (BN / 4);
+        gn = n0 + (tid % (BN / 4)) * 4;
+        sums = bm == 0 && g.xe_db != nullptr;
+#pragma unroll
+        for (int it = 0; it < LB; ++it) { cs[it] = make_float4(0.f, 0.f, 0.f, 0.f); t[it] = -1; hw[it] = fv[it] = 0.0f; }
+    }
+    __device__ __forceinline__ void load(const GemmArgs& g, int k0) {
+        const int tile = gn / BN;
+#pragma unroll
+        for (int it = 0; it < LB; ++it) {
+            const int rc = min(k0 + kr + it * KR, g.K - 1);
+            t[it] = g.xe_t[rc];
+            hw[it] = g.xe_hw[rc];
+            fv[it] = g.xe_f[(long)tile * g.K + rc];
+        }
+    }
+    __device__ __forceinline__ float4 a(float4 v, int, int) { return v; }
+    __device__ __forceinline__ float4 b(float4 v, int it, int k0) {
+        const bool hot = k0 + kr + it * KR < kmax && (unsigned)t[it] < (unsigned)nmax;
+        const int d = hot ? t[it] - gn : -1;
+        const float f = fv[it], h = hw[it];
+        v.x = v.x * f - (d == 0 ? h : 0.0f);
+        v.y = v.y * f - (d == 1 ? h : 0.0f);
+        v.z = v.z * f - (d == 2 ? h : 0.0f);
+        v.w = v.w * f - (d == 3 ? h : 0.0f);
+        if (sums) { cs[it].x += v.x; cs[it].y += v.y; cs[it].z += v.z; cs[it].w += v.w; }
+        return v;
+    }
+    __device__ __forceinline__ void finish(const GemmArgs& g, float* red, int tid, int n0) {
+        if (!sums) return;
+#pragma unroll
+        for (int it = 0; it < LB; ++it)
+            *reinterpret_cast<float4*>(red + (kr + it * KR) * BN + (gn - n0)) = cs[it];
+        __syncthreads();
+        const int col = n0 + tid;
+        if (tid < BN && col < g.N) {
+            float s = 0.0f;
+#pragma unroll
+            for (int k = 0; k < BK; ++k) s += red[k * BN + tid];
+            g.xe_db[col] = g.accumulate ? g.xe_db[col] + s : s;
+        }
+    }
+};
+
+template <int WM, int WN, int TM, int TN, bool TA, bool TB, bool VEC, int BK, bool STATS, int PF, int NCH, bool CHAIN,
+          class XF>
+__device__ __forceinline__ void gemm_tiled_body(const GemmArgs& g, int tiles_m, XF xf) {
+    static_assert(XF::identity || (PF == 1 && NCH == 1 && VEC && !STATS && !CHAIN),
+                  "loader transforms: the one-tile-ahead loop on float4 loads");
     static_assert(!CHAIN || (TA && !TB && VEC && !STATS), "chained K: the weight-gradient form only");
     constexpr int NT = WM * WN * 64;
     constexpr int BM = WM * 32 * TM, BN = WN * 32 * TN;
@@ -175,19 +285,20 @@
             rb[it] = v;
         }
     };
-    auto store_lds = [&](int buf, const float4* ra, const float4* rb) {
+    auto store_lds = [&](int buf, const float4* ra, const float4* rb, int k0) {
 #pragma unroll
         for (int it = 0; it < LA; ++it) {
             const int idx = tid + it * NT;
             if (TA) {
                 const int k = idx / (BM / 4), m = (idx % (BM / 4)) * 4;
-                *reinterpret_cast<float4*>(&As[buf][k][m]) = ra[it];
+                *reinterpret_cast<float4*>(&As[buf][k][m]) = xf.a(ra[it], it, k0);
             } else {
                 const int m = idx / KQ, k = (idx % KQ) * 4;
-                As[buf][k + 0][m] = ra[it].x;
-                As[buf][k + 1][m] = ra[it].y;
-                As[buf][k + 2][m] = ra[it].z;
-                As[buf][k + 3][m] = ra[it].w;
+                const float4 v = xf.a(ra[it], it, k0);
+                As[buf][k + 0][m] = v.x;
+                As[buf][k + 1][m] = v.y;
+                As[buf][k + 2][m] = v.z;
+                As[buf][k + 3][m] = v.w;
             }
         }
 #pragma unroll
@@ -195,13 +306,14 @@
             const int idx = tid + it * NT;
             if (!TB) {
                 const int k = idx / (BN / 4), n = (idx % (BN / 4)) * 4;
-                *reinterpret_cast<float4*>(&Bs[buf][k][n]) = rb[it];
+                *reinterpret_cast<float4*>(&Bs[buf][k][n]) = xf.b(rb[it], it, k0);
             } else {
                 const int n = idx / KQ, k = (idx % KQ) * 4;
-                Bs[buf][k + 0][n] = rb[it].x;
-                Bs[buf][k + 1][n] = rb[it].y;
-                Bs[buf][k + 2][n] = rb[it].z;
-                Bs[buf][k + 3][n] = rb[it].w;
+                const float4 v = xf.b(rb[it], it, k0);
+                Bs[buf][k + 0][n] = v.x;
+                Bs[buf][k + 1][n] = v.y;
+                Bs[buf][k + 2][n] = v.z;
+                Bs[buf][k + 3][n] = v.w;
             }
         }
     };
@@ -251,9 +363,11 @@
         }
     };
 
+    xf.init(g, tid, m0, n0, bm);
     load_a(kt0 * BK, ra0);
     load_b(kt0 * BK, rb0);
-    store_lds(0, ra0, rb0);
+    xf.load(g, kt0 * BK);
+    store_lds(0, ra0, rb0, kt0 * BK);
     __syncthreads();
     if constexpr (PF == 2) {
         if (kt0 + 1 < nkt) { load_a((kt0 + 1) * BK, ra1); load_b((kt0 + 1) * BK, rb1); }
@@ -261,21 +375,21 @@
         while (kt < nkt) {
             if (kt + 2 < nkt) { load_a((kt + 2) * BK, ra0); load_b((kt + 2) * BK, rb0); }
             mma_tile(0, accs[0]);
-            if (kt + 1 < nkt) store_lds(1, ra1, rb1);
+            if (kt + 1 < nkt) store_lds(1, ra1, rb1, 0);
             __syncthreads();
             if (++kt >= nkt) break;
             if (kt + 2 < nkt) { load_a((kt + 2) * BK, ra1); load_b((kt + 2) * BK, rb1); }
             mma_tile(1, accs[0]);
-            if (kt + 1 < nkt) store_lds(0, ra0, rb0);
+            if (kt + 1 < nkt) store_lds(0, ra0, rb0, 0);
             __syncthreads();
             ++kt;
         }
     } else if constexpr (NCH == 1) {
         int cur = 0;
         for (int kt = kt0; kt < nkt; ++kt) {
-            if (kt + 1 < nkt) { load_a((kt + 1) * BK, ra0); load_b((kt + 1) * BK, rb0); }
+            if (kt + 1 < nkt) { load_a((kt + 1) * BK, ra0); load_b((kt + 1) * BK, rb0); xf.load(g, (kt + 1) * BK); }
             mma_tile(cur, accs[0]);
-            if (kt + 1 < nkt) store_lds(cur ^ 1, ra0, rb0);
+            if (kt + 1 < nkt) store_lds(cur ^ 1, ra0, rb0, (kt + 1) * BK);
             __syncthreads();
             cur ^= 1;
         }
@@ -286,7 +400,7 @@
             for (int c = 0; c < NCH; ++c) {
                 if (kt + 1 < nkt) { load_a((kt + 1) * BK, ra0); load_b((kt + 1) * BK, rb0); }
                 mma_tile(c & 1, accs[c]);
-                if (kt + 1 < nkt) store_lds((c & 1) ^ 1, ra0, rb0);
+                if (kt + 1 < nkt) store_lds((c & 1) ^ 1, ra0, rb0, 0);
                 __syncthreads();
                 if (++kt >= nkt) break;
             }
@@ -306,6 +420,7 @@
             }
     }
 
+    xf.finish(g, smem, tid, n0);
     if (g.splitk > 1) {
         GemmArgs gs = g;
         gs.ldc = g.N; gs.bias = nullptr; gs.act = 0; gs.accumulate = 0;
@@ -324,6 +439,7 @@
         static_assert(NP * HR == BM, "statistics epilogue: whole passes");
         constexpr int TPR = NT / HR, CW = BN / TPR;
         static_assert(NT % HR == 0 && BN % TPR == 0 && TPR <= 16, "statistics epilogue thread layout");
+        __shared__ float rowm[BM];
         float* T = smem;
         float* pmax = smem + HR * TS;
         int* parg = reinterpret_cast<int*>(pmax + NT);
@@ -371,8 +487,13 @@
 #pragma unroll
             for (int w = 1; w < TPR; ++w) m = fmaxf(m, pmax[w * HR + rr]);
             float sum = 0.0f;
-#pragma unroll
-            for (int c = 0; c < CW; ++c) sum += expf(trow[c] - m);
+            if (g.xe_store_e) {
+#pragma unroll
+                for (int c = 0; c < CW; ++c) sum += __expf(trow[c] - m);
+            } else {
+#pragma unroll
+                for (int c = 0; c < CW; ++c) sum += expf(trow[c] - m);
+            }
             psum[q * HR + rr] = sum;
             __syncthreads();
             const int row = m0 + h * HR + tid;
@@ -390,9 +511,26 @@
                 float4 rec;
                 rec.x = bm; rec.y = tot; rec.z = __int_as_float(a); rec.w = 0.0f;
                 *reinterpret_cast<float4*>(g.stats + ((long)row * tiles_n + bn) * 4) = rec;
+                if (g.xe_store_e) {
+                    rowm[h * HR + tid] = bm;
+                    const int t = g.xe_t[row];
+                    if (t >= n0 && t < n0 + BN && t < g.N) g.xe_tlogit[row] = T[tid * TS + (t - n0)];
+                }
             }
         }
         if (!g.store_c) return;
+        if (g.xe_store_e) {
+            __syncthreads();
+#pragma unroll
+            for (int i = 0; i < TM; ++i)
+#pragma unroll
+                for (int r = 0; r < 16; ++r) {
+                    const int rl = wm + i * 32 + (r & 3) + 8 * (r >> 2) + 4 * (lane >> 5);
+                    const float mr = m0 + rl < g.M ? rowm[rl] : 0.0f;
+#pragma unroll
+                    for (int j = 0; j < TN; ++j) acc[i][j][r] = __expf(acc[i][j][r] - mr);
+                }
+        }
         GemmArgs gs = g;
         gs.bias = nullptr;
 #pragma unroll
@@ -408,6 +546,20 @@
 #pragma unroll
         for (int j = 0; j < TN; ++j)
             store_tile32(g, C, acc[i][j], m0 + wm + i * 32, n0 + wn + j * 32, lane);
+}
+
+template <int WM, int WN, int TM, int TN, bool TA, bool TB, bool VEC, int BK, bool STATS = false, int PF = 1,
+          int NCH = 1, bool CHAIN = false>
+__global__ __launch_bounds__(WM * WN * 64) void gemm_tiled(GemmArgs g, int tiles_m) {
+    gemm_tiled_body<WM, WN, TM, TN, TA, TB, VEC, BK, STATS, PF, NCH, CHAIN>(g, tiles_m, LoadIdentity{});
+}
+
+template <int MODE>
+__global__ __launch_bounds__(512) void gemm_xent(GemmArgs g, int tiles_m) {
+    if constexpr (MODE == 0)
+        gemm_tiled_body<4, 2, 1, 2, false, true, true, 16, false, 1, 1, false>(g, tiles_m, XentLoadA<512, 4, 1>{});
+    else
+        gemm_tiled_body<4, 2, 1, 2, true, false, true, 16, false, 1, 1, false>(g, tiles_m, XentLoadB<512, 128, 16, 1>{});
 }
 
 __global__ void splitk_reduce(GemmArgs g) {
@@ -1059,6 +1211,24 @@
 #undef NM_GT
 }
 
+static long splitk_makespan(long M, long N, long K, bool big, long tiles, int64_t workspace_bytes) {
+    const long nkt = (K + 15) / 16;
+    const double kt_us = big ? 0.95 : 0.30;
+    long best_sk = 1;
+    double best = 1e30;
+    for (long sk = 1; sk <= 16; ++sk) {
+        if (sk > 1 && (K / sk < 128 || sk * M * N * (long)sizeof(float) > workspace_bytes)) break;
+        const long blocks = tiles * sk;
+        const long rounds = (blocks + 255) / 256;
+        const double per_cu = (double)blocks / 256.0;
+        const double thin = per_cu <= 1.0 ? 1.35 : (per_cu <= 2.0 ? 1.15 : 1.0);
+        double cost = (double)rounds * (double)((nkt + sk - 1) / sk) * kt_us * thin;
+        if (sk > 1) cost += (double)(sk + 1) * M * N * 4.0 / 3.0e6 + 3.0;
+        if (cost < best) { best = cost; best_sk = sk; }
+    }
+    return best_sk;
+}
+
 extern "C" int nm_gemm_f32(void* stream, int transA, int transB, int64_t M, int64_t N, int64_t K,
                            const float* A, int64_t lda, const float* B, int64_t ldb, float* C,
                            int64_t ldc, const float* bias, int act, int accumulate, int64_t batch,
@@ -1111,20 +1281,7 @@
             const int tile = big ? 128 : 64;
             const long tiles = (long)nm_cdiv(M, tile) * nm_cdiv(N, tile);
             const int sk_env = sw.gemm_sk;
-            const long nkt = (K + 15) / 16;
-            const double kt_us = big ? 0.95 : 0.30;
-            long best_sk = 1;
-            double best = 1e30;
-            for (long sk = 1; sk <= 16; ++sk) {
-                if (sk > 1 && (K / sk < 128 || sk * M * N * (long)sizeof(float) > workspace_bytes)) break;
-                const long blocks = tiles * sk;
-                const long rounds = (blocks + 255) / 256;
-                const double per_cu = (double)blocks / 256.0;
-                const double thin = per_cu <= 1.0 ? 1.35 : (per_cu <= 2.0 ? 1.15 : 1.0);
-                double cost = (double)rounds * (double)((nkt + sk - 1) / sk) * kt_us * thin;
-                if (sk > 1) cost += (double)(sk + 1) * M * N * 4.0 / 3.0e6 + 3.0;
-                if (cost < best) { best = cost; best_sk = sk; }
-            }
+            long best_sk = splitk_makespan(M, N, K, big, tiles, workspace_bytes);
             if (sk_env > 0 && sk_env <= 16 && K / sk_env >= 128 &&
                 (long)sk_env * M * N * (long)sizeof(float) <= workspace_bytes) best_sk = sk_env;
             if (best_sk >= 2) {
@@ -1207,20 +1364,7 @@
     const int tile = big ? 128 : 64;
     const long tiles = (long)nm_cdiv(M, tile) * nm_cdiv(N, tile);
     if (workspace && K >= 1024) {
-        const long nkt = (K + 15) / 16;
-        const double kt_us = big ? 0.95 : 0.30;
-        long best_sk = 1;
-        double best = 1e30;
-        for (long sk = 1; sk <= 16; ++sk) {
-            if (sk > 1 && (K / sk < 128 || sk * M * N * (long)sizeof(float) > workspace_bytes)) break;
-            const long blocks = tiles * sk;
-            const long rounds = (blocks + 255) / 256;
-            const double per_cu = (double)blocks / 256.0;
-            const double thin = per_cu <= 1.0 ? 1.35 : (per_cu <= 2.0 ? 1.15 : 1.0);
-            double cost = (double)rounds * (double)((nkt + sk - 1) / sk) * kt_us * thin;
-            if (sk > 1) cost += (double)(sk + 1) * M * N * 4.0 / 3.0e6 + 3.0;
-            if (cost < best) { best = cost; best_sk = sk; }
-        }
+        const long best_sk = splitk_makespan(M, N, K, big, tiles, workspace_bytes);
         if (best_sk >= 2) { g.splitk = (int)best_sk; g.ws = reinterpret_cast<float*>(workspace); }
     }
     hipStream_t st = nm_stream(stream);
@@ -1322,3 +1466,88 @@
 #undef NM_ST
     NM_LAUNCH_CHECK("nm_logits_stats_gemm");
 }
+
+extern "C" int64_t nm_xent_tiles(int64_t V) { return V > 0 ? (V + 127) / 128 : 0; }
+
+extern "C" int nm_xent_logits_fwd(void* stream, int64_t rows, int64_t V, int64_t K, const float* state, int64_t lds,
+                                  const float* W, int64_t ldw, const float* bias, float* E, int64_t lde, float* stats,
+                                  int64_t stats_bytes, const int32_t* targets, float* tlogit) {
+    NM_REQUIRE(state && W && E && stats && targets && tlogit, "nm_xent_logits_fwd: null pointer");
+    NM_REQUIRE(rows > 0 && V > 0 && K > 0 && rows < (1 << 30) && V < (1 << 30) && K < (1 << 30) &&
+                   rows * nm_xent_tiles(V) < (1L << 31),
+               "nm_xent_logits_fwd: bad shape %ld %ld %ld", (long)rows, (long)V, (long)K);
+    NM_REQUIRE(stats_bytes >= rows * nm_xent_tiles(V) * 16 && nm_aligned16(stats),
+               "nm_xent_logits_fwd: statistics buffer too small / unaligned");
+    NM_REQUIRE(lds >= K && ldw >= V && lde >= V, "nm_xent_logits_fwd: leading dimension below the row length");
+    NM_REQUIRE(nm_aligned16(state) && lds % 4 == 0 && K % 4 == 0 && nm_aligned16(W) && ldw % 4 == 0 && V % 4 == 0,
+               "nm_xent_logits_fwd: operands must be 16-byte aligned with K, V and the leading dimensions multiples of 4");
+    GemmArgs g{state, W, E, bias, (int)rows, (int)V, (int)K, (long)lds, (long)ldw, (long)lde, 0, 0, 0, 0, 0,
+               nullptr, 1, 1, stats, 1};
+    g.xe_store_e = 1;
+    g.xe_t = targets;
+    g.xe_tlogit = tlogit;
+    const int tiles_m = nm_cdiv(rows, 128), tiles_n = nm_cdiv(V, 128);
+    hipLaunchKernelGGL((gemm_tiled<4, 2, 1, 2, false, false, true, 16, true, 1>), dim3(tiles_m * tiles_n, 1, 1), dim3(512),
+                       0, nm_stream(stream), g, tiles_m);
+    NM_LAUNCH_CHECK("nm_xent_logits_fwd");
+}
+
+static int xent_bwd_check(const char* who, int64_t rows, int64_t V, int64_t odim, const float* E, int64_t lde,
+                          const float* f, const int32_t* targets, const float* hw, const float* X, int64_t ldx,
+                          const float* out, int64_t ldo) {
+    NM_REQUIRE(E && f && targets && hw && X && out, "%s: null pointer", who);
+    NM_REQUIRE(rows > 0 && V > 0 && odim > 0 && rows < (1 << 30) && V < (1 << 30) && odim < (1 << 30) &&
+                   rows * nm_xent_tiles(V) < (1L << 31),
+               "%s: bad shape rows=%ld V=%ld state=%ld", who, (long)rows, (long)V, (long)odim);
+    NM_REQUIRE(nm_aligned16(E) && lde % 4 == 0 && lde >= V && V % 4 == 0 && nm_aligned16(X) && ldx % 4 == 0 &&
+                   odim % 4 == 0 && nm_aligned16(out) && ldo % 4 == 0,
+               "%s: operands must be 16-byte aligned with V, the state size and the leading dimensions multiples of 4", who);
+    return NM_OK;
+}
+
+extern "C" int nm_xent_dstate(void* stream, int64_t rows, int64_t V, int64_t odim, const float* E, int64_t lde,
+                              const float* f, const int32_t* targets, const float* hw, const float* W, int64_t ldw,
+                              float* d_state, int64_t ldd, void* workspace, int64_t workspace_bytes) {
+    const int rc = xent_bwd_check("nm_xent_dstate", rows, V, odim, E, lde, f, targets, hw, W, ldw, d_state, ldd);
+    if (rc != NM_OK) return rc;
+    NM_REQUIRE(ldw >= V && ldd >= odim, "nm_xent_dstate: leading dimension below the row length");
+    GemmArgs g{E, W, d_state, nullptr, (int)rows, (int)odim, (int)V, (long)lde, (long)ldw, (long)ldd, 0, 0, 0, 0, 0,
+               nullptr, 1, 0, nullptr, 1};
+    const NmSwitches& sw = nm_cur()->sw;
+    g.swizzle = sw.gemm_swz;
+    g.xe_f = f; g.xe_t = targets; g.xe_hw = hw; g.xe_tiles = (int)nm_xent_tiles(V);
+    const int tiles_m = nm_cdiv(rows, 128), tiles_n = nm_cdiv(odim, 128);
+    if (workspace && V >= 1024) {
+        long sk = splitk_makespan(rows, odim, V, true, (long)tiles_m * tiles_n, workspace_bytes);
+        const int sk_env = sw.gemm_sk;
+        if (sk_env > 0 && sk_env <= 16 && V / sk_env >= 128 &&
+            (long)sk_env * rows * odim * (long)sizeof(float) <= workspace_bytes) sk = sk_env;
+        if (sk >= 2) { g.splitk = (int)sk; g.ws = reinterpret_cast<float*>(workspace); }
+    }
+    hipStream_t st = nm_stream(stream);
+    hipLaunchKernelGGL(gemm_xent<0>, dim3(tiles_m * tiles_n, g.splitk, 1), dim3(512), 0, st, g, tiles_m);
+    if (g.splitk > 1)
+        hipLaunchKernelGGL(splitk_reduce, dim3(nm_cdiv((long)rows * odim, 256)), dim3(256), 0, st, g);
+    NM_LAUNCH_CHECK("nm_xent_dstate");
+}
+
+extern "C" int nm_xent_dweight(void* stream, int64_t rows, int64_t V, int64_t odim, const float* state, int64_t lds,
+                               const float* E, int64_t lde, const float* f, const int32_t* targets, const float* hw,
+                               float* dW, int64_t lddw, float* db, int accumulate, int algo) {
+    const int rc = xent_bwd_check("nm_xent_dweight", rows, V, odim, E, lde, f, targets, hw, state, lds, dW, lddw);
+    if (rc != NM_OK) return rc;
+    NM_REQUIRE(lds >= odim && lddw >= V, "nm_xent_dweight: leading dimension below the row length");
+    NM_REQUIRE(algo == 0 || algo == 4, "nm_xent_dweight: algo %d (0 or 4, the background launch)", algo);
+    GemmArgs g{state, E, dW, nullptr, (int)odim, (int)V, (int)rows, (long)lds, (long)lde, (long)lddw, 0, 0, 0, 0,
+               accumulate, nullptr, 1, 0, nullptr, 1};
+    const NmSwitches& sw = nm_cur()->sw;
+    g.swizzle = sw.gemm_swz;
+    g.xe_f = f; g.xe_t = targets; g.xe_hw = hw; g.xe_tiles = (int)nm_xent_tiles(V);
+    g.xe_db = db;
+    const int bg_lds = (algo == 4 || sw.background) ? bg_lds_target() : 0;
+    const int tiles_m = nm_cdiv(odim, 128), tiles_n = nm_cdiv(V, 128);
+    static DevMask devs;
+    launch_padded(gemm_xent<1>, devs, bg_pad(bg_lds, 33792), dim3(tiles_m * tiles_n, 1, 1), dim3(512),
+                  nm_stream(stream), g, tiles_m);
+    NM_LAUNCH_CHECK("nm_xent_dweight");
+}
diff --git a/neuralmonkey_amd/csrc/nm_logits.hip b/neuralmonkey_amd/csrc/nm_logits.hip
--- a/neuralmonkey_amd/csrc/nm_logits.hip
+++ b/neuralmonkey_amd/csrc/nm_logits.hip
@@ -1214,3 +1214,49 @@
                        first, out, (int)steps, (int)R);
     NM_LAUNCH_CHECK("nm_beam_backtrace");
 }
+
+__global__ __launch_bounds__(256) void xent_merge_kernel(const float4* __restrict__ stats, int rows, int tiles, int V,
+                                                         const float* __restrict__ tlogit,
+                                                         const int* __restrict__ targets,
+                                                         const float* __restrict__ weights,
+                                                         const float* __restrict__ grad_scale,
+                                                         float* __restrict__ loss_rows, float* __restrict__ f,
+                                                         float* __restrict__ hw) {
+    const int lane = threadIdx.x & 63;
+    const int row = blockIdx.x * 4 + (threadIdx.x >> 6);
+    if (row >= rows) return;
+    const float4* rec = stats + (long)row * tiles;
+    float mx = -INFINITY;
+    for (int j = lane; j < tiles; j += 64) mx = fmaxf(mx, rec[j].x);
+    mx = nm_wave_max(mx);
+    float S = 0.0f;
+    for (int j0 = 0; j0 < tiles; j0 += 64) {
+        const int j = j0 + lane;
+        float term = 0.0f;
+        if (j < tiles) { const float4 r = rec[j]; term = r.y * expf(r.x - mx); }
+        const int n = min(64, tiles - j0);
+        for (int l = 0; l < n; ++l) S += __shfl(term, l, 64);
+    }
+    const float w = weights ? weights[row] : 1.0f;
+    const float wg = w * (grad_scale ? grad_scale[0] : 1.0f);
+    const float scale = wg / S;
+    for (int j = lane; j < tiles; j += 64) f[(long)j * rows + row] = scale * expf(rec[j].x - mx);
+    if (lane == 0) {
+        const int t = targets[row];
+        loss_rows[row] = (t >= 0 && t < V) ? (mx + logf(S) - tlogit[row]) * w : 0.0f;
+        hw[row] = wg;
+    }
+}
+
+extern "C" int nm_xent_merge(void* stream, const float* stats, int64_t rows, int64_t V, const float* tlogit,
+                             const int32_t* targets, const float* weights, const float* grad_scale, float* loss_rows,
+                             float* f, float* hw) {
+    NM_REQUIRE(stats && tlogit && targets && loss_rows && f && hw, "nm_xent_merge: null pointer");
+    NM_REQUIRE(rows > 0 && V > 0 && rows < (1 << 30) && V < (1 << 30) && rows * ((V + 127) / 128) < (1L << 31),
+               "nm_xent_merge: bad shape rows=%ld V=%ld", (long)rows, (long)V);
+    NM_REQUIRE(nm_aligned16(stats), "nm_xent_merge: statistics not 16-byte aligned");
+    hipLaunchKernelGGL(xent_merge_kernel, dim3((unsigned)((rows + 3) / 4)), dim3(256), 0, nm_stream(stream),
+                       reinterpret_cast<const float4*>(stats), (int)rows, (int)((V + 127) / 128), (int)V, tlogit, targets,
+                       weights, grad_scale, loss_rows, f, hw);
+    NM_LAUNCH_CHECK("nm_xent_merge");
+}
diff --git a/neuralmonkey_amd/decoders/decoder.py b/neuralmonkey_amd/decoders/decoder.py
--- a/neuralmonkey_amd/decoders/decoder.py
+++ b/neuralmonkey_amd/decoders/decoder.py
@@ -297,14 +297,29 @@
         self.output_projection.apply(ctx, self, s_all.view(rows, h), emb_all.view(rows, e),
                                      [st.contexts.view(rows, -1) for st in att_states], out_all)
         logits = ctx.buffer(key + ("logits",), (rows, v))
-        self.state_to_logits(ctx, out_all, logits)
         loss_rows = ctx.buffer(key + ("loss_rows",), (rows,))
         db_partial = None
-        if want_grad and not self.tie_embeddings and ops.xent_colsum_ok(logits):
+        xent_fused = None
+        if (want_grad and ops.XENT_FUSED and not self.tie_embeddings and not self.label_smoothing
+                and self.logits_stats_ok(ctx, out_all)):
+            tiles = ops.xent_tiles(v)
+            stats = ctx.buffer(key + ("xe_stats",), (rows * tiles * 4,))
+            tlogit = ctx.buffer(key + ("xe_tlogit",), (rows,))
+            xe_f = ctx.buffer(key + ("xe_f",), (tiles, rows))
+            xe_hw = ctx.buffer(key + ("xe_hw",), (rows,))
+            tflat = tgt.reshape(-1)
+            ops.xent_logits_fwd(out_all, self.var(ctx, "state_to_word_W"), self.decoding_bias(ctx), logits, stats,
+                                tflat, tlogit)
+            ops.xent_merge(stats, v, tlogit, tflat, self.xent_weights(tmask.reshape(-1)), grad_scale, loss_rows,
+                           xe_f, xe_hw)
+            xent_fused = (xe_f, tflat, xe_hw)
+        elif want_grad and not self.tie_embeddings and ops.xent_colsum_ok(logits):
+            self.state_to_logits(ctx, out_all, logits)
             db_partial = ctx.buffer(key + ("db_partial",), (min(rows, ops.XENT_COLSUM_ROWS), v))
             ops.xent_colsum(logits, tgt.reshape(-1), self.xent_weights(tmask.reshape(-1)), loss_rows, grad_scale,
                             self.label_smoothing or 0.0, db_partial)
         else:
+            self.state_to_logits(ctx, out_all, logits)
             ops.xent(logits, tgt.reshape(-1), self.xent_weights(tmask.reshape(-1)), loss_rows, grad_scale, want_grad,
                      self.label_smoothing or 0.0)
         loss_sum = ctx.buffer(key + ("loss_sum",), (1,))
@@ -314,7 +329,8 @@
         saved = {"emb_all": emb_all, "xp": xp, "s0": s0, "s_all": s_all, "s_ext": s_ext, "ru_all": ru_all,
                  "c_all": c_all, "rh_all": rh_all, "y_all": y_all, "e_all": e_all,
                  "att_states": att_states, "out_all": out_all,
-                 "dlogits": logits if want_grad else None, "db_partial": db_partial, "cell": cell, "steps": steps,
+                 "dlogits": logits if want_grad else None, "db_partial": db_partial, "xent_fused": xent_fused,
+                 "cell": cell, "steps": steps,
                  "bsz": bsz,
                  "loss_rows": loss_rows, "loss_layout": "tb"}
         return TrainResult(loss_sum, self.train_token_count(ctx), steps, saved)
@@ -343,7 +359,10 @@
         dp_overlap = dp is not None and bool(ctx.memo.get("dp_overlap", False))
 
         d_out = ctx.buffer(key + ("d_out",), (rows, odim))
-        if self.tie_embeddings:
+        xent_fused = sv.get("xent_fused")
+        if xent_fused is not None:
+            ops.xent_dstate(dlogits, *xent_fused, self.var(ctx, "state_to_word_W"), d_out)
+        elif self.tie_embeddings:
             emat = self.embedding_matrix(ctx)
             ops.gemm(dlogits, emat, out=d_out)
         else:
@@ -372,7 +391,12 @@
             ops.colsum(d_out, store.g(self.var_name("attention_decoder/{}/bias".format(proj.scope))), accumulate=acc)
 
         def vocabulary_projection_gradient():
-            if self.tie_embeddings:
+            if xent_fused is not None:
+                ops.xent_dweight(out_all, dlogits, *xent_fused, store.g(self.var_name("state_to_word_W")),
+                                 db=store.g(self.var_name("state_to_word_b")), accumulate=acc, algo=bg)
+                if dp_overlap:
+                    dp.all_reduce_early(store, [self.var_name("state_to_word_W"), self.var_name("state_to_word_b")])
+            elif self.tie_embeddings:
                 ops.gemm(dlogits, out_all, out=store.g(self.embedding_matrix_name), trans_a=True,
                          accumulate=True, algo=bg)
             else:
diff --git a/neuralmonkey_amd/ops.py b/neuralmonkey_amd/ops.py
--- a/neuralmonkey_amd/ops.py
+++ b/neuralmonkey_amd/ops.py
@@ -352,6 +352,70 @@
     _lib.check(lib.nm_xent_colsum(_stream(), logits.data_ptr(), logits.stride(0), logits.shape[0], logits.shape[1],
                                   targets.data_ptr(), _p(weights), _p(loss_rows), _p(grad_scale),
                                   float(label_smoothing), partial.data_ptr(), partial.shape[0]), "nm_xent_colsum")
+
+
+XENT_FUSED = os.environ.get("NM_XENT_FUSED", "1") != "0"
+XENT_FUSED_LAUNCHES = 0
+
+
+def xent_tiles(vocab: int) -> int:
+    return _lib.load().nm_xent_tiles(vocab)
+
+
+def xent_logits_fwd(state, w, bias, e_out, stats, targets, tlogit):
+    global XENT_FUSED_LAUNCHES
+    _f32(state), _f32(w), _f32(e_out), _f32(stats), _f32(tlogit), _i32(targets)
+    rows, k = state.shape
+    v = w.shape[1]
+    assert w.shape[0] == k and e_out.shape == (rows, v) and targets.numel() == rows == tlogit.numel()
+    assert state.stride(1) == 1 and w.stride(1) == 1 and e_out.stride(1) == 1 and targets.is_contiguous()
+    XENT_FUSED_LAUNCHES += 1
+    _lib.check(_lib.load().nm_xent_logits_fwd(_stream(), rows, v, k, state.data_ptr(), state.stride(0), w.data_ptr(),
+                                              w.stride(0), _p(bias), e_out.data_ptr(), e_out.stride(0),
+                                              stats.data_ptr(), stats.numel() * 4, targets.data_ptr(),
+                                              tlogit.data_ptr()), "nm_xent_logits_fwd")
+
+
+def xent_merge(stats, vocab, tlogit, targets, weights, grad_scale, loss_rows, f, hw):
+    global XENT_FUSED_LAUNCHES
+    rows = loss_rows.numel()
+    assert f.is_contiguous() and f.shape == (xent_tiles(vocab), rows) and hw.numel() == rows == tlogit.numel()
+    assert stats.numel() >= rows * f.shape[0] * 4 and targets.numel() == rows and targets.is_contiguous()
+    _f32(stats), _f32(f), _f32(hw), _f32(loss_rows), _i32(targets)
+    XENT_FUSED_LAUNCHES += 1
+    _lib.check(_lib.load().nm_xent_merge(_stream(), stats.data_ptr(), rows, vocab, tlogit.data_ptr(),
+                                         targets.data_ptr(), _p(weights), _p(grad_scale), loss_rows.data_ptr(),
+                                         f.data_ptr(), hw.data_ptr()), "nm_xent_merge")
+
+
+def xent_dstate(e, f, targets, hw, w, out):
+    global XENT_FUSED_LAUNCHES
+    rows, v = e.shape
+    k = w.shape[0]
+    assert w.shape[1] == v and out.shape == (rows, k) and f.is_contiguous() and f.shape == (xent_tiles(v), rows)
+    assert e.stride(1) == 1 and w.stride(1) == 1 and out.stride(1) == 1 and targets.is_contiguous()
+    _f32(e), _f32(f), _f32(hw), _f32(w), _f32(out), _i32(targets)
+    ws = _gemm_workspace(e.device) if v >= 1024 else None
+    XENT_FUSED_LAUNCHES += 1
+    _lib.check(_lib.load().nm_xent_dstate(_stream(), rows, v, k, e.data_ptr(), e.stride(0), f.data_ptr(),
+                                          targets.data_ptr(), hw.data_ptr(), w.data_ptr(), w.stride(0), out.data_ptr(),
+                                          out.stride(0), _p(ws), ws.numel() * 4 if ws is not None else 0),
+               "nm_xent_dstate")
+    return out
+
+
+def xent_dweight(state, e, f, targets, hw, dw, db=None, accumulate=False, algo=0):
+    global XENT_FUSED_LAUNCHES
+    rows, v = e.shape
+    k = state.shape[1]
+    assert state.shape[0] == rows and dw.shape == (k, v) and f.is_contiguous() and f.shape == (xent_tiles(v), rows)
+    assert e.stride(1) == 1 and state.stride(1) == 1 and dw.stride(1) == 1 and targets.is_contiguous()
+    assert db is None or (db.is_contiguous() and db.numel() == v)
+    _f32(e), _f32(f), _f32(hw), _f32(state), _f32(dw), _i32(targets)
+    XENT_FUSED_LAUNCHES += 1
+    _lib.check(_lib.load().nm_xent_dweight(_stream(), rows, v, k, state.data_ptr(), state.stride(0), e.data_ptr(),
+                                           e.stride(0), f.data_ptr(), targets.data_ptr(), hw.data_ptr(), dw.data_ptr(),
+                                           dw.stride(0), _p(db), int(accumulate), algo), "nm_xent_dweight")
 
 
 def beam_workspace(b, k, v, device):
```

Result: no change. 599,400 tokens/s, median of 2 (-0.3%).
